# rvp-group/Splat-LOAM

Measured on AMD Instinct MI355X. Metric: fwd+bwd Msplats/s, higher is better.
Workload: dtype f32; 1 GPU; 500000 surfels, 64x2048 spherical, 1 keyframe/GPU per iteration drawn from a window of 8 keyframes as Mapper.optimize does (sample_geometric, p=0.4): render fwd + mapper loss + bwd + fused Adam (one native sls_mapping_step per iteration); step=one bench step = 10 mapping iterations (1013 steps = 10130 timed iterations), N=500000, H=64, W=2048, keyframes=8, parallelism=keyframe-dp1, status_read=lagged-1, gradient_sums=float atomics

## Files before the change

### splat_loam_amd/csrc/sls_launch.hpp

```cpp
#pragma once
#include "sls_common.hpp"

namespace sls {

struct ConsumerArgs;

inline bool launch_order_possible(int T) { return T % 32 == 0 && kTileW == 16 && kTileH == 16; }

struct ScanHandoff {
    const uint32_t *block_sums;
    int resort_windows;
    const uint64_t *resort_edges;
    int counted;
};

constexpr int kDirectChunk = 1024;
constexpr int kDirectMaxBins = 512;

struct DirectBin {
    uint32_t *cnt;
    uint32_t *totals;
    uint2 *serec;
    int bins, nchunks, pos0;
    int stride;
    uint32_t *coarse;
};
constexpr int kDirectGroup = 16;

size_t sort_scratch_bytes(uint64_t cap);
size_t order_scratch_bytes(int N);
int radix_sort_pairs_u32(uint32_t *keys, uint32_t *vals, uint32_t *keys_tmp, uint32_t *vals_tmp,
                         const uint32_t *count_ptr, uint32_t cap, int nbits, void *scratch, size_t scratch_bytes,
                         int *result_in_tmp, hipStream_t st);
void depth_order_key_buffers(int N, void *scratch, uint32_t *order, uint32_t **keys, uint32_t **vals0, uint32_t **n_dev);
uint64_t *resort_comp_buffer(int N, void *scratch);
bool bin_direct_possible(const DevCam &cam, int N, uint32_t cap);
DirectBin make_direct_bin(const DevCam &cam, int N, void *sort_scratch, uint2 *serec, bool repaired, bool coarse);
size_t direct_coarse_words(const DevCam &cam, int N);

struct DepthOrderScan {
    int N; const uint32_t *tiles; uint32_t *order, *offsets, *total_out;
    void *scratch; size_t scratch_bytes;
    int reuse_order;
    uint32_t *fail_flag;
    bool window_sort_done;
    const DirectBin *direct;
    const int4 *erec_box; int GX;
};
int launch_depth_order_scan(const DepthOrderScan &a, hipStream_t st, ScanHandoff *handoff);

struct BinSortLaunch {
    int N;
    const uint32_t *count_ptr; uint32_t cap;
    const uint32_t *order; const int32_t *rect; const uint32_t *tiles; const uint64_t *tile_mask; const int32_t *erec;
    const float *depth; const uint32_t *offsets;
    uint32_t *tkeys, *vals, *tkeys_tmp, *vals_tmp;
    void *scratch; size_t scratch_bytes;
    uint32_t *ranges; uint64_t *keys64_out; uint32_t *overflow;
    const ScanHandoff *handoff; uint32_t *total_out;
    const uint32_t *sbox; int bmask_mode;
};
int launch_bin_sort(const DevCam &cam, const BinSortLaunch &a, hipStream_t st, int *sorted_in_tmp, const uint2 **bmask_out);

struct BinDirectLaunch {
    int N; uint32_t cap;
    DirectBin db; bool counted;
    const uint32_t *order; const int32_t *erec_box; const int32_t *rect; const uint32_t *sbox;
    void *scratch; uint32_t *vals_out, *ranges, *total_out, *overflow;
    int resort_windows; const uint64_t *resort_edges; int bmask_mode;
    uint32_t *status_mirror;
};
int launch_bin_direct(const DevCam &cam, const BinDirectLaunch &a, hipStream_t st, const uint2 **bmask_out);

struct PreFwdLaunch {
    int N;
    int raw; float smax, pen; float *reg_out;
    const float *means, *scales, *rots, *opac;
    float *rec; int32_t *radii, *rect; uint32_t *tiles; float *depth;
    uint32_t *order_keys, *order_vals, *n_dev;
    uint32_t *status_clear;
    const float *col_cs, *row_cs; uint64_t *tile_mask;
    int32_t *erec; int erec_box;
    const uint32_t *resort_prev_order; uint64_t *resort_comp;
    uint32_t *sbox;
    uint32_t *zero_words; int n_zero_words;
};
int launch_preprocess_fwd(const DevCam &cam, const PreFwdLaunch &a, hipStream_t st);

struct PreBwdLaunch {
    int N;
    int raw; float smax, pen;
    const float *means, *scales, *rots, *opac;
    float *dmeans, *dscales, *drots, *dopac; const PoseOut *pose;
    const int32_t *radii; const float *grec; const AdamFuse *fuse;
};
int launch_preprocess_bwd(const DevCam &cam, const PreBwdLaunch &a, hipStream_t st);
int launch_preprocess_bwd_batch(const PreBwdLaunch &a, const BatchFuse &bf, hipStream_t st);
int launch_mark_visible(const DevCam &cam, int N, const float *means, uint8_t *visible, hipStream_t st);

size_t block_mask_bytes(uint64_t cap, int T);
struct RenderFwdLaunch {
    const uint32_t *ranges, *vals; const float *rec, *col_cs, *row_cs;
    float *allmap, *pix_state; uint32_t *pix_contrib, *tile_consumed; bool consumed_zeroed;
    uint64_t *block_masks;
    bool lean; uint32_t *block_cost;
    const uint2 *bmask;
    bool order_in_handover;
};
int launch_render_fwd(const DevCam &cam, const RenderFwdLaunch &a, hipStream_t st);

struct RenderBwdLaunch {
    const uint32_t *ranges, *vals; int vals_stride;
    const float *rec, *col_cs, *row_cs, *pix_state; const uint32_t *pix_contrib; const float *dL_dallmap;
    float *grec; uint8_t *touched; bool lean;
    const uint64_t *block_masks; int block_masks_shape;
    const ConsumerArgs *fused_consumer; bool consumer_b_inline;
    uint32_t *det_max; unsigned long long *det_acc;
    const uint8_t *det_prev; const uint32_t *det_gex; uint32_t *det_flag;
    const uint32_t *block_order; uint32_t order_tag;
    bool order_in_handover;
};
int launch_render_bwd(const DevCam &cam, const RenderBwdLaunch &a, hipStream_t st);

size_t consumer_scratch_bytes(int H, int W);
int launch_consumer(const ConsumerArgs &in, int n_valid, void *scratch, size_t scratch_bytes, bool no_launch, hipStream_t st,
                    ConsumerArgs *args_out_skip_c);
int launch_render_maps(int H, int W, const float *allmap, const float *rot9, const float *col_h, const float *row_h,
                       float depth_ratio, float *rend_normal, float *surf_depth, float *surf_normal, hipStream_t st);
int launch_densify_weights(int H, int W, const float *depth, const uint8_t *valid, const float *alpha, float thr, float *w_out,
                           uint32_t *stats, hipStream_t st);
int launch_densify_rows(int n, int H, int W, const int64_t *pix, const float *depth, const float *normal, const float *col_h,
                        const float *row_h, const float *c2w, const float *mTf, float *xyz, float *quat, hipStream_t st);

size_t densify_draw_scratch_bytes(int H, int W);
int launch_densify_draw(int H, int W, const float *depth, const uint8_t *valid, const float *alpha, float thr, double percentage,
                        uint64_t seed, uint32_t draw_index, float *w_out, int64_t *pixels_out, uint32_t *stats,
                        uint32_t *stats_mirror, void *scratch, hipStream_t st);
size_t surface_scratch_bytes(int H, int W);
int launch_surface_samples(int H, int W, const float *allmap, const float *col_h, const float *row_h, const float *M,
                           float min_opacity, float max_depth_dist, float depth_ratio, int n_samples, uint64_t seed,
                           uint32_t frame_id, float *points, float *normals, int32_t *pixels, uint32_t *status, void *scratch,
                           hipStream_t st);
size_t knn_scratch_bytes(int M);
int launch_knn(int M, const float *xyz, float *out, void *scratch, size_t scratch_bytes, hipStream_t st, int Mq);
int launch_touched_bitmap(int N, const uint8_t *touched, const float *scaling_raw, float smax, float pen,
                          const uint32_t *status_block, uint64_t *bitmap, hipStream_t st);
int launch_adam(const SlsAdamGroup *groups, int ngroups, double beta1, double beta2, double eps, int64_t step,
                const uint32_t *skip_flag, hipStream_t stream, const float *void_flags, uint32_t *status_block,
                uint32_t *status_mirror);

}
```

### splat_loam_amd/csrc/sls_pipeline.hip

```cpp
#include <stdlib.h>
#include <string.h>

#include "sls_consumer_dev.hpp"
#include "sls_launch.hpp"

namespace sls {

struct MapWs {
    float *rec; int32_t *radii; int32_t *rect; uint32_t *tiles; uint64_t *tmask; int32_t *erec; int32_t *serec; uint32_t *sbox; float *depth; uint32_t *order; uint32_t *offsets;
    void *order_scratch; size_t order_scratch_bytes;
    uint32_t *tkeys, *vals, *tkeys_tmp, *vals_tmp; void *sort_scratch; size_t sort_scratch_bytes;
    uint32_t *ranges; float *allmap; float *pix_state; uint32_t *pix_contrib; uint32_t *tile_consumed;
    float *dL_dallmap; void *consumer_scratch; size_t consumer_scratch_bytes; float *grec; size_t zero_bytes; uint64_t *block_masks; float *reg_accum; uint8_t *touched;
    uint32_t *det_max; unsigned long long *det_acc; size_t det_bytes;
    uint32_t *det_gex;
    uint32_t *block_cost, *block_order;
    size_t total;
};

struct Taker {
    char *p; size_t off;
    void *operator()(size_t bytes) { void *r = (void *)(p + off); off += (bytes + 255) & ~(size_t)255; return r; }
};

// ... 201 lines not shown
        po->out[g] = pose_grad[g];
    }
    return SLS_OK;
}
static const PoseOut *pose_arg(const PoseOut &po) { return po.counter ? &po : nullptr; }

int sls_backward(const SlsCamera *cam, int N, uint64_t R, const float *means3D, const float *scales,
                 const float *rotations, const int32_t *radii, const float *rec, const uint32_t *ranges,
                 const uint32_t *vals_sorted, int vals_stride, const float *col_cs, const float *row_cs,
                 const float *pix_state, const uint32_t *pix_contrib, const float *dL_dallmap, float *grec,
                 float *dL_dmeans3D, float *dL_dscales, float *dL_drotations, float *dL_dopacities,
                 const uint64_t *block_masks, int block_masks_shape, void *stream)
{
    return sls_backward_pose(cam, N, R, means3D, scales, rotations, radii, rec, ranges, vals_sorted, vals_stride, col_cs,
                             row_cs, pix_state, pix_contrib, dL_dallmap, grec, dL_dmeans3D, dL_dscales, dL_drotations,
                             dL_dopacities, block_masks, block_masks_shape, nullptr, nullptr, 0, stream);
}

int sls_backward_pose(const SlsCamera *cam, int N, uint64_t R, const float *means3D, const float *scales,
                      const float *rotations, const int32_t *radii, const float *rec, const uint32_t *ranges,
                      const uint32_t *vals_sorted, int vals_stride, const float *col_cs, const float *row_cs,
                      const float *pix_state, const uint32_t *pix_contrib, const float *dL_dallmap, float *grec,
                      float *dL_dmeans3D, float *dL_dscales, float *dL_drotations, float *dL_dopacities,
                      const uint64_t *block_masks, int block_masks_shape, float *pose_grad, void *pose_scratch,
                      size_t pose_scratch_bytes_, void *stream)
{
    SLS_REQUIRE(cam, "null pointer");
    SLS_REQUIRE(N >= 0, "negative N");
    if (N == 0) {
        if (pose_grad) SLS_HIP_CHECK(hipMemsetAsync(pose_grad, 0, 6 * sizeof(float), (hipStream_t)stream));
        return SLS_OK;
    }
    PoseOut po;
    if (int prc = make_pose_out(1, N, &pose_grad, pose_scratch, pose_scratch_bytes_, &po)) return prc;
    SLS_REQUIRE(means3D && scales && rotations && radii && grec && dL_dmeans3D && dL_dscales && dL_drotations &&
                    dL_dopacities,
                "null pointer");
    SLS_REQUIRE(vals_stride == 1 || vals_stride == 2, "vals_stride: 1 (plain list) or 2 ((surfel, block mask) pairs)");
    hipStream_t st = (hipStream_t)stream;
    const DevCam dc = make_devcam(*cam);
    {
        ScopedTimer tm(T_GREC_MEMSET, st);
        SLS_HIP_CHECK(hipMemsetAsync(grec, 0, sizeof(float) * (size_t)N * SLS_GREC_STRIDE, st));
    }
    if (R > 0) {
        SLS_REQUIRE(rec && ranges && vals_sorted && col_cs && row_cs && pix_state && pix_contrib && dL_dallmap,
                    "null pointer");
        RenderBwdLaunch rb{};
        rb.ranges = ranges; rb.vals = vals_sorted; rb.vals_stride = vals_stride; rb.rec = rec; rb.col_cs = col_cs; rb.row_cs = row_cs;
        rb.pix_state = pix_state; rb.pix_contrib = pix_contrib; rb.dL_dallmap = dL_dallmap;
        rb.block_masks = block_masks_shape ? block_masks : nullptr; rb.block_masks_shape = block_masks_shape;
        rb.lean = (cam->flags & SLS_CAM_LEAN_ALLMAP) != 0;
        rb.grec = grec; rb.order_in_handover = true;
        if (int rc = launch_render_bwd(dc, rb, st)) return rc;
    }
    PreBwdLaunch pb{};
    pb.N = N; pb.means = means3D; pb.scales = scales; pb.rots = rotations; pb.radii = radii; pb.grec = grec;
    pb.dmeans = dL_dmeans3D; pb.dscales = dL_dscales; pb.drots = dL_drotations; pb.dopac = dL_dopacities;
    pb.pose = pose_arg(po);
    return launch_preprocess_bwd(dc, pb, st);
}

size_t sls_backward_det_scratch_bytes(int N) { return N > 0 ? (size_t)N * SLS_GREC_STRIDE * 12 + 256 : 256; }

int sls_backward_det(const SlsCamera *cam, int N, uint64_t R, const float *means3D, const float *scales,
                     const float *rotations, const int32_t *radii, const float *rec, const uint32_t *ranges,
                     const uint32_t *vals_sorted, int vals_stride, const float *col_cs, const float *row_cs,
                     const float *pix_state, const uint32_t *pix_contrib, const float *dL_dallmap, float *dL_dmeans3D,
                     float *dL_dscales, float *dL_drotations, float *dL_dopacities, const uint64_t *block_masks,
                     int block_masks_shape, void *det_scratch, size_t det_scratch_bytes, void *stream)
{
    return sls_backward_det_pose(cam, N, R, means3D, scales, rotations, radii, rec, ranges, vals_sorted, vals_stride,
                                 col_cs, row_cs, pix_state, pix_contrib, dL_dallmap, dL_dmeans3D, dL_dscales,
                                 dL_drotations, dL_dopacities, block_masks, block_masks_shape, det_scratch,
                                 det_scratch_bytes, nullptr, nullptr, 0, stream);
}

int sls_backward_det_pose(const SlsCamera *cam, int N, uint64_t R, const float *means3D, const float *scales,
                          const float *rotations, const int32_t *radii, const float *rec, const uint32_t *ranges,
                          const uint32_t *vals_sorted, int vals_stride, const float *col_cs, const float *row_cs,
                          const float *pix_state, const uint32_t *pix_contrib, const float *dL_dallmap,
                          float *dL_dmeans3D, float *dL_dscales, float *dL_drotations, float *dL_dopacities,
                          const uint64_t *block_masks, int block_masks_shape, void *det_scratch, size_t det_scratch_bytes,
                          float *pose_grad, void *pose_scratch, size_t pose_scratch_bytes_, void *stream)
{
    SLS_REQUIRE(cam, "null pointer");
    SLS_REQUIRE(N >= 0, "negative N");
    if (N == 0) {
        if (pose_grad) SLS_HIP_CHECK(hipMemsetAsync(pose_grad, 0, 6 * sizeof(float), (hipStream_t)stream));
        return SLS_OK;
    }
    PoseOut po;
    if (int prc = make_pose_out(1, N, &pose_grad, pose_scratch, pose_scratch_bytes_, &po)) return prc;
    SLS_REQUIRE(means3D && scales && rotations && radii && det_scratch && dL_dmeans3D && dL_dscales && dL_drotations &&
                    dL_dopacities,
                "null pointer");
    SLS_REQUIRE(vals_stride == 1 || vals_stride == 2, "vals_stride: 1 (plain list) or 2 ((surfel, block mask) pairs)");
    if (det_scratch_bytes < sls_backward_det_scratch_bytes(N)) {
        set_error("deterministic-backward scratch too small");
        return SLS_E_SCRATCH;
    }
    hipStream_t st = (hipStream_t)stream;
    const DevCam dc = make_devcam(*cam);
    unsigned long long *acc = (unsigned long long *)(((uintptr_t)det_scratch + 255) & ~(uintptr_t)255);
    uint32_t *mx = (uint32_t *)(acc + (size_t)N * SLS_GREC_STRIDE);
    SLS_HIP_CHECK(hipMemsetAsync(acc, 0, (size_t)N * SLS_GREC_STRIDE * 12, st));
    if (R > 0) {
        SLS_REQUIRE(rec && ranges && vals_sorted && col_cs && row_cs && pix_state && pix_contrib && dL_dallmap,
                    "null pointer");
        RenderBwdLaunch rb{};
        rb.ranges = ranges; rb.vals = vals_sorted; rb.vals_stride = vals_stride; rb.rec = rec; rb.col_cs = col_cs; rb.row_cs = row_cs;
        rb.pix_state = pix_state; rb.pix_contrib = pix_contrib; rb.dL_dallmap = dL_dallmap;
        rb.block_masks = block_masks_shape ? block_masks : nullptr; rb.block_masks_shape = block_masks_shape;
        rb.lean = (cam->flags & SLS_CAM_LEAN_ALLMAP) != 0;
        rb.det_max = mx; rb.det_acc = acc; rb.order_in_handover = true;
        if (int rc = launch_render_bwd(dc, rb, st)) return rc;
    }
    AdamFuse fuse;
    memset(&fuse, 0, sizeof(fuse));
    fuse.det_max = mx;
    fuse.det_acc = (const long long *)acc;
    PreBwdLaunch pb{};
    pb.N = N; pb.means = means3D; pb.scales = scales; pb.rots = rotations; pb.radii = radii;
    pb.dmeans = dL_dmeans3D; pb.dscales = dL_dscales; pb.drots = dL_drotations; pb.dopac = dL_dopacities;
    pb.fuse = &fuse; pb.pose = pose_arg(po);
    return launch_preprocess_bwd(dc, pb, st);
}

struct FrontArgs {
    PreFwdLaunch pf;
    uint32_t *depth_order; int reuse_rounds;
    int workspace_ready;
    uint32_t *status_mirror;
    int list_pairs;
    float *allmap; bool lean;
    bool want_backward;
};

static int binning_front(const DevCam &dc, uint32_t cap, const MapWs &w, const FrontArgs &f, SlsMappingStatus *status_dev,
                         hipStream_t st, const uint32_t **sorted_list, int *sorted_stride)
{
    const int N = f.pf.N;
    if (!f.workspace_ready) {
        ScopedTimer tm(T_GREC_MEMSET, st);
        SLS_HIP_CHECK(hipMemsetAsync(w.reg_accum, 0, w.zero_bytes, st));
    }
    uint32_t *okeys, *ovals, *n_dev;
    uint32_t *order = f.depth_order ? f.depth_order : w.order;
    depth_order_key_buffers(N, w.order_scratch, order, &okeys, &ovals, &n_dev);
    const bool merged_sort = f.reuse_rounds >= 1;
    const bool direct = bin_direct_possible(dc, N, cap);
    BinDirectLaunch bd{};
    if (direct) bd.db = make_direct_bin(dc, N, w.sort_scratch, (uint2 *)w.serec, merged_sort, true);
    PreFwdLaunch pf = f.pf;
    pf.rec = w.rec; pf.order_vals = ovals; pf.n_dev = n_dev;
    pf.status_clear = (uint32_t *)status_dev; pf.tile_mask = w.tmask; pf.erec = w.erec;
    if (merged_sort) { pf.resort_prev_order = order; pf.resort_comp = resort_comp_buffer(N, w.order_scratch); }
    if (direct) {
        pf.order_keys = merged_sort ? nullptr : okeys;
        pf.erec_box = 1;
        if (bd.db.coarse) { pf.zero_words = bd.db.coarse; pf.n_zero_words = (int)direct_coarse_words(dc, N); }
    } else {
        pf.rect = w.rect; pf.tiles = w.tiles; pf.depth = w.depth; pf.order_keys = okeys; pf.sbox = w.sbox;
    }
    if (int rc = launch_preprocess_fwd(dc, pf, st)) return rc;
    ScanHandoff handoff = { nullptr, 0, nullptr, 0 };
    DepthOrderScan ds{};
    ds.N = N; ds.tiles = w.tiles; ds.order = order; ds.offsets = w.offsets; ds.total_out = &status_dev->R;
    ds.scratch = w.order_scratch; ds.scratch_bytes = w.order_scratch_bytes;
    ds.reuse_order = f.reuse_rounds; ds.fail_flag = &status_dev->overflow; ds.window_sort_done = merged_sort;
    ds.direct = direct ? &bd.db : nullptr; ds.erec_box = (const int4 *)w.erec; ds.GX = dc.GX;
    if (int rc = launch_depth_order_scan(ds, st, &handoff)) return rc;
    int in_tmp = 0, rc;
    const uint2 *bmask = nullptr;
    if (direct) {
        bd.N = N; bd.cap = cap; bd.counted = handoff.counted != 0; bd.order = order; bd.erec_box = w.erec;
        bd.scratch = w.sort_scratch; bd.vals_out = w.vals; bd.ranges = w.ranges;
        bd.total_out = &status_dev->R; bd.overflow = &status_dev->overflow;
        bd.resort_windows = handoff.resort_windows; bd.resort_edges = handoff.resort_edges;
        bd.bmask_mode = f.list_pairs; bd.status_mirror = f.status_mirror;
        rc = launch_bin_direct(dc, bd, st, &bmask);
    } else {
        BinSortLaunch bs{};
        bs.N = N; bs.count_ptr = &status_dev->R; bs.cap = cap; bs.order = order; bs.rect = w.rect; bs.tiles = w.tiles;
        bs.tile_mask = dc.tile_cull ? w.tmask : nullptr; bs.erec = (dc.GX < 65536 && dc.GY < 65536) ? w.erec : nullptr;
        bs.depth = w.depth; bs.offsets = w.offsets; bs.sbox = w.sbox; bs.bmask_mode = f.list_pairs;
        bs.tkeys = w.tkeys; bs.vals = w.vals; bs.tkeys_tmp = w.tkeys_tmp; bs.vals_tmp = w.vals_tmp;
        bs.scratch = w.sort_scratch; bs.scratch_bytes = w.sort_scratch_bytes; bs.ranges = w.ranges;
        bs.overflow = &status_dev->overflow; bs.handoff = &handoff; bs.total_out = &status_dev->R;
        rc = launch_bin_sort(dc, bs, st, &in_tmp, &bmask);
    }
    if (rc) return rc;
    *sorted_list = bmask ? (const uint32_t *)bmask : (in_tmp ? w.vals_tmp : w.vals);
    *sorted_stride = bmask ? 2 : 1;
    RenderFwdLaunch rf{};
    rf.ranges = w.ranges; rf.vals = *sorted_list; rf.rec = w.rec; rf.col_cs = pf.col_cs; rf.row_cs = pf.row_cs;
    rf.allmap = f.allmap; rf.pix_state = w.pix_state; rf.pix_contrib = w.pix_contrib; rf.lean = f.lean; rf.bmask = bmask;
    rf.consumed_zeroed = true;
    if (f.want_backward) { rf.block_masks = w.block_masks; rf.block_cost = w.block_cost; }
    return launch_render_fwd(dc, rf, st);
}

size_t sls_forward_ws_bytes(int N, int H, int W, uint64_t R_capacity)
{
    return (N < 0 || H <= 0 || W <= 0) ? 0 : carve(N, H, W, R_capacity, nullptr, false).total;
}

int sls_forward_ws(const SlsCamera *cam, int N, const float *means3D, const float *scales, const float *rotations,
                   const float *opacities, const float *col_cs, const float *row_cs, uint64_t R_capacity,
                   uint32_t *depth_order, int reuse_rounds, int list_pairs, int workspace_ready, int want_backward,
                   int32_t *radii, float *allmap, void *workspace, size_t workspace_bytes, SlsMappingStatus *status_dev,
                   SlsMappingStatus *status_mirror, const uint32_t **sorted_list, int *sorted_stride,
                   int *block_masks_shape, void *stream)
{
    SLS_REQUIRE(cam && status_dev && workspace && sorted_list && sorted_stride && block_masks_shape, "null pointer");
    SLS_REQUIRE(N > 0, "N must be positive");
    SLS_REQUIRE(means3D && scales && rotations && opacities && col_cs && row_cs && radii && allmap, "null pointer");
    SLS_REQUIRE(R_capacity > 0 && R_capacity < (1ull << 32), "bad instance capacity");
    SLS_REQUIRE(((uintptr_t)workspace & 255) == 0, "workspace must be 256-byte aligned");
    SLS_REQUIRE(reuse_rounds >= 0 && reuse_rounds <= 4, "reuse_rounds: 0 from scratch, 1..4 repair rounds");
    SLS_REQUIRE(reuse_rounds == 0 || depth_order, "a repair needs the camera's previous depth order");
    SLS_REQUIRE(list_pairs >= 0 && list_pairs <= 2, "list_pairs: 0 auto, 1 whenever possible, 2 never");
    const int H = cam->H, W = cam->W;
    const DevCam dc = make_devcam(*cam);
    const uint32_t cap = (uint32_t)R_capacity;
    if (!bin_direct_possible(dc, N, cap)) {
        set_error("sls_forward_ws serves what the direct binning serves (<= 512 tiles, D10 off): use the staged forward");
        return SLS_E_UNSUPPORTED;
    }
    const MapWs w = carve(N, H, W, R_capacity, workspace, false);
    if (workspace_bytes < w.total) {
        set_error("forward workspace too small: %zu < %zu", workspace_bytes, w.total);
        return SLS_E_SCRATCH;
    }
    FrontArgs f{};
    f.pf.N = N; f.pf.means = means3D; f.pf.scales = scales; f.pf.rots = rotations; f.pf.opac = opacities;
    f.pf.col_cs = col_cs; f.pf.row_cs = row_cs; f.pf.radii = radii;
    f.depth_order = depth_order; f.reuse_rounds = reuse_rounds; f.workspace_ready = workspace_ready;
    f.status_mirror = (uint32_t *)status_mirror;
    f.list_pairs = list_pairs; f.allmap = allmap; f.lean = (cam->flags & SLS_CAM_LEAN_ALLMAP) != 0;
    f.want_backward = want_backward != 0;
    *block_masks_shape = want_backward ? 3 : 0;
    return binning_front(dc, cap, w, f, status_dev, (hipStream_t)stream, sorted_list, sorted_stride);
}

int sls_backward_ws(const SlsCamera *cam, int N, const float *means3D, const float *scales, const float *rotations,
                    const int32_t *radii, const float *col_cs, const float *row_cs, const float *dL_dallmap,
                    uint64_t R_capacity, void *workspace, size_t workspace_bytes, const uint32_t *sorted_list,
                    int sorted_stride, int block_masks_shape, uint32_t *block_order, float *dL_dmeans3D,
                    float *dL_dscales, float *dL_drotations, float *dL_dopacities, void *stream)
{
    return sls_backward_ws_pose(cam, N, means3D, scales, rotations, radii, col_cs, row_cs, dL_dallmap, R_capacity, workspace,
                                workspace_bytes, sorted_list, sorted_stride, block_masks_shape, block_order, dL_dmeans3D,
                                dL_dscales, dL_drotations, dL_dopacities, nullptr, nullptr, 0, stream);
}

int sls_backward_ws_pose(const SlsCamera *cam, int N, const float *means3D, const float *scales, const float *rotations,
                         const int32_t *radii, const float *col_cs, const float *row_cs, const float *dL_dallmap,
                         uint64_t R_capacity, void *workspace, size_t workspace_bytes, const uint32_t *sorted_list,
                         int sorted_stride, int block_masks_shape, uint32_t *block_order, float *dL_dmeans3D,
                         float *dL_dscales, float *dL_drotations, float *dL_dopacities, float *pose_grad,
                         void *pose_scratch, size_t pose_scratch_bytes_, void *stream)
{
    SLS_REQUIRE(cam && workspace && sorted_list, "null pointer");
    SLS_REQUIRE(N > 0, "N must be positive");
    PoseOut po;
    if (int prc = make_pose_out(1, N, &pose_grad, pose_scratch, pose_scratch_bytes_, &po)) return prc;
    SLS_REQUIRE(means3D && scales && rotations && radii && col_cs && row_cs && dL_dallmap && dL_dmeans3D && dL_dscales &&
                    dL_drotations && dL_dopacities,
                "null pointer");
    SLS_REQUIRE(sorted_stride == 1 || sorted_stride == 2, "sorted_stride: 1 (plain list) or 2 ((surfel, block mask) pairs)");
    const MapWs w = carve(N, cam->H, cam->W, R_capacity, workspace, false);
    if (workspace_bytes < w.total) {
        set_error("forward workspace too small: %zu < %zu", workspace_bytes, w.total);
        return SLS_E_SCRATCH;
    }
    hipStream_t st = (hipStream_t)stream;
    const DevCam dc = make_devcam(*cam);
    const int T = dc.GX * dc.GY;
    const bool order_bwd = block_order != nullptr && block_masks_shape == 3 && launch_order_possible(T);
    RenderBwdLaunch rb{};
    rb.ranges = w.ranges; rb.vals = sorted_list; rb.vals_stride = sorted_stride; rb.rec = w.rec; rb.col_cs = col_cs; rb.row_cs = row_cs;
    rb.pix_state = w.pix_state; rb.pix_contrib = w.pix_contrib; rb.dL_dallmap = dL_dallmap;
    rb.block_masks = block_masks_shape ? w.block_masks : nullptr; rb.block_masks_shape = block_masks_shape;
    rb.lean = (cam->flags & SLS_CAM_LEAN_ALLMAP) != 0;
    rb.grec = w.grec; rb.touched = w.touched;
    if (order_bwd) { rb.block_order = block_order; rb.order_tag = block_order_tag(T); }
    if (int rc = launch_render_bwd(dc, rb, st)) return rc;
    AdamFuse fuse;
    memset(&fuse, 0, sizeof(fuse));
    fuse.clear_grec = 1;
    fuse.touched = w.touched;
    if (order_bwd) { fuse.order_T = T; fuse.order_cost = w.block_cost; fuse.order_out = block_order; }
    PreBwdLaunch pb{};
    pb.N = N; pb.means = means3D; pb.scales = scales; pb.rots = rotations; pb.radii = radii; pb.grec = w.grec;
    pb.dmeans = dL_dmeans3D; pb.dscales = dL_dscales; pb.drots = dL_drotations; pb.dopac = dL_dopacities;
    pb.fuse = &fuse; pb.pose = pose_arg(po);
    return launch_preprocess_bwd(dc, pb, st);
}

struct StepSwitches {
    bool det, det_one;
    bool fuse_c, fuse_b;
    bool order_bwd;
};
static StepSwitches step_switches(const SlsMappingConfig *cfg, int deterministic, bool have_det_prev, bool have_block_order, int T)
{
    StepSwitches s;
    s.det = deterministic != 0;
    s.det_one = deterministic == 2 && have_det_prev;
    s.fuse_c = cfg->depth_ratio == 0.0f;
    s.fuse_b = s.fuse_c && have_block_order;
    s.order_bwd = launch_order_possible(T);
    return s;
}

static void loss_weights(const SlsMappingConfig *cfg, int H, int W, int n_valid, float *lw)
{
    lw[0] = 1.0f / ((float)H * (float)W);
    lw[1] = n_valid > 0 ? cfg->lambda_normal * (1.0f / (float)n_valid) : 0.0f;
    lw[2] = n_valid > 0 ? cfg->lambda_alpha * (1.0f / (float)n_valid) : 0.0f;
}

static void fill_step_fuse(AdamFuse &af, const SlsMappingConfig *cfg, SlsMappingStatus *status_dev, float *reg_accum, int N,
                           float *exp_avg, float *exp_avg_sq, int64_t adam_step)
{
    static_assert(sizeof(SlsMappingStatus) == 32, "the mirror copy moves 8 words");
    af.status_src = (uint32_t *)status_dev; af.status_mirror = (uint32_t *)cfg->status_mirror;
    af.reg_accum = reg_accum; af.void_flags = cfg->void_flags_out;
    const bool aligned = (N % 2 == 0) && ((((uintptr_t)exp_avg | (uintptr_t)exp_avg_sq) & 15) == 0);
    if (!cfg->apply_adam || !aligned) return;
    af.enabled = 1;
    af.write_grads = cfg->keep_grads;
    af.c = make_adam_coef(cfg->beta1, cfg->beta2, cfg->eps, adam_step);
    af.lr_xyz = cfg->lr_xyz; af.lr_opacity = cfg->lr_opacity;
    af.lr_scaling = cfg->lr_scaling; af.lr_rotation = cfg->lr_rotation;
    af.exp_avg = exp_avg; af.exp_avg_sq = exp_avg_sq;
}

static int fallback_adam(const SlsMappingConfig *cfg, int N, float *xyz, float *scaling_raw, float *rotation_raw,
                         float *opacity_raw, float *grads, float *exp_avg, float *exp_avg_sq, int64_t adam_step,
                         const uint32_t *skip_flag, hipStream_t st)
{
    SlsAdamGroup grp[4];
    memset(grp, 0, sizeof(grp));
    float *params[4] = { xyz, opacity_raw, scaling_raw, rotation_raw };
    const size_t offs[4] = { 0, (size_t)3 * N, (size_t)4 * N, (size_t)6 * N };
    const int64_t numel[4] = { (int64_t)3 * N, (int64_t)N, (int64_t)2 * N, (int64_t)4 * N };
    const float lrs[4] = { cfg->lr_xyz, cfg->lr_opacity, cfg->lr_scaling, cfg->lr_rotation };
    for (int k = 0; k < 4; ++k) {
        grp[k].param = params[k];
        grp[k].grad = grads + offs[k];
        grp[k].exp_avg = exp_avg + offs[k];
        grp[k].exp_avg_sq = exp_avg_sq + offs[k];
        grp[k].numel = numel[k];
        grp[k].lr = lrs[k];
    }
    return launch_adam(grp, 4, cfg->beta1, cfg->beta2, cfg->eps, adam_step, skip_flag, st, nullptr, nullptr, nullptr);
}

static int mapping_front(const SlsCamera *cam, int N, const float *xyz, const float *scaling_raw, const float *rotation_raw,
                         const float *opacity_raw, const float *gt_depth, const uint8_t *valid, int n_valid,
                         const float *col_cs, const float *row_cs, const float *col_cs_half, const float *row_cs_half,
                         const SlsMappingConfig *cfg, const StepSwitches &sw, uint32_t cap, const MapWs &w,
                         SlsMappingStatus *status_dev, hipStream_t st)
{
    const DevCam dc = make_devcam(*cam);
    const int T = dc.GX * dc.GY;
    FrontArgs f{};
    f.pf.N = N; f.pf.raw = 1; f.pf.smax = cfg->scaling_max; f.pf.pen = cfg->scaling_max_penalty; f.pf.reg_out = w.reg_accum;
    f.pf.means = xyz; f.pf.scales = scaling_raw; f.pf.rots = rotation_raw; f.pf.opac = opacity_raw;
    f.pf.col_cs = col_cs; f.pf.row_cs = row_cs; f.pf.radii = w.radii;
    f.depth_order = cfg->depth_order; f.reuse_rounds = cfg->reuse_depth_order; f.workspace_ready = cfg->workspace_ready;
    f.list_pairs = cfg->block_masks; f.allmap = w.allmap;
// ... 12 lines not shown
    if (sw.det && !sw.det_one) SLS_HIP_CHECK(hipMemsetAsync(w.det_max, 0, w.det_bytes, st));
    RenderBwdLaunch rb{};
    rb.ranges = w.ranges; rb.vals = sorted_vals; rb.vals_stride = vals_stride; rb.rec = w.rec; rb.col_cs = col_cs; rb.row_cs = row_cs;
    rb.pix_state = w.pix_state; rb.pix_contrib = w.pix_contrib; rb.dL_dallmap = w.dL_dallmap; rb.grec = w.grec;
    rb.block_masks = w.block_masks; rb.block_masks_shape = 3;
    rb.lean = sw.fuse_c;
    rb.touched = w.touched;
    rb.fused_consumer = sw.fuse_c ? &cargs : nullptr; rb.consumer_b_inline = sw.fuse_b;
    rb.det_max = (sw.det && !sw.det_one) ? w.det_max : nullptr; rb.det_acc = sw.det ? w.det_acc : nullptr;
    rb.det_prev = sw.det_one ? cfg->det_prev : nullptr; rb.det_gex = w.det_gex; rb.det_flag = &status_dev->overflow;
    if (sw.order_bwd) rb.block_order = sw.fuse_b ? cfg->block_order : w.block_order;
    if (sw.fuse_b && sw.order_bwd) rb.order_tag = block_order_tag(T);
    if (int rc = launch_render_bwd(dc, rb, st)) return rc;
    if (cfg->phase == 1 && cfg->grad_bitmap)
        return launch_touched_bitmap(N, w.touched, scaling_raw, cfg->scaling_max, cfg->scaling_max_penalty,
                                     (const uint32_t *)status_dev, cfg->grad_bitmap, st);
    return SLS_OK;
}

size_t sls_mapping_workspace_bytes(int N, int H, int W, uint64_t R_capacity)
{
    return (N < 0 || H <= 0 || W <= 0) ? 0 : carve(N, H, W, R_capacity, nullptr, true).total;
}

size_t sls_block_order_bytes(int H, int W)
{
    if (H <= 0 || W <= 0) return 0;
    const size_t T = (size_t)((W + kTileW - 1) / kTileW) * (size_t)((H + kTileH - 1) / kTileH);
    return sizeof(uint32_t) * (1 + T * (size_t)(kTilePix / 16));
}

size_t sls_mapping_workspace_bytes_cfg(int N, int H, int W, uint64_t R_capacity, const SlsMappingConfig *cfg)
{
    return (N < 0 || H <= 0 || W <= 0) ? 0 : carve(N, H, W, R_capacity, nullptr, !cfg || cfg->deterministic != 0).total;
}

int sls_mapping_step(const SlsCamera *cam, int N, float *xyz, float *scaling_raw, float *rotation_raw,
                     float *opacity_raw, float *grads, float *exp_avg, float *exp_avg_sq, int64_t adam_step,
                     const float *gt_depth, const uint8_t *valid, int n_valid, const float *col_cs,
                     const float *row_cs, const float *col_cs_half, const float *row_cs_half,
                     const SlsMappingConfig *cfg, uint64_t R_capacity, void *workspace, size_t workspace_bytes,
                     SlsMappingStatus *status_dev, float **allmap_out, void *stream)
{
    SLS_REQUIRE(cam && cfg && status_dev && workspace, "null pointer");
    SLS_REQUIRE(N > 0, "N must be positive");
    SLS_REQUIRE(xyz && scaling_raw && rotation_raw && opacity_raw && grads && gt_depth && valid && col_cs && row_cs &&
                    col_cs_half && row_cs_half,
                "null pointer");
    SLS_REQUIRE(!cfg->apply_adam || (exp_avg && exp_avg_sq && adam_step >= 1), "Adam state missing");
    SLS_REQUIRE(R_capacity > 0 && R_capacity < (1ull << 32), "bad instance capacity");
    SLS_REQUIRE(((uintptr_t)workspace & 255) == 0, "workspace must be 256-byte aligned");
    SLS_REQUIRE(cfg->phase >= 0 && cfg->phase <= 2, "phase: 0 whole iteration, 1 up to the tile backward, 2 the rest");
    PoseOut po;
    {
        float *pg = cfg->pose_grad;
        if (int prc = make_pose_out(1, N, &pg, cfg->pose_scratch, cfg->pose_scratch_bytes, &po)) return prc;
    }
    SLS_REQUIRE(!cfg->grad_bitmap || ((!cfg->apply_adam || cfg->union_bitmap) && !cfg->grad_chunk),
                "the gradient bitmap belongs to apply_adam = 0 with the flat bucket");
    SLS_REQUIRE(!cfg->union_bitmap || (cfg->phase == 2 && cfg->apply_adam && cfg->union_prefix && cfg->grad_compact && cfg->grad_compact_index &&
                                       !cfg->grad_chunk && !cfg->keep_grads && (N % 2) == 0 &&
                                       ((((uintptr_t)exp_avg | (uintptr_t)exp_avg_sq) & 15) == 0)),
                "union_bitmap: phase 2 with apply_adam = 1, the union's prefix and row buffer, even N, 16-byte aligned moments");
    SLS_REQUIRE(!cfg->grad_chunk ||
                    (!cfg->apply_adam && cfg->grad_ranks >= 1 && (cfg->grad_chunk % 4u) == 0 && (N % 2) == 0 &&
                     (uint64_t)cfg->grad_chunk * cfg->grad_ranks >= (uint64_t)10 * (uint64_t)N &&
                     (uint64_t)10 * (uint64_t)N < (1ull << 32)),
                "reduce-scatter gradient layout: apply_adam = 0, even N, chunk a multiple of 4 covering 10 N");
    const int H = cam->H, W = cam->W;
    const MapWs w = carve(N, H, W, R_capacity, workspace, cfg->deterministic != 0);
    if (workspace_bytes < w.total) {
        set_error("mapping workspace too small: %zu < %zu", workspace_bytes, w.total);
        return SLS_E_SCRATCH;
    }
    hipStream_t st = (hipStream_t)stream;
    const DevCam dc = make_devcam(*cam);
    const uint32_t cap = (uint32_t)R_capacity;
    if (allmap_out) *allmap_out = w.allmap;
    SLS_REQUIRE(cfg->deterministic >= 0 && cfg->deterministic <= 2, "deterministic: 0 off, 1 two launches, 2 one launch with predicted scales");
    SLS_REQUIRE(cfg->deterministic != 2 || cfg->det_prev, "deterministic = 2 needs the keyframe's det_prev buffer");
    const int T = dc.GX * dc.GY;
    const StepSwitches sw = step_switches(cfg, cfg->deterministic, cfg->det_prev != nullptr, cfg->block_order != nullptr, T);
    int rc = SLS_OK;
    if (cfg->phase != 2)
        rc = mapping_front(cam, N, xyz, scaling_raw, rotation_raw, opacity_raw, gt_depth, valid, n_valid, col_cs, row_cs,
                           col_cs_half, row_cs_half, cfg, sw, cap, w, status_dev, st);
    if (rc || cfg->phase == 1) return rc;
    AdamFuse fuse;
    memset(&fuse, 0, sizeof(fuse));
    fill_step_fuse(fuse, cfg, status_dev, w.reg_accum, N, exp_avg, exp_avg_sq, adam_step);
    if (fuse.enabled) fuse.skip_flag = &status_dev->overflow;
    fuse.clear_grec = 1;
    fuse.touched = w.touched;
    fuse.void_count = 1; fuse.void_stride = 0;
    if (sw.det) {
        fuse.det_max = w.det_max; fuse.det_acc = (const long long *)w.det_acc;
        fuse.det_prev = cfg->det_prev; fuse.det_gex = w.det_gex; fuse.det_onepass = sw.det_one ? 1 : 0;
    }
    if (sw.fuse_b) {
        fuse.loss_partials = (const float *)w.consumer_scratch;
        fuse.n_loss_partials = T * (kTilePix / 16);
        loss_weights(cfg, H, W, n_valid, fuse.loss_w);
        if (sw.order_bwd) { fuse.order_T = T; fuse.order_cost = w.block_cost; fuse.order_out = cfg->block_order; }
    }
    if (cfg->grad_bitmap && cfg->phase != 2) { fuse.grad_bitmap = cfg->grad_bitmap; fuse.grad_bitmap_words = (N + 63) / 64; }
    if (cfg->grad_chunk) {
        fuse.gchunk = cfg->grad_chunk; fuse.gbase = grads;
        fuse.void_flags = grads + cfg->grad_chunk; fuse.void_count = (int)cfg->grad_ranks; fuse.void_stride = (int)cfg->grad_chunk + 4;
    }
    if (cfg->union_bitmap) {
        fuse.union_bitmap = cfg->union_bitmap; fuse.union_prefix = cfg->union_prefix;
        fuse.compact = cfg->grad_compact; fuse.compact_idx = cfg->grad_compact_index; fuse.compact_cap = cfg->grad_compact_capacity;
    }
    PreBwdLaunch pb{};
    pb.N = N; pb.raw = 1; pb.smax = cfg->scaling_max; pb.pen = cfg->scaling_max_penalty;
    pb.means = xyz; pb.scales = scaling_raw; pb.rots = rotation_raw; pb.opac = opacity_raw; pb.radii = w.radii; pb.grec = w.grec;
    pb.dmeans = grads; pb.dopac = grads + (size_t)3 * N; pb.dscales = grads + (size_t)4 * N; pb.drots = grads + (size_t)6 * N;
    pb.fuse = &fuse; pb.pose = pose_arg(po);
    rc = launch_preprocess_bwd(dc, pb, st);
    if (rc || !cfg->apply_adam || fuse.enabled) return rc;
    return fallback_adam(cfg, N, xyz, scaling_raw, rotation_raw, opacity_raw, grads, exp_avg, exp_avg_sq, adam_step,
                         &status_dev->overflow, st);
}

size_t sls_mapping_workspace_bytes_batch(int G, int N, int H, int W, uint64_t R_capacity, const SlsMappingConfig *cfg)
{
    if (G < 1 || G > SLS_MAX_BATCH || N < 0 || H <= 0 || W <= 0) return 0;
    return carve_batch(G, N, H, W, R_capacity, nullptr, !cfg || cfg->deterministic != 0, nullptr);
}

int sls_mapping_step_batch(int G, const SlsKeyframeInputs *kfs, int N, float *xyz, float *scaling_raw, float *rotation_raw,
                           float *opacity_raw, float *grads, float *exp_avg, float *exp_avg_sq, int64_t adam_step,
                           const SlsMappingConfig *cfg, uint64_t R_capacity, void *workspace, size_t workspace_bytes,
                           SlsMappingStatus *status_dev, void *stream)
{
    SLS_REQUIRE(G >= 1 && G <= SLS_MAX_BATCH, "G: 1 to SLS_MAX_BATCH keyframes");
    SLS_REQUIRE(kfs && cfg && status_dev && workspace, "null pointer");
    SLS_REQUIRE(N > 0, "N must be positive");
    SLS_REQUIRE(xyz && scaling_raw && rotation_raw && opacity_raw && grads, "null pointer");
    SLS_REQUIRE(!cfg->apply_adam || (exp_avg && exp_avg_sq && adam_step >= 1), "Adam state missing");
    SLS_REQUIRE(R_capacity > 0 && R_capacity < (1ull << 32), "bad instance capacity");
    SLS_REQUIRE(((uintptr_t)workspace & 255) == 0, "workspace must be 256-byte aligned");
    SLS_REQUIRE(cfg->phase == 0 && !cfg->grad_chunk && !cfg->grad_bitmap && !cfg->union_bitmap,
                "a batch is one whole step on the flat bucket: phase 0, no grad_chunk, grad_bitmap or union_bitmap");
    SLS_REQUIRE(cfg->deterministic >= 0 && cfg->deterministic <= 2, "deterministic: 0 off, 1 two launches, 2 one launch with predicted scales");
    const int H = kfs[0].cam.H, W = kfs[0].cam.W;
    SLS_REQUIRE(H > 0 && W > 0, "bad image size");
    for (int g = 0; g < G; ++g) {
        const SlsKeyframeInputs &k = kfs[g];
        SLS_REQUIRE(k.cam.H == H && k.cam.W == W, "the keyframes of a batch share one image size");
        SLS_REQUIRE(k.gt_depth && k.valid && k.col_cs && k.row_cs && k.col_cs_half && k.row_cs_half && k.depth_order,
                    "null per-keyframe pointer");
        SLS_REQUIRE((k.block_order != nullptr) == (kfs[0].block_order != nullptr), "block_order on every keyframe or on none");
        SLS_REQUIRE(k.reuse_depth_order >= 0 && k.reuse_depth_order <= 4, "reuse_depth_order: 0 from scratch, 1..4 repair rounds");
        for (int h = 0; h < g; ++h) {
            SLS_REQUIRE(kfs[h].depth_order != k.depth_order, "two keyframes share one depth_order buffer");
            SLS_REQUIRE(!k.block_order || kfs[h].block_order != k.block_order, "two keyframes share one block_order buffer");
            SLS_REQUIRE(!k.det_prev || kfs[h].det_prev != k.det_prev, "two keyframes share one det_prev buffer");
        }
    }
    SLS_REQUIRE(!cfg->pose_grad, "a batch takes its pose gradients per keyframe: SlsKeyframeInputs.pose_grad");
    PoseOut po;
    {
        float *pg[SLS_MAX_BATCH];
        for (int g = 0; g < G; ++g) pg[g] = kfs[g].pose_grad;
        if (int prc = make_pose_out(G, N, pg, cfg->pose_scratch, cfg->pose_scratch_bytes, &po)) return prc;
    }
    const bool det = cfg->deterministic != 0;
    MapWs ws[SLS_MAX_BATCH];
    const size_t need = carve_batch(G, N, H, W, R_capacity, workspace, det, ws);
    if (workspace_bytes < need) {
        set_error("batch workspace too small: %zu < %zu", workspace_bytes, need);
        return SLS_E_SCRATCH;
    }
    hipStream_t st = (hipStream_t)stream;
    const uint32_t cap = (uint32_t)R_capacity;
    const DevCam dc0 = make_devcam(kfs[0].cam);
    const int T = dc0.GX * dc0.GY;
    const StepSwitches sw = step_switches(cfg, det ? 1 : 0, false, kfs[0].block_order != nullptr, T);
    BatchFuse bf;
    memset(&bf, 0, sizeof(bf));
    bf.G = G;
    for (int g = 0; g < G; ++g) {
        const SlsKeyframeInputs &k = kfs[g];
        const MapWs &w = ws[g];
        SlsMappingConfig kc = *cfg;
        kc.reuse_depth_order = k.reuse_depth_order; kc.depth_order = k.depth_order;
        kc.block_order = k.block_order; kc.det_prev = k.det_prev; kc.deterministic = det ? 1 : 0;
        if (g > 0) kc.scaling_max_penalty = 0.0f;
        int rc = mapping_front(&k.cam, N, xyz, scaling_raw, rotation_raw, opacity_raw, k.gt_depth, k.valid, k.n_valid,
                               k.col_cs, k.row_cs, k.col_cs_half, k.row_cs_half, &kc, sw, cap, w, status_dev + 1 + g, st);
        if (rc) return rc;
        BatchKeyframe &b = bf.kf[g];
        b.cam = make_devcam(k.cam);
        b.radii = w.radii; b.grec = (float4 *)w.grec; b.touched = w.touched;
        b.status = (uint32_t *)(status_dev + 1 + g);
        if (det) {
            b.det_max = w.det_max; b.det_acc = (long long *)w.det_acc;
            b.det_prev = k.det_prev;
        }
        if (sw.fuse_b) {
            b.loss_partials = (const float *)w.consumer_scratch;
            loss_weights(cfg, H, W, k.n_valid, b.loss_w);
            if (sw.order_bwd) { b.order_cost = w.block_cost; b.order_out = k.block_order; }
        }
    }
    if (sw.fuse_b) {
        bf.n_loss_partials = T * (kTilePix / 16);
        if (sw.order_bwd) bf.order_T = T;
    }
    AdamFuse &af = bf.af;
    fill_step_fuse(af, cfg, status_dev, ws[0].reg_accum, N, exp_avg, exp_avg_sq, adam_step);
    PreBwdLaunch pb{};
    pb.N = N; pb.raw = 1; pb.smax = cfg->scaling_max; pb.pen = cfg->scaling_max_penalty;
    pb.means = xyz; pb.scales = scaling_raw; pb.rots = rotation_raw; pb.opac = opacity_raw;
    pb.dmeans = grads; pb.dopac = grads + (size_t)3 * N; pb.dscales = grads + (size_t)4 * N; pb.drots = grads + (size_t)6 * N;
    pb.pose = pose_arg(po);
    int rc = launch_preprocess_bwd_batch(pb, bf, st);
    if (rc || !cfg->apply_adam || af.enabled) return rc;
    return fallback_adam(cfg, N, xyz, scaling_raw, rotation_raw, opacity_raw, grads, exp_avg, exp_avg_sq, adam_step,
                         &status_dev->overflow, st);
}

}
```

### splat_loam_amd/csrc/sls_preprocess.hip

```cpp
#include <cstring>
#include "sls_common.hpp"
#include "sls_consumer_dev.hpp"
#include "sls_resort.hpp"
#include "sls_launch.hpp"

namespace sls {

__device__ __forceinline__ float dot3(const float *a, const float *b)
{
    return fmaf(a[0], b[0], fmaf(a[1], b[1], a[2] * b[2]));
}
__device__ __forceinline__ void cross3(const float *a, const float *b, float *o)
{
    o[0] = fmaf(a[1], b[2], -(a[2] * b[1]));
    o[1] = fmaf(a[2], b[0], -(a[0] * b[2]));
    o[2] = fmaf(a[0], b[1], -(a[1] * b[0]));
}
__device__ __forceinline__ void matvec(const float *M, const float *v, float *o)
{
#pragma unroll
    for (int i = 0; i < 3; ++i) o[i] = dot3(M + 3 * i, v);
}
__device__ __forceinline__ void matTvec(const float *M, const float *v, float *o)
{
#pragma unroll
    for (int i = 0; i < 3; ++i) o[i] = fmaf(M[i], v[0], fmaf(M[3 + i], v[1], M[6 + i] * v[2]));
}
__device__ __forceinline__ int floordiv_i(int a, int b)
{
    int q = a / b;
    if ((a % b != 0) && ((a < 0) != (b < 0))) --q;
    return q;
}
__device__ __forceinline__ int posmod_i(int a, int b)
{
    int m = a % b;
    return m < 0 ? m + b : m;
}
__device__ __forceinline__ int to_int_clamped(float v)
{
    v = fminf(fmaxf(v, -1.0e9f), 1.0e9f);
    return (int)v;
}
__device__ __forceinline__ void quat_axes(const float4 q, float *tu, float *tv, float *tn)
{
    const float r = q.x, x = q.y, y = q.z, z = q.w;
    tu[0] = 1.0f - 2.0f * fmaf(y, y, z * z);
    tu[1] = 2.0f * fmaf(x, y, r * z);
    tu[2] = 2.0f * fmaf(x, z, -(r * y));
    tv[0] = 2.0f * fmaf(x, y, -(r * z));
    tv[1] = 1.0f - 2.0f * fmaf(x, x, z * z);
    tv[2] = 2.0f * fmaf(y, z, r * x);
    tn[0] = 2.0f * fmaf(x, z, r * y);
    tn[1] = 2.0f * fmaf(y, z, -(r * x));
    tn[2] = 1.0f - 2.0f * fmaf(x, x, y * y);
}
__device__ __forceinline__ float asin01_approx(float s)
{
    const float c = __builtin_amdgcn_sqrtf(fmaf(-s, s, 1.0f));
    const float mx = fmaxf(s, c), mn = fminf(s, c);
    const float r = sls_atan_unit(mn * __builtin_amdgcn_rcpf(mx));
    return s > c ? SLS_PIO2 - r : r;
}
template <bool EXACT>
__device__ __forceinline__ void ball_extent(float rad, float rho, float rxy, float &theta, float &daz)
{
    if (!(rad < rho)) { theta = SLS_PI; daz = SLS_PI; return; }
    if (EXACT) {
        theta = sls_asin01(rad / rho);
        const float q = rad / rxy;
        if (!(q < 1.0f)) daz = SLS_PI;
        else daz = sls_asin01(q);
    } else {
        theta = asin01_approx(rad * __builtin_amdgcn_rcpf(rho));
        const float q = rad * __builtin_amdgcn_rcpf(rxy);
        if (!(q < 0.9999f)) daz = SLS_PI;
        else daz = asin01_approx(q);
    }
}

__device__ __forceinline__ uint32_t s_rect_cnt(const int4 rc) { return (uint32_t)(rc.y * rc.w); }

struct SurfelGeom {
    float p[3], rho, rho2, rxy, rxy2;
    float Tu[3], Tv[3], Tn[3], n[3], A[3], B[3], Hu[3], Hv[3];
    float su, sv, sig, c;
};

__device__ __forceinline__ float frcp(float x) { return __builtin_amdgcn_rcpf(x); }
__device__ __forceinline__ float fsqrt(float x) { return __builtin_amdgcn_sqrtf(x); }

template <bool EXACT_ROOTS>
__device__ __forceinline__ void surfel_geom(const DevCam &cam, const float *m, const float2 s, const float4 q,
                                            SurfelGeom &g)
{
#pragma unroll
    for (int k = 0; k < 3; ++k)
        g.p[k] = fmaf(cam.R[3 * k], m[0], fmaf(cam.R[3 * k + 1], m[1], fmaf(cam.R[3 * k + 2], m[2], cam.t[k])));
    g.rxy2 = fmaf(g.p[0], g.p[0], g.p[1] * g.p[1]);
    g.rho2 = fmaf(g.p[2], g.p[2], g.rxy2);
    g.rho = EXACT_ROOTS ? sqrtf(g.rho2) : fsqrt(g.rho2);
    g.rxy = EXACT_ROOTS ? sqrtf(g.rxy2) : fsqrt(g.rxy2);
    float tu[3], tv[3], tn[3];
    quat_axes(q, tu, tv, tn);
    matvec(cam.R, tu, g.Tu);
    matvec(cam.R, tv, g.Tv);
    matvec(cam.R, tn, g.Tn);
    g.su = s.x * cam.mod;
    g.sv = s.y * cam.mod;
    g.c = dot3(g.Tn, g.p);
    g.sig = (g.c > 0.0f) ? -1.0f : 1.0f;
    const float isu = g.sig * frcp(g.su), isv = -g.sig * frcp(g.sv);
#pragma unroll
    for (int k = 0; k < 3; ++k) {
        g.n[k] = g.sig * g.Tn[k];
        g.A[k] = g.Tv[k] * isu;
        g.B[k] = g.Tu[k] * isv;
    }
    cross3(g.A, g.p, g.Hu);
    cross3(g.B, g.p, g.Hv);
}

struct RegArgs {
    int raw;
    float smax, pen;
    float *reg_out;
    uint32_t *status_clear;
    uint32_t *zero_words;
    int n_zero_words;
};

template <bool EXACT>
__device__ __forceinline__ void activate(const RegArgs &ra, float2 &s, float4 &q, float &o)
{
    if (!ra.raw) return;
    const float n2 = q.x * q.x + q.y * q.y + q.z * q.z + q.w * q.w;
    s.x = expf(s.x); s.y = expf(s.y);
    o = frcp(1.0f + __expf(-o));
    const float inv = frcp(fmaxf(fsqrt(n2), 1e-12f));
    q.x *= inv; q.y *= inv; q.z *= inv; q.w *= inv;
}

struct PreFwdArgs {
    const float *means; const float2 *scales; const float4 *rots; const float *opac;
    float4 *rec; int *radii; int4 *rect; uint32_t *tiles; float *depth; uint32_t *order_keys, *order_vals, *n_dev;
    const float2 *col_cs, *row_cs; uint64_t *tile_mask; int4 *erec;
    uint32_t *sbox;
    int erec_box;
};
constexpr int kPreCullBytes = 64 * (int)(sizeof(SlsTileCullSurfel) + sizeof(int4) + 4 * sizeof(uint32_t)) + 16;
constexpr int kPreSliceBytes = kPreCullBytes > 64 * kRec4 * 16 ? kPreCullBytes : 64 * kRec4 * 16;

template <int WAVES>
__device__ __forceinline__ void preprocess_fwd_body(const DevCam &cam, const RegArgs &ra, int N, const PreFwdArgs &pa,
                                                    int first, unsigned char *s_mem, float *s_part)
{
    const float *__restrict__ means = pa.means; const float2 *__restrict__ scales = pa.scales;
    const float4 *__restrict__ rots = pa.rots; const float *__restrict__ opac = pa.opac;
    float4 *__restrict__ rec = pa.rec; int *__restrict__ radii = pa.radii; int4 *__restrict__ rect = pa.rect;
    uint32_t *__restrict__ tiles = pa.tiles; float *__restrict__ depth = pa.depth;
    uint32_t *__restrict__ order_keys = pa.order_keys, *__restrict__ order_vals = pa.order_vals, *__restrict__ n_dev = pa.n_dev;
    const float2 *__restrict__ col_cs = pa.col_cs, *__restrict__ row_cs = pa.row_cs;
    uint64_t *__restrict__ tile_mask = pa.tile_mask; int4 *__restrict__ erec = pa.erec;
    const int i = first + (int)threadIdx.x;
    uint32_t my_tiles = 0;
    uint64_t my_mask = 0;
    bool tested = false;
    SlsTileCullSurfel cull;
    int4 my_rc = make_int4(0, 0, 0, 0);
    float my_reg = 0.0f;
    if (i == 0 && n_dev) *n_dev = (uint32_t)N;
    if (ra.zero_words && i < N) {
        for (int k = i; k < ra.n_zero_words; k += N) ra.zero_words[k] = 0u;
    }
    if (i == 0 && ra.status_clear) {
#pragma unroll
        for (int k = 0; k < 8; ++k) ra.status_clear[k] = 0u;
    }
    float4 q0 = make_float4(0, 0, 0, 0), q1 = q0, q2 = q0, q3 = q0, q4 = q0;
    if (i < N) {
        int r_out = 0;
        int4 rc = make_int4(0, 0, 0, 0);
        float dep = 0.0f;

        const float m[3] = { means[3 * i], means[3 * i + 1], means[3 * i + 2] };
        float2 s = scales[i];
        float4 q = rots[i];
        float o = opac[i];
        activate<true>(ra, s, q, o);
        if (ra.pen != 0.0f) my_reg = ra.pen * fmaxf(fmaxf(s.x, s.y) - ra.smax, 0.0f);
        SurfelGeom g;
        surfel_geom<true>(cam, m, s, q, g);
        bool vis = (g.rho >= cam.near_c) && (g.rho < 1.0e18f);
        if (vis) {
            const float az = sls_atan2(g.p[1], g.p[0]);
            const float el = sls_atan2(g.p[2], g.rxy);
            const float cpx = fmaf(cam.fx, az, cam.cx), cpy = fmaf(cam.fy, el, cam.cy);
            const float smax = fmaxf(g.su, g.sv);
            float theta, daz;
            ball_extent<true>(SLS_CUTOFF * smax, g.rho, g.rxy, theta, daz);
            const float rx = fmaxf(fabsf(cam.fx) * daz, SLS_RMIN_PX);
            const float ry = fmaxf(fabsf(cam.fy) * theta, SLS_RMIN_PX);
            int xlo = to_int_clamped(floorf(cpx - rx + 0.5f));
            int xhi = to_int_clamped(floorf(cpx + rx + 0.5f));
            int ylo = to_int_clamped(floorf(cpy - ry + 0.5f));
            int yhi = to_int_clamped(floorf(cpy + ry + 0.5f));
            ylo = max(ylo, 0);
            yhi = min(yhi, cam.H - 1);
            int txlo = 0, ncols = 0;
            if (ylo > yhi) vis = false;
            if (vis) {
                if (cam.wrap) {
                    if ((long long)xhi - (long long)xlo + 1 >= (long long)cam.W) { txlo = 0; ncols = cam.GX; }
                    else {
                        const int a = floordiv_i(xlo, kTileW), b = floordiv_i(xhi, kTileW);
                        ncols = min(b - a + 1, cam.GX);
                        txlo = posmod_i(a, cam.GX);
                    }
                } else {
                    xlo = max(xlo, 0);
                    xhi = min(xhi, cam.W - 1);
                    if (xlo > xhi) vis = false;
                    else { txlo = xlo / kTileW; ncols = xhi / kTileW - txlo + 1; }
                }
            }
            if (vis) {
                const int tylo = ylo / kTileH, nrows = yhi / kTileH - tylo + 1;
                rc = make_int4(txlo, ncols, tylo, nrows);
                my_tiles = (uint32_t)(ncols * nrows);
                my_rc = rc;
                const float dcv[3] = { g.p[0] / g.rho, g.p[1] / g.rho, g.p[2] / g.rho };
                my_mask = my_tiles >= 64u ? ~0ull : ((1ull << my_tiles) - 1ull);
                tested = cam.tile_cull > 0 && tile_mask && my_tiles >= (uint32_t)cam.tile_cull && my_tiles <= 64u;
                if (tested) sls_tile_cull_surfel(g.Tu, g.Tv, g.n, g.p, dcv, g.su, g.sv, o, cpx, cpy, &cull);
                r_out = to_int_clamped(ceilf(fmaxf(rx, ry)));
                dep = g.rho;
                float ex = -1.0e30f, ey = -1.0e30f, kc = 0.0f;
                const float lo = 255.0f * o;
                if (lo > 1.0f) {
                    const float rho_max = 2.0f * __logf(lo) * 1.001f + 1.0e-3f;
                    float th2, daz2;
                    const float kk = __builtin_amdgcn_sqrtf(rho_max), rad = kk * smax;
                    kc = kk * 1.0001f;
                    ball_extent<false>(rad, g.rho, g.rxy, th2, daz2);
                    const float r2 = __builtin_amdgcn_sqrtf(0.5f * rho_max);
                    if (g.rxy > 2.0f * rad && g.rxy > 0.5f * g.rho) {
                        const float irxy2 = __builtin_amdgcn_rcpf(g.rxy2), irho2 = __builtin_amdgcn_rcpf(g.rho2);
                        const float au = (g.p[0] * g.Tu[1] - g.p[1] * g.Tu[0]) * irxy2;
                        const float av = (g.p[0] * g.Tv[1] - g.p[1] * g.Tv[0]) * irxy2;
                        const float rat_xy = rad * __builtin_amdgcn_rcpf(g.rxy - rad);
                        const float az_ell = kk * __builtin_amdgcn_sqrtf(g.su * g.su * au * au + g.sv * g.sv * av * av) + 0.75f * rat_xy * rat_xy;
                        const float zr = g.p[2] * __builtin_amdgcn_rcpf(g.rxy) * irho2;
                        const float eu = -zr * (g.p[0] * g.Tu[0] + g.p[1] * g.Tu[1]) + g.rxy * irho2 * g.Tu[2];
                        const float ev = -zr * (g.p[0] * g.Tv[0] + g.p[1] * g.Tv[1]) + g.rxy * irho2 * g.Tv[2];
                        const float rat = rad * __builtin_amdgcn_rcpf(g.rho - rad);
                        const float el_ell = kk * __builtin_amdgcn_sqrtf(g.su * g.su * eu * eu + g.sv * g.sv * ev * ev) + 1.5f * rat * rat;
                        daz2 = fminf(daz2, az_ell * 1.02f);
                        th2 = fminf(th2, el_ell * 1.02f);
                    }
                    ex = fmaxf(fabsf(cam.fx) * daz2, r2) * 1.001f + 0.05f;
                    ey = fmaxf(fabsf(cam.fy) * th2, r2) * 1.001f + 0.05f;
                }
                q0 = make_float4(g.Hu[0], g.Hu[1], g.Hu[2], g.sig * g.c);
                q1 = make_float4(g.Hv[0], g.Hv[1], g.Hv[2], g.rho);
                q2 = make_float4(g.n[0], g.n[1], g.n[2], o);
                q3 = make_float4(dcv[0], dcv[1], dcv[2], kc);
                q4 = make_float4(cpx, cpy, ex, ey);
            }
        }
        radii[i] = r_out;
        if (rect) rect[i] = rc;
        if (depth) depth[i] = dep;
        if (order_keys) {
            order_keys[i] = depth_order_key(g.rho);
            if (order_vals) order_vals[i] = (uint32_t)i;
        }
    }
    if (__ballot(tested)) {
        const int lane = threadIdx.x & 63, wave = threadIdx.x >> 6;
        int4 *s_rect_w = reinterpret_cast<int4 *>(s_mem + (size_t)wave * kPreSliceBytes);
        SlsTileCullSurfel *s_cull_w = reinterpret_cast<SlsTileCullSurfel *>(s_rect_w + 64);
        uint32_t *s_scan_w = reinterpret_cast<uint32_t *>(s_cull_w + 64);
        uint32_t *s_drop_w = s_scan_w + 64;
        uint32_t *s_seg_w = s_drop_w + 128;
        uint32_t *s_ends_w = s_seg_w + 64;
        if (tested) s_cull_w[lane] = cull;
        s_rect_w[lane] = tested ? my_rc : make_int4(0, 1, 0, 1);
        uint32_t incl = tested ? my_tiles : 0u;
#pragma unroll
        for (int off = 1; off < 64; off <<= 1) {
            const uint32_t t = __shfl_up(incl, off, 64);
            if (lane >= off) incl += t;
        }
        s_scan_w[lane] = incl;
        s_drop_w[2 * lane] = 0u; s_drop_w[2 * lane + 1] = 0u;
        {
            const uint64_t tb = __ballot(tested);
            if (tested) s_seg_w[__popcll(tb & ((1ull << lane) - 1ull))] = (uint32_t)lane;
            if (lane == 0) { s_ends_w[0] = 0u; s_ends_w[1] = 0u; }
        }
        int seg_base = 0;
        const uint32_t total = (uint32_t)__shfl((int)incl, 63, 64);
        __builtin_amdgcn_wave_barrier();
        for (uint32_t base = 0; base < total; base += 64u) {
            const uint32_t j = base + (uint32_t)lane;
            const bool valid = j < total;
            if (tested && incl > base && incl <= base + 64u) atomicOr(&s_ends_w[(incl - 1u - base) >> 5], 1u << ((incl - 1u - base) & 31u));
            __builtin_amdgcn_wave_barrier();
            const uint64_t ends = ((uint64_t)s_ends_w[1] << 32) | (uint64_t)s_ends_w[0];
            __builtin_amdgcn_wave_barrier();
            if (lane == 0) { s_ends_w[0] = 0u; s_ends_w[1] = 0u; }
            const int seg = seg_base + (int)__popcll(ends & ((1ull << lane) - 1ull));
            seg_base += (int)__popcll(ends);
            const int owner = valid ? (int)s_seg_w[min(seg, 63)] : 0;
            const uint32_t idx = valid ? j - (s_scan_w[owner] - s_rect_cnt(s_rect_w[owner])) : 0u;
            const int4 orc = s_rect_w[owner];
            const int ncols = max(orc.y, 1);
            const int ky = (int)idx / ncols, kx = (int)idx - ky * ncols;
            int tx = orc.x + kx;
            if (tx >= cam.GX) tx -= cam.GX;
            const int ty = orc.z + ky;
            const int x0 = tx * kTileW, y0 = ty * kTileH;
            const float2 cc = col_cs[min(max(x0 + kTileW / 2 - 1, 0), cam.W - 1)], rr = row_cs[min(max(y0 + kTileH / 2 - 1, 0), cam.H - 1)];
            const int out = sls_tile_outside(&cam.tc, &s_cull_w[owner], (float)x0, (float)y0, cc.x, cc.y, rr.x, rr.y);
            if (valid && out) atomicOr(&s_drop_w[2 * owner + (int)(idx >> 5)], 1u << (idx & 31u));
        }
// ... 559 lines not shown
        }
    }
    if (i >= N) { if constexpr (POSE) goto pose_reduce; else return; }
    {
    uint32_t skip = 0u;
#pragma unroll
    for (int g = 0; g < SLS_MAX_BATCH; ++g) {
        if (g >= bf.G) break;
        skip |= bf.kf[g].status[1];
    }
    float dm[3] = { 0, 0, 0 };
    float2 ds = make_float2(0, 0);
    float4 dq = make_float4(0, 0, 0, 0);
    float dop = 0.0f;
    const float2 s_in = scales[i];
    float2 s = s_in;
    const float4 q_in = rots[i];
    float4 q = q_in;
    const float o_in = opac[i];
    float o = o_in;
    activate<false>(ra, s, q, o);
    const float m[3] = { means[3 * i], means[3 * i + 1], means[3 * i + 2] };
#pragma unroll
    for (int kg = 0; kg < SLS_MAX_BATCH; ++kg) {
        if (kg >= bf.G) break;
        const BatchKeyframe &kf = bf.kf[kg];
        if (kf.touched[i] == 0) continue;
        kf.touched[i] = 0;
        if (kf.radii[i] <= 0) continue;
        SurfelGeom g;
        surfel_geom<false>(kf.cam, m, s, q, g);
        float4 g0, g1, g2, g3;
        if (kf.det_acc) {
            float gv[16];
#pragma unroll
            for (int k = 0; k < 16; ++k) {
                const int ex = (int)((kf.det_max[(size_t)i * 16 + k] >> 23) & 0xFFu);
                gv[k] = (float)ldexp((double)kf.det_acc[(size_t)i * 16 + k], ex - 166);
                kf.det_acc[(size_t)i * 16 + k] = 0;
            }
            if (kf.det_prev && skip == 0u) {
                uint32_t pw[4];
#pragma unroll
                for (int w4 = 0; w4 < 4; ++w4) {
                    pw[w4] = 0u;
#pragma unroll
                    for (int b = 0; b < 4; ++b) pw[w4] |= det_predict(gv[4 * w4 + b]) << (8 * b);
                }
                reinterpret_cast<uint4 *>(kf.det_prev)[i] = make_uint4(pw[0], pw[1], pw[2], pw[3]);
                if (kf.det_gex) {
#pragma unroll
                    for (int k = 0; k < 16; ++k) {
                        const uint32_t pe = (pw[k >> 2] >> (8 * (k & 3))) & 0xFFu;
                        if (pe > kf.det_gex[k]) atomicMax(&kf.det_gex[k], pe);
                    }
                }
            }
            g0 = make_float4(gv[0], gv[1], gv[2], gv[3]); g1 = make_float4(gv[4], gv[5], gv[6], gv[7]);
            g2 = make_float4(gv[8], gv[9], gv[10], gv[11]); g3 = make_float4(gv[12], gv[13], gv[14], gv[15]);
        } else {
            float4 *rec = kf.grec + (size_t)i * 4;
            g0 = rec[0]; g1 = rec[1]; g2 = rec[2]; g3 = rec[3];
            const float4 z = make_float4(0.0f, 0.0f, 0.0f, 0.0f);
            rec[0] = z; rec[1] = z; rec[2] = z; rec[3] = z;
        }
        float dmk[3], dopk;
        float2 dsk;
        float4 dqk;
        chain_grad_record<POSE>(kf.cam, g, q, g0, g1, g2, g3, dmk, dsk, dopk, dqk, pg[POSE ? kg : 0]);
        dm[0] += dmk[0]; dm[1] += dmk[1]; dm[2] += dmk[2];
        ds.x += dsk.x; ds.y += dsk.y;
        dop += dopk;
        dq.x += dqk.x; dq.y += dqk.y; dq.z += dqk.z; dq.w += dqk.w;
    }
    if (ra.pen != 0.0f) {
        const bool first = s.x >= s.y;
        if ((first ? s.x : s.y) >= ra.smax) { if (first) ds.x += ra.pen; else ds.y += ra.pen; }
    }
    ds.x *= s.x; ds.y *= s.y;
    dop *= o * (1.0f - o);
    {
        const float nrm = fsqrt(q_in.x * q_in.x + q_in.y * q_in.y + q_in.z * q_in.z + q_in.w * q_in.w);
        const float inv = frcp(fmaxf(nrm, 1e-12f));
        const float dd = dq.x * q.x + dq.y * q.y + dq.z * q.z + dq.w * q.w;
        dq.x = (dq.x - dd * q.x) * inv; dq.y = (dq.y - dd * q.y) * inv;
        dq.z = (dq.z - dd * q.z) * inv; dq.w = (dq.w - dd * q.w) * inv;
    }
    if (!af.enabled || af.write_grads) {
        dmeans[3 * i] = dm[0]; dmeans[3 * i + 1] = dm[1]; dmeans[3 * i + 2] = dm[2];
        dscales[i] = ds;
        drots[i] = dq;
        dopac[i] = dop;
    }
    if (af.enabled && skip == 0u) {
        const size_t n = (size_t)N, ix = 3 * (size_t)i, io = 3 * n + i, is = 4 * n + 2 * (size_t)i, ir = 6 * n + 4 * (size_t)i;
        float *M = af.exp_avg, *V = af.exp_avg_sq;
        float p, mm, vv;
        const float ibc1 = frcp(af.c.bc1);
        const float st_x = af.lr_xyz * ibc1, st_o = af.lr_opacity * ibc1;
        const float st_s = af.lr_scaling * ibc1, st_r = af.lr_rotation * ibc1;
#pragma unroll
        for (int k = 0; k < 3; ++k) {
            p = m[k]; mm = M[ix + k]; vv = V[ix + k];
            adam_one(p, dm[k], mm, vv, st_x, af.c);
            means[3 * i + k] = p; M[ix + k] = mm; V[ix + k] = vv;
        }
        p = o_in; mm = M[io]; vv = V[io];
        adam_one(p, dop, mm, vv, st_o, af.c);
        opac[i] = p; M[io] = mm; V[io] = vv;
        float2 ps = s_in, ms = *reinterpret_cast<float2 *>(M + is), vs = *reinterpret_cast<float2 *>(V + is);
        adam_one(ps.x, ds.x, ms.x, vs.x, st_s, af.c);
        adam_one(ps.y, ds.y, ms.y, vs.y, st_s, af.c);
        scales[i] = ps; *reinterpret_cast<float2 *>(M + is) = ms; *reinterpret_cast<float2 *>(V + is) = vs;
        float4 pq = q_in, mq = *reinterpret_cast<float4 *>(M + ir), vq = *reinterpret_cast<float4 *>(V + ir);
        adam_one(pq.x, dq.x, mq.x, vq.x, st_r, af.c);
        adam_one(pq.y, dq.y, mq.y, vq.y, st_r, af.c);
        adam_one(pq.z, dq.z, mq.z, vq.z, st_r, af.c);
        adam_one(pq.w, dq.w, mq.w, vq.w, st_r, af.c);
        rots[i] = pq; *reinterpret_cast<float4 *>(M + ir) = mq; *reinterpret_cast<float4 *>(V + ir) = vq;
    }
    }
pose_reduce:
    if constexpr (POSE) {
        const PoseOut &po = pose_arg(pose_args...);
        const int row = (int)blockIdx.x - 1 - n_ord, nb = (int)gridDim.x - 1 - n_ord;
#pragma unroll
        for (int g = 0; g < SLS_MAX_BATCH; ++g) {
            if (g >= bf.G) break;
            pose_block_row(pg[g], po.rows + ((size_t)g * nb + row) * kPoseRow);
        }
        pose_finish(po, bf.G, nb);
    }
}

__global__ __launch_bounds__(256) void mark_visible_kernel(DevCam cam, int N, const float *__restrict__ means,
                                                           uint8_t *__restrict__ visible)
{
    const int i = blockIdx.x * 256 + threadIdx.x;
    if (i >= N) return;
    float p[3];
#pragma unroll
    for (int k = 0; k < 3; ++k)
        p[k] = fmaf(cam.R[3 * k], means[3 * i], fmaf(cam.R[3 * k + 1], means[3 * i + 1], fmaf(cam.R[3 * k + 2], means[3 * i + 2], cam.t[k])));
    const float rho = sqrtf(fmaf(p[2], p[2], fmaf(p[0], p[0], p[1] * p[1])));
    visible[i] = (rho >= cam.near_c && rho < 1.0e18f) ? 1 : 0;
}

int launch_preprocess_fwd(const DevCam &cam, const PreFwdLaunch &a, hipStream_t st)
{
    const int N = a.N;
    RegArgs ra;
    ra.raw = a.raw; ra.smax = a.smax; ra.pen = a.pen; ra.reg_out = a.reg_out; ra.status_clear = a.status_clear;
    ra.zero_words = a.zero_words; ra.n_zero_words = a.n_zero_words;
    PreFwdArgs pa;
    pa.means = a.means; pa.scales = (const float2 *)a.scales; pa.rots = (const float4 *)a.rots; pa.opac = a.opac;
    pa.rec = (float4 *)a.rec; pa.radii = a.radii; pa.rect = (int4 *)a.rect; pa.tiles = a.tiles; pa.depth = a.depth;
    pa.order_keys = a.order_keys; pa.order_vals = a.order_vals; pa.n_dev = a.n_dev;
    pa.col_cs = (const float2 *)a.col_cs; pa.row_cs = (const float2 *)a.row_cs;
    pa.tile_mask = (a.col_cs && a.row_cs) ? a.tile_mask : nullptr;
    pa.erec = (cam.GX < 65536 && cam.GY < 65536) ? (int4 *)a.erec : nullptr;
    pa.sbox = block_box_fits(cam.GX * kTileW, cam.H) ? a.sbox : nullptr;
    pa.erec_box = (a.erec_box && pa.erec && block_box_fits(cam.GX * kTileW, cam.H)) ? 1 : 0;
    ScopedTimer tm(T_PREPROCESS_FWD, st);
    if (a.resort_prev_order && a.resort_comp) {
        pa.order_vals = nullptr;
        const int nw = (N + kResortWindow - 1) / kResortWindow, nb = (N + 511) / 512;
        hipLaunchKernelGGL(preprocess_fwd_resort_kernel, dim3(nw + nb), dim3(512), 0, st, cam, ra, N, pa, nw, a.resort_prev_order,
                           a.resort_comp);
        SLS_LAUNCH_CHECK("preprocess_fwd_resort_kernel");
        return SLS_OK;
    }
    hipLaunchKernelGGL(preprocess_fwd_kernel, dim3((N + 255) / 256), dim3(256), 0, st, cam, ra, N, pa);
    SLS_LAUNCH_CHECK("preprocess_fwd_kernel");
    return SLS_OK;
}

int launch_preprocess_bwd(const DevCam &cam, const PreBwdLaunch &a, hipStream_t st)
{
    const int N = a.N, nb = (N + 255) / 256;
    RegArgs ra{};
    ra.raw = a.raw; ra.smax = a.smax; ra.pen = a.pen;
    AdamFuse af;
    memset(&af, 0, sizeof(af));
    if (a.fuse) af = *a.fuse;
    af.publisher = (af.loss_partials || af.reg_accum || af.void_flags || af.status_mirror || af.grad_bitmap) ? 1 : 0;
    ScopedTimer tm(T_PREPROCESS_BWD, st);
    if (a.pose)
        hipLaunchKernelGGL((preprocess_bwd_kernel<true, PoseOut>), dim3(nb + af.publisher + (af.order_out ? 8 : 0)), dim3(256), 0, st, cam, ra, af, N,
                           const_cast<float *>(a.means), (float2 *)const_cast<float *>(a.scales), (float4 *)const_cast<float *>(a.rots),
                           const_cast<float *>(a.opac), a.radii, (float4 *)const_cast<float *>(a.grec), a.dmeans, (float2 *)a.dscales,
                           (float4 *)a.drots, a.dopac, *a.pose);
    else
        hipLaunchKernelGGL(preprocess_bwd_kernel<false>, dim3(nb + af.publisher + (af.order_out ? 8 : 0)), dim3(256), 0, st, cam, ra, af, N,
                           const_cast<float *>(a.means), (float2 *)const_cast<float *>(a.scales), (float4 *)const_cast<float *>(a.rots),
                           const_cast<float *>(a.opac), a.radii, (float4 *)const_cast<float *>(a.grec), a.dmeans, (float2 *)a.dscales,
                           (float4 *)a.drots, a.dopac);
    SLS_LAUNCH_CHECK("preprocess_bwd_kernel");
    return SLS_OK;
}

int launch_preprocess_bwd_batch(const PreBwdLaunch &a, const BatchFuse &bf, hipStream_t st)
{
    const int N = a.N, nb = (N + 255) / 256;
    float *means = const_cast<float *>(a.means), *scales = const_cast<float *>(a.scales), *rots = const_cast<float *>(a.rots),
          *opac = const_cast<float *>(a.opac);
    RegArgs ra{};
    ra.raw = 1; ra.smax = a.smax; ra.pen = a.pen;
    ScopedTimer tm(T_PREPROCESS_BWD, st);
    if (a.pose)
        hipLaunchKernelGGL((preprocess_bwd_batch_kernel<true, PoseOut>), dim3(nb + 1 + (bf.order_T > 0 ? 8 * bf.G : 0)), dim3(256), 0, st, ra, bf, N,
                           means, (float2 *)scales, (float4 *)rots, opac, a.dmeans, (float2 *)a.dscales, (float4 *)a.drots, a.dopac, *a.pose);
    else
        hipLaunchKernelGGL(preprocess_bwd_batch_kernel<false>, dim3(nb + 1 + (bf.order_T > 0 ? 8 * bf.G : 0)), dim3(256), 0, st, ra, bf, N,
                           means, (float2 *)scales, (float4 *)rots, opac, a.dmeans, (float2 *)a.dscales, (float4 *)a.drots, a.dopac);
    SLS_LAUNCH_CHECK("preprocess_bwd_batch_kernel");
    return SLS_OK;
}

int launch_mark_visible(const DevCam &cam, int N, const float *means, uint8_t *visible, hipStream_t st)
{
    const int nb = (N + 255) / 256;
    hipLaunchKernelGGL(mark_visible_kernel, dim3(nb), dim3(256), 0, st, cam, N, means, visible);
    SLS_LAUNCH_CHECK("mark_visible_kernel");
    return SLS_OK;
}

}
```

### splat_loam_amd/csrc/sls_resort.hpp

```cpp
#pragma once
#include "sls_common.hpp"

namespace sls {

constexpr int kResortWindow = 1024;
constexpr uint32_t kResortFailed = 2u;

constexpr int kResortThreads = 512;
static_assert(kResortWindow == 2 * kResortThreads, "one pair of elements per thread");

template <int M>
__device__ __forceinline__ uint32_t lane_xor_u32(uint32_t v)
{
    static_assert(M == 1 || M == 2 || M == 4 || M == 8 || M == 16 || M == 32, "lane distance inside a wave");
    if (M == 1) return (uint32_t)__builtin_amdgcn_update_dpp(0, (int)v, 0xB1, 0xF, 0xF, true);
    if (M == 2) return (uint32_t)__builtin_amdgcn_update_dpp(0, (int)v, 0x4E, 0xF, 0xF, true);
    if (M == 4) {
        int a = __builtin_amdgcn_update_dpp(0, (int)v, 0x104, 0xF, 0x5, false);
        a = __builtin_amdgcn_update_dpp(a, (int)v, 0x114, 0xF, 0xA, false);
        return (uint32_t)a;
    }
    if (M == 8) return (uint32_t)__builtin_amdgcn_update_dpp(0, (int)v, 0x128, 0xF, 0xF, false);
    return (uint32_t)__shfl_xor((int)v, M, 64);
}
template <int M>
__device__ __forceinline__ uint64_t lane_xor_u64(uint64_t v)
{
    return ((uint64_t)lane_xor_u32<M>((uint32_t)(v >> 32)) << 32) | lane_xor_u32<M>((uint32_t)v);
}
__device__ __forceinline__ void keep64(uint64_t &e, uint64_t p, bool keep_min)
{
    e = ((p < e) == keep_min) ? p : e;
}
template <int M>
__device__ __forceinline__ void bitonic_stage(uint64_t &e0, uint64_t &e1, bool asc, ulonglong2 *s_pairs)
{
    const int t = threadIdx.x;
    const bool keep_min = ((t & M) == 0) == asc;
    uint64_t p0, p1;
    if constexpr (M >= 64) {
        s_pairs[t] = make_ulonglong2(e0, e1);
        __syncthreads();
        const ulonglong2 pp = s_pairs[t ^ M];
        p0 = pp.x; p1 = pp.y;
        __syncthreads();
    } else {
        p0 = lane_xor_u64<M>(e0); p1 = lane_xor_u64<M>(e1);
    }
    keep64(e0, p0, keep_min);
    keep64(e1, p1, keep_min);
}
template <int K>
__device__ __forceinline__ void bitonic_width(uint64_t &e0, uint64_t &e1, ulonglong2 *s_pairs)
{
    const bool asc = (K == kResortWindow) || ((2 * (int)threadIdx.x) & K) == 0;
    if constexpr (K >= 1024) bitonic_stage<256>(e0, e1, asc, s_pairs);
    if constexpr (K >= 512) bitonic_stage<128>(e0, e1, asc, s_pairs);
    if constexpr (K >= 256) bitonic_stage<64>(e0, e1, asc, s_pairs);
    if constexpr (K >= 128) bitonic_stage<32>(e0, e1, asc, s_pairs);
    if constexpr (K >= 64) bitonic_stage<16>(e0, e1, asc, s_pairs);
    if constexpr (K >= 32) bitonic_stage<8>(e0, e1, asc, s_pairs);
    if constexpr (K >= 16) bitonic_stage<4>(e0, e1, asc, s_pairs);
    if constexpr (K >= 8) bitonic_stage<2>(e0, e1, asc, s_pairs);
    if constexpr (K >= 4) bitonic_stage<1>(e0, e1, asc, s_pairs);
    const bool sw = (e0 > e1) == asc;
    const uint64_t lo = sw ? e1 : e0, hi = sw ? e0 : e1;
    e0 = lo; e1 = hi;
}
template <int K0>
__device__ __forceinline__ void bitonic_pairs(uint64_t &e0, uint64_t &e1, ulonglong2 *s_pairs)
{
    if constexpr (K0 <= 2) bitonic_width<2>(e0, e1, s_pairs);
    if constexpr (K0 <= 4) bitonic_width<4>(e0, e1, s_pairs);
    if constexpr (K0 <= 8) bitonic_width<8>(e0, e1, s_pairs);
    if constexpr (K0 <= 16) bitonic_width<16>(e0, e1, s_pairs);
    if constexpr (K0 <= 32) bitonic_width<32>(e0, e1, s_pairs);
    if constexpr (K0 <= 64) bitonic_width<64>(e0, e1, s_pairs);
    if constexpr (K0 <= 128) bitonic_width<128>(e0, e1, s_pairs);
    if constexpr (K0 <= 256) bitonic_width<256>(e0, e1, s_pairs);
    if constexpr (K0 <= 512) bitonic_width<512>(e0, e1, s_pairs);
    bitonic_width<1024>(e0, e1, s_pairs);
}
__device__ __forceinline__ int bitonic_src(int o)
{
    return o < kResortWindow / 2 ? o : (kResortWindow + kResortWindow / 2 - 1 - o);
}


template <typename KeyOf>
__device__ __forceinline__ void resort_sort_window(int window, int N, const uint32_t *__restrict__ prev_order, KeyOf key_of,
                                                   uint64_t *__restrict__ comp, ulonglong2 *s_pairs)
{
    const int pos0 = window * kResortWindow + 2 * (int)threadIdx.x;
    const uint32_t g0 = min(prev_order[min(pos0, N - 1)], (uint32_t)(N - 1));
    const uint32_t g1 = min(prev_order[min(pos0 + 1, N - 1)], (uint32_t)(N - 1));
    const uint32_t k0 = key_of(g0), k1 = key_of(g1);
    uint64_t e0 = pos0 < N ? (((uint64_t)k0 << 32) | g0) : ~0ull;
    uint64_t e1 = pos0 + 1 < N ? (((uint64_t)k1 << 32) | g1) : ~0ull;
    bitonic_pairs<2>(e0, e1, s_pairs);
    if (pos0 < N) comp[pos0] = e0;
    if (pos0 + 1 < N) comp[pos0 + 1] = e1;
}

}
```

### splat_loam_amd/csrc/sls_sort.hip

```cpp
#include <cstdlib>
#include "sls_common.hpp"
#include "sls_resort.hpp"
#include "sls_launch.hpp"

namespace sls {

#ifndef SLS_SORT_ROUNDS
#define SLS_SORT_ROUNDS 16
#endif
#ifndef SLS_SORT_WAVES
#define SLS_SORT_WAVES 8
#endif
constexpr int kSortRounds = SLS_SORT_ROUNDS;
constexpr int kSortWaveItems = kWave * kSortRounds;
constexpr int kSortMaxBins = 2048;
constexpr int kDepthKeyBits = 29;

__device__ __forceinline__ uint32_t load_count(const uint32_t *count_ptr, uint32_t cap)
{
    const uint32_t c = *count_ptr;
    return c < cap ? c : cap;
}

__device__ __forceinline__ void resort_verify(int nwin, const uint64_t *__restrict__ edges, uint32_t *__restrict__ flag);
// ... 1043 lines not shown
}

__global__ __launch_bounds__(256) void gather_scan_final_kernel(int N, const uint32_t *__restrict__ order,
                                                                const uint32_t *__restrict__ tiles,
                                                                const uint32_t *__restrict__ block_sums,
                                                                uint32_t *__restrict__ offsets,
                                                                uint32_t *__restrict__ total_out, int resort_windows,
                                                                const uint64_t *__restrict__ resort_edges,
                                                                uint32_t *__restrict__ fail_flag)
{
    __shared__ uint32_t s_wave[4];
    __shared__ uint32_t s_pre[4];
    if (resort_windows > 0 && blockIdx.x == 0) resort_verify(resort_windows, resort_edges, fail_flag);
    const int i = blockIdx.x * 256 + threadIdx.x;
    const int lane = threadIdx.x & 63, wave = threadIdx.x >> 6;
    uint32_t pre = 0;
    for (int b = threadIdx.x; b < (int)blockIdx.x; b += 256) pre += block_sums[b];
#pragma unroll
    for (int off = 32; off > 0; off >>= 1) pre += __shfl_xor(pre, off, 64);
    const uint32_t v = (i < N) ? tiles[order[i]] : 0u;
    uint32_t incl = v;
#pragma unroll
    for (int off = 1; off < 64; off <<= 1) {
        const uint32_t t = __shfl_up(incl, off, 64);
        if (lane >= off) incl += t;
    }
    if (lane == 63) s_wave[wave] = incl;
    if (lane == 0) s_pre[wave] = pre;
    __syncthreads();
    uint32_t wave_prefix = 0;
    for (int w = 0; w < wave; ++w) wave_prefix += s_wave[w];
    const uint32_t block_prefix = s_pre[0] + s_pre[1] + s_pre[2] + s_pre[3];
    if (i < N) offsets[i] = block_prefix + wave_prefix + incl;
    if (blockIdx.x == gridDim.x - 1 && threadIdx.x == 255) *total_out = block_prefix + wave_prefix + incl;
}

template <int EB>
__global__ __launch_bounds__(EB) void emit_tiles_kernel(int N, int GX, const uint32_t *__restrict__ order,
                                                         const int4 *__restrict__ rect,
                                                         const uint32_t *__restrict__ tiles,
                                                         const uint64_t *__restrict__ tile_mask,
                                                         const int4 *__restrict__ erec,
                                                         const uint32_t *__restrict__ offsets, uint32_t cap,
                                                         uint32_t *__restrict__ tkeys, uint32_t *__restrict__ vals,
                                                         uint32_t *__restrict__ overflow, int pack_shift,
                                                         ScanHandoff fused, uint32_t *__restrict__ total_out,
                                                         uint32_t *__restrict__ fail_flag,
                                                         uint32_t *__restrict__ hist_cnt, int hist_bins,
                                                         uint32_t *__restrict__ chunk_start,
                                                         const uint32_t *__restrict__ sbox, uint64_t *__restrict__ wide)
{
    __shared__ uint32_t s_hist[kSortMaxBins];
    if (hist_cnt) {
        for (int d = threadIdx.x; d < hist_bins; d += EB) s_hist[d] = 0u;
        __syncthreads();
    }
    constexpr int EW = EB / 64;
    const int i = blockIdx.x * EB + threadIdx.x;
    const uint32_t g = order[min(i, N - 1)];
    int4 rc;
    uint64_t mask;
    if (erec) {
        const int4 e = erec[g];
        rc = make_int4(e.x & 0xFFFF, e.y & 0xFFFF, (int)((uint32_t)e.x >> 16), (int)((uint32_t)e.y >> 16));
        mask = ((uint64_t)(uint32_t)e.w << 32) | (uint64_t)(uint32_t)e.z;
    } else {
        rc = rect[g];
        mask = (tile_mask && (uint32_t)(rc.y * rc.w) <= 64u) ? tile_mask[g] : ~0ull;
    }
    const uint64_t box_hi = wide ? ((uint64_t)sbox[g] << 32) : 0ull;
    const uint32_t nrect = (uint32_t)(rc.y * rc.w);
    if (nrect > 64u) mask = ~0ull;
    const uint32_t t = (i < N) ? (nrect <= 64u ? (uint32_t)__popcll(mask & (nrect >= 64u ? ~0ull : ((1ull << nrect) - 1ull))) : nrect) : 0u;
    uint32_t end;
    if (fused.block_sums) {
        __shared__ uint32_t s_wave[EW];
        __shared__ uint32_t s_pre[EW];
        if (fused.resort_windows > 0 && blockIdx.x == 0) resort_verify(fused.resort_windows, fused.resort_edges, fail_flag);
        const int lane = threadIdx.x & 63, wave = threadIdx.x >> 6;
        uint32_t pre = 0;
        for (int b = threadIdx.x; b < (int)blockIdx.x * (EB / 256); b += EB) pre += fused.block_sums[b];
#pragma unroll
        for (int off = 32; off > 0; off >>= 1) pre += __shfl_xor(pre, off, 64);
        uint32_t incl = t;
#pragma unroll
        for (int off = 1; off < 64; off <<= 1) {
            const uint32_t u = __shfl_up(incl, off, 64);
            if (lane >= off) incl += u;
        }
        if (lane == 63) s_wave[wave] = incl;
        if (lane == 0) s_pre[wave] = pre;
        __syncthreads();
        uint32_t wave_prefix = 0;
        for (int w = 0; w < wave; ++w) wave_prefix += s_wave[w];
        uint32_t block_prefix = 0;
#pragma unroll
        for (int w = 0; w < EW; ++w) block_prefix += s_pre[w];
        end = block_prefix + wave_prefix + incl;
        if (blockIdx.x == gridDim.x - 1 && threadIdx.x == EB - 1) *total_out = end;
    } else {
        end = (i < N) ? offsets[i] : 0u;
    }
    if (chunk_start && threadIdx.x == 0) {
        chunk_start[blockIdx.x] = end - t;
        if (blockIdx.x == gridDim.x - 1 && !fused.block_sums) chunk_start[gridDim.x] = offsets[N - 1];
    }
    if (chunk_start && fused.block_sums && blockIdx.x == gridDim.x - 1 && threadIdx.x == EB - 1) chunk_start[gridDim.x] = end;
    bool emit = i < N && t != 0u;
    uint32_t off = end - t;
    if (emit && end > cap) {
        if (overflow) atomicOr(overflow, 1u);
        if (off >= cap) emit = false;
    }
    if (emit) {
        uint32_t bit = 0;
        for (int y = 0; y < rc.w; ++y) {
            const uint32_t row = (uint32_t)(rc.z + y) * (uint32_t)GX;
            for (int k = 0; k < rc.y; ++k, ++bit) {
                if (bit < 64u && !((mask >> bit) & 1ull)) continue;
                int tx = rc.x + k;
                if (tx >= GX) tx -= GX;
                if (off < cap) {
                    const uint32_t tile = row + (uint32_t)tx;
                    if (wide) wide[off] = box_hi | (uint64_t)((tile << pack_shift) | g);
                    else if (vals) { tkeys[off] = tile; vals[off] = g; }
                    else tkeys[off] = (tile << pack_shift) | g;
                    if (hist_cnt) atomicAdd(&s_hist[tile], 1u);
                }
                ++off;
            }
        }
    }
    if (hist_cnt) {
        __syncthreads();
        for (int d = threadIdx.x; d < hist_bins; d += EB) hist_cnt[(size_t)d * gridDim.x + blockIdx.x] = s_hist[d];
    }
}

__global__ __launch_bounds__(256) void tile_ranges_kernel(const uint32_t *__restrict__ tkeys,
                                                          const uint32_t *__restrict__ vals,
                                                          const uint32_t *__restrict__ count_ptr, uint32_t cap,
                                                          const float *__restrict__ depth, uint2 *__restrict__ ranges,
                                                          uint64_t *__restrict__ keys64)
{
    const uint32_t R = load_count(count_ptr, cap);
    const uint32_t j = blockIdx.x * 256 + threadIdx.x;
    if (j >= R) return;
    const uint32_t t = tkeys[j];
    if (j == 0 || tkeys[j - 1] != t) ranges[t].x = j;
    if (j + 1 == R || tkeys[j + 1] != t) ranges[t].y = j + 1;
    if (keys64) keys64[j] = ((uint64_t)t << 32) | (uint64_t)__float_as_uint(depth[vals[j]]);
}

static int bits_for(uint32_t max_value)
{
    int b = 0;
    while (b < 32 && (max_value >> b) != 0) ++b;
    return b;
}

size_t order_scratch_bytes(int N)
{
    const size_t n = (size_t)(N > 0 ? N : 1);
    return sizeof(uint32_t) * (3 * n + (n + 255) / 256 + 64) + sort_scratch_bytes(n) + 16 + n / 32 + 128;
}

struct OrderScratch {
    uint32_t *keys, *keys_tmp, *vals_tmp, *block_sums, *n_dev;
    void *sort_scratch;
    uint64_t *comp;
    bool odd;
    OrderScratch(int N, void *scratch)
    {
        keys = (uint32_t *)scratch; keys_tmp = keys + N; vals_tmp = keys_tmp + N;
        block_sums = vals_tmp + N + 2;
        n_dev = block_sums + (N + 255) / 256;
        sort_scratch = (void *)(n_dev + 32);
        comp = (uint64_t *)(((uintptr_t)keys_tmp + 7) & ~(uintptr_t)7);
        odd = (sort_passes(kDepthKeyBits) & 1) != 0;
    }
};

void depth_order_key_buffers(int N, void *scratch, uint32_t *order, uint32_t **keys, uint32_t **vals0, uint32_t **n_dev)
{
    const OrderScratch s(N, scratch);
    *keys = s.keys;
    *vals0 = s.odd ? s.vals_tmp : order;
    *n_dev = s.n_dev;
}

uint64_t *resort_comp_buffer(int N, void *scratch) { return OrderScratch(N, scratch).comp; }

int launch_depth_order_scan(const DepthOrderScan &a, hipStream_t st, ScanHandoff *handoff)
{
    const int N = a.N, reuse_order = a.reuse_order;
    uint32_t *order = a.order;
    const DirectBin *direct = a.direct;
    if (a.scratch_bytes < order_scratch_bytes(N)) {
        set_error("depth-order scratch too small: %zu < %zu", a.scratch_bytes, order_scratch_bytes(N));
        return SLS_E_SCRATCH;
    }
    const int nb = (N + 255) / 256;
    const OrderScratch s(N, a.scratch);
    uint32_t *keys = s.keys, *block_sums = s.block_sums;
    uint32_t *v0 = s.odd ? s.vals_tmp : order, *v1 = s.odd ? order : s.vals_tmp;
    int resort_windows = 0;
    const uint64_t *resort_edges = nullptr;
    if (reuse_order && a.fail_flag) {
        uint64_t *comp = s.comp;
        uint64_t *edges = (uint64_t *)(((uintptr_t)s.sort_scratch + 7) & ~(uintptr_t)7);
        const int nA = (N + kResortWindow - 1) / kResortWindow;
        const int nB = (N + kResortWindow / 2 + kResortWindow - 1) / kResortWindow;
        ScopedTimer tm(T_RESORT, st);
        if (!a.window_sort_done) {
            hipLaunchKernelGGL(resort_sort_kernel, dim3(nA), dim3(kResortThreads), 0, st, N, (const uint32_t *)order,
                               (const uint32_t *)keys, comp);
            SLS_LAUNCH_CHECK("resort_sort_kernel");
        }
        const DirectBin no_db = { nullptr, nullptr, nullptr, 0, 0, 0 };
        const bool count_here = direct != nullptr && handoff != nullptr;
        uint64_t *comp2 = edges + 2 * (size_t)nB + 2;
#define SLS_MERGE(PRE_, last_, in_, out_)                                                                                    \
        do {                                                                                                                 \
            if (count_here && (last_))                                                                                       \
                hipLaunchKernelGGL((resort_merge_kernel<true, PRE_>), dim3(nB), dim3(kResortThreads), 0, st, N,               \
                                   (const uint64_t *)(in_), order, edges, a.tiles, block_sums, a.GX, (const uint2 *)a.erec_box,      \
                                   *direct, (uint64_t *)(out_));                                                              \
            else                                                                                                             \
                hipLaunchKernelGGL((resort_merge_kernel<false, PRE_>), dim3(nB), dim3(kResortThreads), 0, st, N,              \
                                   (const uint64_t *)(in_), order, edges, a.tiles, block_sums, a.GX, (const uint2 *)a.erec_box,      \
                                   no_db, (uint64_t *)(out_));                                                                \
        } while (0)
        SLS_MERGE(false, reuse_order <= 1, comp, reuse_order > 1 ? comp : nullptr);
        SLS_LAUNCH_CHECK("resort_merge_kernel");
        uint64_t *cin = comp, *cout = comp2;
        for (int round = 1; round < reuse_order; ++round) {
            const bool last = round + 1 == reuse_order;
            SLS_MERGE(true, last, cin, last ? nullptr : cout);
            SLS_LAUNCH_CHECK("resort_merge_kernel (further round)");
            uint64_t *t = cin; cin = cout; cout = t;
        }
#undef SLS_MERGE
        if (count_here) {
            if (direct->nchunks != nB || direct->pos0 != -kResortWindow / 2) {
                set_error("internal: the direct binning's chunks are not the repair's windows");
                return SLS_E_ARG;
            }
            handoff->counted = 1;
        }
        resort_windows = nB;
        resort_edges = edges;
    } else {
        int which = 0;
        int rc = radix_sort_pairs_t<uint32_t>(keys, v0, s.keys_tmp, v1, s.n_dev, (uint32_t)N, kDepthKeyBits, s.sort_scratch,
                                              sort_scratch_bytes((uint64_t)N), &which, st, nullptr, 0, true);
        if (rc) return rc;
        if ((which != 0) != s.odd) {
            set_error("internal: depth order ended in the wrong buffer");
            return SLS_E_ARG;
        }
    }
    if (handoff && direct && resort_windows == 0) {
        *handoff = ScanHandoff{ nullptr, 0, nullptr, 0 };
        return SLS_OK;
    }
    if (handoff && resort_windows > 0) {
        *handoff = ScanHandoff{ block_sums, resort_windows, resort_edges, handoff->counted };
        return SLS_OK;
    }
    ScopedTimer tm(T_SCAN, st);
    if (resort_windows == 0) {
        hipLaunchKernelGGL(gather_block_sums_kernel, dim3(nb), dim3(256), 0, st, N, (const uint32_t *)order, a.tiles,
                           block_sums);
        SLS_LAUNCH_CHECK("gather_block_sums_kernel");
    }
    if (handoff) {
        *handoff = ScanHandoff{ block_sums, 0, nullptr, handoff->counted };
        return SLS_OK;
    }
    hipLaunchKernelGGL(gather_scan_final_kernel, dim3(nb), dim3(256), 0, st, N, (const uint32_t *)order, a.tiles,
                       (const uint32_t *)block_sums, a.offsets, a.total_out, resort_windows, resort_edges, a.fail_flag);
    SLS_LAUNCH_CHECK("gather_scan_final_kernel");
    return SLS_OK;
}

int launch_bin_sort(const DevCam &cam, const BinSortLaunch &a, hipStream_t st, int *sorted_in_tmp, const uint2 **bmask_out)
{
    const int T = cam.GX * cam.GY, N = a.N;
    const uint32_t cap = a.cap;
    void *scratch = a.scratch;
    uint32_t *ranges = a.ranges, *tkeys = a.tkeys, *vals = a.vals, *tkeys_tmp = a.tkeys_tmp, *vals_tmp = a.vals_tmp;
    *sorted_in_tmp = 0;
    if (bmask_out) *bmask_out = nullptr;
    if (cap == 0 || N == 0) {
        SLS_HIP_CHECK(hipMemsetAsync(ranges, 0, sizeof(uint32_t) * 2 * (size_t)T, st));
        return SLS_OK;
    }
    if (a.scratch_bytes < sort_scratch_bytes(cap)) {
        set_error("sort scratch too small: %zu < %zu", a.scratch_bytes, sort_scratch_bytes(cap));
        return SLS_E_SCRATCH;
    }
    const int tile_bits = bits_for((uint32_t)(T - 1));
    const bool fused_ranges = sort_passes(tile_bits) == 1 && a.keys64_out == nullptr;
    if (!fused_ranges) SLS_HIP_CHECK(hipMemsetAsync(ranges, 0, sizeof(uint32_t) * 2 * (size_t)T, st));
    const int idx_bits = bits_for((uint32_t)(N - 1)) > 0 ? bits_for((uint32_t)(N - 1)) : 1;
    const bool packed = fused_ranges && tile_bits + idx_bits <= 32;
    const int bins = 1 << (tile_bits < 8 ? 8 : tile_bits);
    constexpr int eb = 256;
    const int nemit = (N + eb - 1) / eb;
    uint32_t *cnt = (uint32_t *)scratch, *totals = cnt + (size_t)bins * nemit, *chunk_start = totals + bins;
    const bool emit_hist = fused_ranges && (size_t)bins * nemit <= (size_t)400000 &&
                           ((size_t)bins * nemit + bins + nemit + 1) * sizeof(uint32_t) <= sort_core_bytes(cap);
    const bool long_lists = a.bmask_mode == 1 || (a.bmask_mode == 0 && (uint64_t)cap >= 1500ull * (uint64_t)T);
    BlockMaskArgs bm = { nullptr, cam.GX, 1.0f / (float)cam.GX, (cam.GX * kTileW) / 8 };
    uint64_t *wide = nullptr;
    if (a.sbox && bmask_out && packed && kTileW == 16 && kTileH == 16 && long_lists &&
        block_box_fits(cam.GX * kTileW, cam.H)) {
        bm.out = sort_bmask_buffer(scratch, cap);
        wide = sort_wide_buffer(scratch, cap);
        *bmask_out = bm.out;
    }
    {
        ScopedTimer tm(T_EMIT_KEYS, st);
        hipLaunchKernelGGL(emit_tiles_kernel<eb>, dim3(nemit), dim3(eb), 0, st, N, cam.GX, a.order, (const int4 *)a.rect, a.tiles,
                           a.tile_mask, (const int4 *)a.erec, a.offsets, cap, tkeys, packed ? (uint32_t *)nullptr : vals, a.overflow,
                           packed ? idx_bits : 0, a.handoff ? *a.handoff : ScanHandoff{ nullptr, 0, nullptr, 0 }, a.total_out,
                           a.overflow, emit_hist ? cnt : (uint32_t *)nullptr, bins, emit_hist ? chunk_start : (uint32_t *)nullptr,
                           a.sbox, wide);
    }
    SLS_LAUNCH_CHECK("emit_tiles_kernel");
    int which = 0;
    int rc;
    if (emit_hist) {
        const uint32_t *vin = packed ? nullptr : vals;
        const int shift = packed ? idx_bits : 0;
        const uint32_t pmask = packed ? ((1u << idx_bits) - 1u) : 0u;
#define SLS_CASE(K_, B) case B: rc = tile_sort_emit_chunks<K_, B>(wide ? (const K_ *)wide : (const K_ *)tkeys, vin, (K_ *)nullptr, vals_tmp, chunk_start, \
                                                              cap, shift, cnt, totals, nemit, (uint2 *)ranges, T, pmask, st, bm); break;
        if (wide) {
            switch (tile_bits < 8 ? 8 : tile_bits) { SLS_CASE(uint64_t, 8) SLS_CASE(uint64_t, 9) SLS_CASE(uint64_t, 10) default: SLS_CASE(uint64_t, 11) }
        } else {
            switch (tile_bits < 8 ? 8 : tile_bits) { SLS_CASE(uint32_t, 8) SLS_CASE(uint32_t, 9) SLS_CASE(uint32_t, 10) default: SLS_CASE(uint32_t, 11) }
        }
#undef SLS_CASE
        which = 1;
    } else if (wide) {
        rc = radix_sort_pairs_t<uint64_t>(wide, nullptr, nullptr, vals_tmp, a.count_ptr, cap, tile_bits, scratch,
                                          a.scratch_bytes, &which, st, (uint2 *)ranges, T, true, idx_bits, bm);
    } else if (packed) {
        rc = radix_sort_pairs_t<uint32_t>(tkeys, nullptr, tkeys_tmp, vals_tmp, a.count_ptr, cap, tile_bits, scratch,
                                          a.scratch_bytes, &which, st, (uint2 *)ranges, T, true, idx_bits);
    } else {
        rc = radix_sort_pairs_t<uint32_t>(tkeys, vals, tkeys_tmp, vals_tmp, a.count_ptr, cap, tile_bits, scratch,
                                          a.scratch_bytes, &which, st, fused_ranges ? (uint2 *)ranges : nullptr, T,
                                          fused_ranges);
    }
    if (rc) return rc;
    *sorted_in_tmp = which;
    if (!fused_ranges) {
        ScopedTimer tm(T_TILE_RANGES, st);
        hipLaunchKernelGGL(tile_ranges_kernel, dim3((cap + 255) / 256), dim3(256), 0, st,
                           (const uint32_t *)(which ? tkeys_tmp : tkeys), (const uint32_t *)(which ? vals_tmp : vals),
                           a.count_ptr, cap, a.depth, (uint2 *)ranges, a.keys64_out);
        SLS_LAUNCH_CHECK("tile_ranges_kernel");
    }
    return SLS_OK;
}


static int direct_bins(const DevCam &cam)
{
    const int tb = bits_for((uint32_t)(cam.GX * cam.GY - 1));
    return 1 << (tb < 8 ? 8 : tb);
}
static size_t direct_max_stride(int N)
{
    const size_t nchunks = (size_t)(N + kDirectChunk / 2 + kDirectChunk - 1) / kDirectChunk;
    return (nchunks + kDirectGroup - 1) / kDirectGroup * kDirectGroup;
}
bool bin_direct_possible(const DevCam &cam, int N, uint32_t cap)
{
    if (N <= 0 || cap == 0 || cam.tile_cull != 0 || cam.GX > 512 || cam.GY > 64) return false;
    if (cam.GX * cam.GY > kDirectMaxBins) return false;
    if (!block_box_fits(cam.GX * kTileW, cam.H)) return false;
    const size_t bins = (size_t)direct_bins(cam);
    return (bins * direct_max_stride(N) + bins + direct_coarse_words(cam, N)) * sizeof(uint32_t) <= sort_core_bytes(cap);
}
size_t direct_coarse_words(const DevCam &cam, int N)
{
    const size_t nchunks = (size_t)(N + kDirectChunk / 2 + kDirectChunk - 1) / kDirectChunk;
    return ((nchunks + kDirectGroup - 1) / kDirectGroup) * (size_t)direct_bins(cam);
}
DirectBin make_direct_bin(const DevCam &cam, int N, void *sort_scratch, uint2 *serec, bool repaired, bool coarse)
{
    DirectBin db;
    db.bins = direct_bins(cam);
    db.nchunks = repaired ? (N + kResortWindow / 2 + kResortWindow - 1) / kResortWindow : (N + kDirectChunk - 1) / kDirectChunk;
    db.pos0 = repaired ? -kResortWindow / 2 : 0;
    db.stride = coarse ? (db.nchunks + kDirectGroup - 1) / kDirectGroup * kDirectGroup : db.nchunks;
    db.cnt = (uint32_t *)sort_scratch;
    db.totals = db.cnt + (size_t)db.bins * db.stride;
    db.serec = serec;
    db.coarse = coarse ? (uint32_t *)sort_scratch + (size_t)db.bins * direct_max_stride(N) + db.bins : nullptr;
    return db;
// ... 43 lines not shown
```

### splat_loam_amd/engine.py

```python
from __future__ import annotations

import ctypes as C
import os
import weakref

import torch
import torch.distributed as dist

from . import _abi
from .fused import camera_aux
from .rasterizer import GaussianRasterizationSettings, get_camera


def carry_bucket(buf: torch.Tensor, keep: torch.Tensor, n_new: int) -> torch.Tensor:
    n_old = int(keep.numel())
    n_keep = int(keep.sum().item())
    if buf.numel() != 10 * n_old or n_new < n_keep:
        raise ValueError("bucket / mask / new size do not fit together")
    out = torch.zeros((10 * n_new,), dtype=buf.dtype, device=buf.device)
    src_off = dst_off = 0
    for width in (3, 1, 2, 4):
        src = buf[src_off:src_off + width * n_old].view(n_old, width)
        out[dst_off:dst_off + width * n_keep].view(n_keep, width).copy_(src[keep])
        src_off += width * n_old
        dst_off += width * n_new
    return out


def dp_chunk(N: int, G: int) -> int:
    return -(-(10 * N) // (4 * G)) * 4


def dp_pieces(N: int, lo: int, hi: int, lrs):
    out = []
    for g0, g1, lr in ((0, 3 * N, lrs[0]), (3 * N, 4 * N, lrs[1]), (4 * N, 6 * N, lrs[2]), (6 * N, 10 * N, lrs[3])):
        a, b = max(lo, g0), min(hi, g1)
        if b > a:
            out.append((a, b, lr))
    return out


def dp_chunked(flat: torch.Tensor, C: int, G: int) -> torch.Tensor:
    out = torch.zeros((G, C + 4), dtype=flat.dtype, device=flat.device)
    pad = torch.zeros((G * C,), dtype=flat.dtype, device=flat.device)
    pad[:flat.numel()] = flat
    out[:, :C] = pad.view(G, C)
    return out.reshape(-1)


class MappingEngine:
    def __init__(self, model, cfg, lrs=(5e-4, 5e-2, 5e-3, 1e-3), betas=(0.9, 0.999), eps=1e-15,
                 capacity_factor: float = 1.3):
        self.model, self.cfg = model, cfg
        self.lrs, self.betas, self.eps = tuple(lrs), tuple(betas), float(eps)
        self.capacity_factor = float(capacity_factor)
        p = model._xyz
        if not p.is_cuda:
            raise RuntimeError("MappingEngine needs ROCm device parameters; there is no CPU fallback")
        self.dev = p.device
        self.N = int(p.shape[0])
        n10 = 10 * self.N
        self.grads = torch.zeros((n10 + 2,), dtype=torch.float32, device=self.dev)
        self.exp_avg = torch.zeros((n10,), dtype=torch.float32, device=self.dev)
        self.exp_avg_sq = torch.zeros((n10,), dtype=torch.float32, device=self.dev)
        self.status = torch.zeros((8,), dtype=torch.int32, device=self.dev)
        self.t = 0
        self.capacity = 0
        self.workspace = None
        self.allmap_ptr = C.c_void_p(0)
        self.last = None
        self._lag_dev = torch.zeros((2, 8), dtype=torch.int32, device=self.dev)
        self._lag_host = torch.zeros((2, 8), dtype=torch.int32).pin_memory()
        self._lag_ev = [torch.cuda.Event(), torch.cuda.Event()]
        self._lag_np = self._lag_host.numpy()
        self.status_poll = True
        self._lag_polled = [False, False]
        self._group = None
        self._lag_ready = []
        self.flushed = []
        self._lag_pending = None
        self.reuse_depth_order = True
        self.inline_loss_stage = True
        self.repair_span = 256
        self._repair_rounds, self._repair_until = 1, 0
        self.keep_grads = False
        self._ws_ready = False
        self._ws_hw = None
        self._ws_det = None
        self.status_mirror = True
        self._orders = {}
        self._set_order_ages()
        self.max_cached_orders = 64
        self.stats = {"repeated_too_small": 0, "repeated_resort": 0, "repeated_exchange": 0, "repeated_det": 0}
        self._enq = 0
        self.dp_mode = os.environ.get("SLS_DP_MODE", "rs_ag")
        self._dp = None
        self._dp_agreed, self._dp_use_rs, self._dp_scheme = None, False, 0
        from .rasterizer import deterministic_mode
        self.deterministic = 2 if os.environ.get("SLS_DETERMINISTIC", "0") == "2" else deterministic_mode()
        self._det_prev = {}
        self._det_two_pass_next = True
        self.block_masks = int(os.environ.get("SLS_BLOCK_MASKS", "0"))
        self._sx = None
        self.exchanged_bytes = 0
        self.exchange_at_world_1 = False
        self.comm_events = None
        self._last_call = None
        self.pose_grad = None
        self._pose_buf = torch.zeros((_abi.SLS_MAX_BATCH, 6), dtype=torch.float32, device=self.dev)
        self._pose_scratch = None

    def grad_views(self):
        N = self.N
        g = self.grads
        if self._dp is not None:
            C, G = self._dp["C"], self._dp["G"]
            g = g.view(G, C + 4)[:, :C].reshape(-1)[:10 * N].clone()
        return {"xyz": g[0:3 * N].view(N, 3), "opacity": g[3 * N:4 * N].view(N, 1),
                "scaling": g[4 * N:6 * N].view(N, 2), "rotation": g[6 * N:10 * N].view(N, 4)}

    def _ensure_workspace(self, H, W, capacity):
        lib = _abi.lib()
        if (self.workspace is None or capacity > self.capacity or (H, W) != self._ws_hw
                or self._ws_det != bool(self.deterministic) or self.N > getattr(self, "_ws_n", 0)):
            self._ws_det = bool(self.deterministic)
            self.capacity, self._ws_hw = int(max(capacity, self.capacity)), (H, W)
            wcfg = _abi.SlsMappingConfig()
            wcfg.deterministic = 1 if self.deterministic else 0
            self._ws_n = self.N + (self.N // 4 if getattr(self, "_bucket_store", None) is not None else 0)
            nbytes = int(lib.sls_mapping_workspace_bytes_cfg(self._ws_n, H, W, self.capacity, C.byref(wcfg)))
            self.workspace = None
            self.workspace = torch.empty((nbytes + 256,), dtype=torch.uint8, device=self.dev)
            self._ws_ready = False
        base = self.workspace.data_ptr()
        return (base + 255) & ~255, self.workspace.numel() - 256

    def _config(self, apply_adam, with_regulariser, reuse_order=False):
        c, cfg = _abi.SlsMappingConfig(), self.cfg
        c.reuse_depth_order = int(reuse_order)
        c.keep_grads = 1 if self.keep_grads else 0
        c.workspace_ready = 1 if self._ws_ready else 0
        self._ws_ready = True
        c.lambda_alpha, c.lambda_normal = cfg.opt_lambda_alpha, cfg.opt_lambda_normal
        c.scaling_max = cfg.opt_scaling_max
        c.scaling_max_penalty = cfg.opt_scaling_max_penalty if with_regulariser else 0.0
        c.depth_ratio = cfg.depth_ratio
        c.lr_xyz, c.lr_opacity, c.lr_scaling, c.lr_rotation = self.lrs
        c.apply_adam = 1 if apply_adam else 0
        c.beta1, c.beta2, c.eps = self.betas[0], self.betas[1], self.eps
        if self._dp is not None and not apply_adam:
            c.grad_chunk, c.grad_ranks = self._dp["C"], self._dp["G"]
        c.deterministic = 1 if self.deterministic else 0
        c.block_masks = int(self.block_masks)
        if self._sx is not None and not apply_adam:
            c.grad_bitmap = self._sx["mine"].data_ptr()
        return c

    def _order_entry(self, camera):
        ent = self._orders.get(id(camera))
        return ent if ent is not None and ent[2]() is camera else None

    def _forget_order(self, camera, failed_repair=False):
        ent = self._order_entry(camera)
        if ent is not None:
            ent[1] = None
        if failed_repair:
            self._repair_rounds = min(self._repair_rounds + 1, 3)
            self._repair_until = self._enq + self.repair_span

    def _set_order_ages(self):
        scale = min(max(500000.0 / max(self.N, 1), 1.0), 3.0)
        self.max_order_age = int(4 * scale)
        self.order_age_round3 = int(12 * scale)
        self.max_order_age_extra = int(48 * scale)
        self.order_age_round4 = 1000000

    def _order_for(self, camera, allow_reuse, H, W, advance=True):
        lib = _abi.lib()
        ent = self._order_entry(camera)
        if ent is None:
            stale = [k for k, e in self._orders.items() if e[2]() is None]
            for k in stale:
                del self._orders[k]
            if len(self._orders) >= self.max_cached_orders:
                self._orders.pop(next(iter(self._orders)))
            ent = [torch.empty((self.N,), dtype=torch.int32, device=self.dev), None, weakref.ref(camera),
                   torch.zeros((int(lib.sls_block_order_bytes(H, W)) // 4,), dtype=torch.int32, device=self.dev)]
            self._orders[id(camera)] = ent
        age = self._enq - ent[1] if ent[1] is not None else None
        reuse = allow_reuse and self.reuse_depth_order and age is not None and age <= self.max_order_age_extra
        if self._repair_rounds > 1 and self._enq >= self._repair_until:
            self._repair_rounds -= 1
            self._repair_until = self._enq + self.repair_span
        reuse = min(self._repair_rounds + (1 if age is not None and age > self.max_order_age else 0)
                    + (1 if age is not None and age > self.order_age_round3 else 0)
                    + (1 if age is not None and age > self.order_age_round4 else 0), 4) if reuse else 0
        if advance:
            self._enq += 1
            ent[1] = self._enq
        return ent, reuse

    def _det_prev_for(self, camera):
        dent = self._det_prev.get(id(camera))
        first_visit = dent is None or dent[1]() is not camera
        if first_visit:
            for k in [k for k, e in self._det_prev.items() if e[1]() is None]:
                del self._det_prev[k]
            while len(self._det_prev) >= self.max_cached_orders:
                self._det_prev.pop(next(iter(self._det_prev)))
            dent = [torch.zeros((self.N, 16), dtype=torch.uint8, device=self.dev), weakref.ref(camera)]
            self._det_prev[id(camera)] = dent
        return dent, first_visit

    def _pose_args(self, cfg, slots):
        need = int(_abi.lib().sls_pose_grad_scratch_bytes(self.N)) * int(slots)
        if self._pose_scratch is None or self._pose_scratch.numel() < need:
            self._pose_scratch = torch.zeros((need,), dtype=torch.uint8, device=self.dev)
        cfg.pose_scratch, cfg.pose_scratch_bytes = self._pose_scratch.data_ptr(), int(self._pose_scratch.numel())

    def _params(self):
        m = self.model
        ps = (m._xyz, m._scaling, m._rotation, m._opacity)
        for p in ps:
            if p.dtype != torch.float32 or not p.is_contiguous() or p.shape[0] != self.N:
                raise RuntimeError("model parameters must stay contiguous float32 of the engine's size")
        return ps

    def _enqueue(self, camera, apply_adam, with_regulariser, status=None, mirror=None, allow_reuse=True, phase=0,
                 pose_grad=False):
        lib = _abi.lib()
        H, W = int(camera.image_height), int(camera.image_width)
        settings = GaussianRasterizationSettings(H, W, 1.0, camera.world_view_transform, camera.projection_matrix)
        ce = get_camera(settings, self.dev)
        aux = camera_aux(camera)
        if self.capacity == 0:
            self.capacity = max(4 * self.N, 1 << 16)
        ws_ptr, ws_bytes = self._ensure_workspace(H, W, self.capacity)
        xyz, scaling, rotation, opacity = self._params()
        ent, reuse = self._order_for(camera, allow_reuse, H, W)
        cfg = self._config(apply_adam, with_regulariser, reuse)
        if self.deterministic == 2:
            dent, first_visit = self._det_prev_for(camera)
            cfg.det_prev = dent[0].data_ptr()
            cfg.deterministic = 1 if (self._det_two_pass_next or first_visit or not cfg.workspace_ready) else 2
            self._det_two_pass_next = False
        cfg.depth_order = ent[0].data_ptr()
        cfg.block_order = ent[3].data_ptr() if self.inline_loss_stage else None
        cfg.status_mirror = mirror
        cfg.void_flags_out = None if (apply_adam or self._dp is not None) else self.grads.data_ptr() + 4 * 10 * self.N
        cfg.phase = int(phase)
        if pose_grad:
            cfg.pose_grad = self._pose_buf.data_ptr()
            self._pose_args(cfg, 1)
        args = (C.byref(ce.cam), self.N, xyz.data_ptr(), scaling.data_ptr(), rotation.data_ptr(), opacity.data_ptr(),
                self.grads.data_ptr(), self.exp_avg.data_ptr(), self.exp_avg_sq.data_ptr(), self.t + 1,
                aux.gt.data_ptr(), aux.valid.data_ptr(), aux.n_valid, ce.col_cs.data_ptr(), ce.row_cs.data_ptr(),
                aux.col_h.data_ptr(), aux.row_h.data_ptr(), C.byref(cfg), self.capacity, ws_ptr, ws_bytes,
                (self.status if status is None else status).data_ptr(), C.byref(self.allmap_ptr),
                torch.cuda.current_stream(self.dev).cuda_stream)
        self._last_call = (args, cfg) if phase == 1 else None
        _abi.check(lib.sls_mapping_step(*args), "sls_mapping_step")

    @staticmethod
    def _void_reason(st):
        if st["too_small"]:
            return "repeated_too_small"
        if st["resort_failed"]:
            return "repeated_resort"
        return "repeated_det" if st.get("det_mispredicted") else "repeated_exchange"

    def _sharded(self, group):
        if not dist.is_initialized():
            return False
        return dist.get_world_size(group) > 1 or self.exchange_at_world_1

    def _read_status(self):
        return self._note(self._parse_status(self.status.cpu()))

    def _note(self, st):
        if st["overflow"] and self.deterministic == 2:
            self._det_two_pass_next = True
        if st.get("outside_union"):
            raise RuntimeError("a surfel outside the agreed union of the touched sets had a non-zero gradient: the early "
                               "gradient bitmap was no superset (sparse exchange) — the iteration's update is void")
        if st.get("handover_mismatch"):
            raise RuntimeError("the tile backward found a forward -> backward hand-over buffer that is not this forward's "
                               "(its tag word does not match): the iteration's gradients are void")
        if self._sx is not None and (not st["overflow"] or st["exchange_too_small"]):
            want = int(st["exchange_count"] * 1.5) + 4096
            self._sx["send"] = int(min(self.N, max(want, int(self._sx["send"] * 0.97))))
        return st

    @staticmethod
    def _parse_status(h):
        R, flags = int(h[0].item()) & 0xFFFFFFFF, int(h[1].item())
        f = h.view(torch.float32)
        return {"R": R, "overflow": bool(flags), "too_small": bool(flags & 1), "resort_failed": bool(flags & 2),
                "exchange_too_small": bool(flags & 4), "det_mispredicted": bool(flags & 8),
                "handover_mismatch": bool(flags & 16), "outside_union": bool(flags & 32),
                "exchange_count": int(h[7].item()) & 0xFFFFFFFF,
                "loss_pixel": float(f[5]), "loss_reg": float(f[6]),
                "loss": float(f[5]) + float(f[6]), "sums": [float(f[2]), float(f[3]), float(f[4])]}

    @staticmethod
    def _parse_status_np(h):
        import numpy as np
        f = h.view(np.float32)
        R, flags = int(h[0]) & 0xFFFFFFFF, int(h[1])
        return {"R": R, "overflow": bool(flags), "too_small": bool(flags & 1), "resort_failed": bool(flags & 2),
                "exchange_too_small": bool(flags & 4), "det_mispredicted": bool(flags & 8),
                "handover_mismatch": bool(flags & 16), "outside_union": bool(flags & 32),
                "exchange_count": int(h[7]) & 0xFFFFFFFF,
                "loss_pixel": float(f[5]), "loss_reg": float(f[6]),
                "loss": float(f[5]) + float(f[6]), "sums": [float(f[2]), float(f[3]), float(f[4])]}

    @torch.no_grad()
    def step(self, camera, group=None, sync: bool = True, pose_grad: bool = False):
        sharded = self._sharded(group)
        if pose_grad:
            if sync is not True:
                raise ValueError("pose_grad needs sync=True: the gradient belongs to the iteration whose status is returned")
            if sharded:
                raise NotImplementedError("pose_grad is served on the single-process path only")
        if self._dp is not None and not sharded:
            raise RuntimeError("this engine's optimiser state is sharded over a process group (dp_mode rs_ag): "
                               "it cannot take a single-process step")
        self._group = group
        if sync == "lagged":
            return self._step_lagged(camera)
        if self._lag_pending is not None:
            self.flush()
        reuse_ok = sync is not False
        while True:
            if not sharded:
                self._enqueue(camera, apply_adam=True, with_regulariser=True, allow_reuse=reuse_ok, pose_grad=pose_grad)
            else:
                rank = dist.get_rank(group)
                self._ensure_dp(group)
                self._enqueue(camera, apply_adam=False, with_regulariser=(rank == 0), allow_reuse=reuse_ok,
                              phase=self._phase_for_exchange())
                self._exchange_and_adam(group, self.status, None)
            if not sync:
                self.t += 1
                return None
            st = self._read_status()
            if not st["overflow"]:
                self.t += 1
                self.last = st
                self.pose_grad = self._pose_buf[0] if pose_grad else None
                return st
            if st["too_small"] or st["resort_failed"]:
                self._forget_order(camera, failed_repair=st["resort_failed"])
            self.stats[self._void_reason(st)] += 1
            if st["too_small"]:
                need = st["R"]
                if sharded:
                    t = torch.tensor([need], dtype=torch.int64, device=self.dev)
                    dist.all_reduce(t, op=dist.ReduceOp.MAX, group=group)
                    need = int(t.item())
                self.capacity = int(max(need, self.capacity) * self.capacity_factor) + 1024
                self.workspace = None

    @torch.no_grad()
    def pose_step(self, camera):
        if self._dp is not None or self._sx is not None:
            raise RuntimeError("this engine's gradient bucket is laid out for a keyframe-parallel exchange: pose_step "
                               "needs the single-process engine")
        if self._lag_pending is not None:
            self.flush()
        while True:
            self._enqueue(camera, apply_adam=False, with_regulariser=False, pose_grad=True)
            st = self._read_status()
            if not st["overflow"]:
                self.pose_grad = self._pose_buf[0]
                return st
            if st["too_small"] or st["resort_failed"]:
                self._forget_order(camera, failed_repair=st["resort_failed"])
            self.stats[self._void_reason(st)] += 1
            if st["too_small"]:
                self.capacity = int(max(st["R"], self.capacity) * self.capacity_factor) + 1024
                self.workspace = None

    def _ensure_batch_workspace(self, G, H, W, capacity):
        lib = _abi.lib()
        b = getattr(self, "_bws", None)
        det = bool(self.deterministic)
        if b is None or G > b["G"] or capacity != b["cap"] or (H, W) != b["hw"] or det != b["det"] or self.N != b["n"]:
            wcfg = _abi.SlsMappingConfig()
            wcfg.deterministic = 1 if det else 0
            Gw = max(G, b["G"] if b is not None and (H, W) == b["hw"] else 1)
            nbytes = int(lib.sls_mapping_workspace_bytes_batch(Gw, self.N, H, W, capacity, C.byref(wcfg)))
            self._bws = None
            b = self._bws = {"G": Gw, "cap": int(capacity), "hw": (H, W), "det": det, "n": self.N, "ready": 0,
                             "buf": torch.empty((nbytes + 256,), dtype=torch.uint8, device=self.dev),
                             "status": torch.zeros((_abi.SLS_MAX_BATCH + 1, 8), dtype=torch.int32, device=self.dev)}
        base = b["buf"].data_ptr()
        return b, (base + 255) & ~255, b["buf"].numel() - 256

    def _enqueue_batch(self, cameras, apply_adam, with_regulariser, allow_reuse=True, pose_grad=False):
        lib = _abi.lib()
        G = len(cameras)
        H, W = int(cameras[0].image_height), int(cameras[0].image_width)
        if self.capacity == 0:
            self.capacity = max(4 * self.N, 1 << 16)
        b, ws_ptr, ws_bytes = self._ensure_batch_workspace(G, H, W, self.capacity)
        xyz, scaling, rotation, opacity = self._params()
        kfs = (_abi.SlsKeyframeInputs * G)()
        keep = []
        reuse_used, ents = [], []
        for g, camera in enumerate(cameras):
            settings = GaussianRasterizationSettings(H, W, 1.0, camera.world_view_transform, camera.projection_matrix)
            ce = get_camera(settings, self.dev)
            aux = camera_aux(camera)
            ent, reuse = self._order_for(camera, allow_reuse, H, W, advance=False)
            ents.append(ent)
            k = kfs[g]
            k.cam = ce.cam
            k.gt_depth, k.valid, k.n_valid = aux.gt.data_ptr(), aux.valid.data_ptr(), aux.n_valid
            k.reuse_depth_order = int(reuse)
            k.col_cs, k.row_cs = ce.col_cs.data_ptr(), ce.row_cs.data_ptr()
            k.col_cs_half, k.row_cs_half = aux.col_h.data_ptr(), aux.row_h.data_ptr()
            k.depth_order = ent[0].data_ptr()
            k.block_order = ent[3].data_ptr() if self.inline_loss_stage else None
            k.det_prev = self._det_prev_for(camera)[0][0].data_ptr() if self.deterministic == 2 else None
            k.pose_grad = self._pose_buf[g].data_ptr() if pose_grad else None
            keep.append((ce, aux))
            reuse_used.append(int(reuse))
        self._enq += 1
        for ent in ents:
            ent[1] = self._enq
        ready = self._ws_ready
        cfg = self._config(apply_adam, with_regulariser)
        self._ws_ready = ready
        cfg.workspace_ready = 1 if G <= b["ready"] else 0
        b["ready"] = max(b["ready"], G)
        cfg.void_flags_out = None if apply_adam else self.grads.data_ptr() + 4 * 10 * self.N
        if pose_grad:
            self._pose_args(cfg, G)
        self.last_batch_reuse = reuse_used
        _abi.check(lib.sls_mapping_step_batch(G, kfs, self.N, xyz.data_ptr(), scaling.data_ptr(), rotation.data_ptr(),
                                              opacity.data_ptr(), self.grads.data_ptr(), self.exp_avg.data_ptr(),
                                              self.exp_avg_sq.data_ptr(), self.t + 1, C.byref(cfg), b["cap"],
                                              ws_ptr, ws_bytes, b["status"].data_ptr(),
                                              torch.cuda.current_stream(self.dev).cuda_stream),
                   "sls_mapping_step_batch")
        return b["status"]

    @torch.no_grad()
    def step_batch(self, cameras, group=None, sync: bool = True, pose_grad: bool = False):
        cams = list(cameras)
        if pose_grad and sync is not True:
            raise ValueError("pose_grad needs sync=True: the gradients belong to the iteration whose status is returned")
        if pose_grad and self._sharded(group):
            raise NotImplementedError("pose_grad is served on the single-process path only")
        if sync == "lagged":
            raise ValueError("step_batch has no lagged mode")
        if not 1 <= len(cams) <= _abi.SLS_MAX_BATCH:
            raise ValueError(f"a batch holds 1 to {_abi.SLS_MAX_BATCH} keyframes, not {len(cams)}")
        if len({id(c) for c in cams}) != len(cams):
            raise ValueError("a keyframe appears twice in the batch")
        if len({(int(c.image_height), int(c.image_width)) for c in cams}) != 1:
            raise ValueError("the keyframes of a batch must share one image size")
        sharded = self._sharded(group)
        if sharded and self.dp_mode != "allreduce":
            raise NotImplementedError(f"step_batch over a process group needs dp_mode 'allreduce', not {self.dp_mode!r}")
        if self._dp is not None or self._sx is not None:
            raise RuntimeError("this engine's optimiser state is laid out for another exchange: step_batch cannot use it")
        self._group = group
        if self._lag_pending is not None:
            self.flush()
        reuse_ok = sync is not False
        while True:
            if not sharded:
                status = self._enqueue_batch(cams, apply_adam=True, with_regulariser=True, allow_reuse=reuse_ok,
                                             pose_grad=pose_grad)
            else:
                self._ensure_dp(group)
                status = self._enqueue_batch(cams, apply_adam=False, with_regulariser=(dist.get_rank(group) == 0),
                                             allow_reuse=reuse_ok)
                self._exchange_and_adam(group, status[0], None)
            if not sync:
                self.t += 1
                return None
            h = status[:len(cams) + 1].cpu()
            st = self._note(self._parse_status(h[0]))
            st["keyframes"] = [self._parse_status(h[1 + g]) for g in range(len(cams))]
            if not st["overflow"]:
                self.t += 1
                self.last = st
                self.pose_grad = self._pose_buf[:len(cams)] if pose_grad else None
                return st
            for cam, kst in zip(cams, st["keyframes"]):
                if kst["too_small"] or kst["resort_failed"]:
                    self._forget_order(cam, failed_repair=kst["resort_failed"])
            self.stats[self._void_reason(st)] += 1
            if st["too_small"]:
                need = st["R"]
                if sharded:
                    t = torch.tensor([need], dtype=torch.int64, device=self.dev)
                    dist.all_reduce(t, op=dist.ReduceOp.MAX, group=group)
                    need = int(t.item())
                self.capacity = int(max(need, self.capacity) * self.capacity_factor) + 1024
                self.workspace = None
                self._bws = None

    def _step_lagged(self, camera):
        slot = 0 if self._lag_pending is None else self._lag_pending[0] ^ 1
        group = self._group
        polled = False
        if self._sharded(group):
            self._ensure_dp(group)
            self._enqueue(camera, apply_adam=False, with_regulariser=(dist.get_rank(group) == 0),
                          status=self._lag_dev[slot], phase=self._phase_for_exchange())
            self._exchange_and_adam(group, self._lag_dev[slot],
                                    self._lag_host[slot].data_ptr() if self.status_mirror else None)
            if not self.status_mirror:
                self._lag_host[slot].copy_(self._lag_dev[slot], non_blocking=True)
        elif self.status_mirror:
            polled = self.status_poll
            if polled:
                self._lag_np[slot, 0] = -1
                self._lag_np[slot, 7] = -1
            self._enqueue(camera, apply_adam=True, with_regulariser=True, status=self._lag_dev[slot],
                          mirror=self._lag_host[slot].data_ptr())
        else:
            self._enqueue(camera, apply_adam=True, with_regulariser=True, status=self._lag_dev[slot])
            self._lag_host[slot].copy_(self._lag_dev[slot], non_blocking=True)
        self.t += 1
        self._lag_polled[slot] = polled
        if not polled:
            self._lag_ev[slot].record(torch.cuda.current_stream(self.dev))
        prev, self._lag_pending = self._lag_pending, (slot, camera)
        if prev is not None:
            self._lag_collect(prev, redo_current=True)
        return self._lag_ready.pop(0) if self._lag_ready else None

    def _lag_collect(self, prev, redo_current):
        pslot, pcam = prev
        if self._lag_polled[pslot]:
            row, spins = self._lag_np[pslot], 0
            while row[7] == -1 or row[0] == -1:
                spins += 1
                if spins > 2_000_000:
                    torch.cuda.current_stream(self.dev).synchronize()
                    if row[7] == -1 or row[0] == -1:
                        raise RuntimeError("the mapping iteration's status never reached its host mirror")
            st = self._note(self._parse_status_np(row.copy()))
        else:
            self._lag_ev[pslot].synchronize()
            st = self._note(self._parse_status(self._lag_host[pslot].clone()))
        if not st["overflow"]:
            self.last = st
            self._lag_ready.append(st)
            return st
        cur, self._lag_pending = self._lag_pending, None
        torch.cuda.current_stream(self.dev).synchronize()
        cur_st = self._note(self._parse_status(self._lag_dev[cur[0]].cpu())) if cur is not None else None
        cur_void = cur_st is not None and cur_st["overflow"]
        self.t -= 2 if cur is not None else 1
        if st["too_small"] or st["resort_failed"]:
            self._forget_order(pcam, failed_repair=st["resort_failed"])
        if cur_void and (cur_st["too_small"] or cur_st["resort_failed"]):
            self._forget_order(cur[1], failed_repair=cur_st["resort_failed"])
        self.stats[self._void_reason(st)] += 1
        if st["too_small"] or (cur_void and cur_st["too_small"]):
            need = max(st["R"], cur_st["R"] if cur_void else 0, self.capacity)
            self.capacity = int(need * self.capacity_factor) + 1024
            self.workspace = None
        if cur_st is not None and not cur_void:
            self._lag_ready.append(cur_st)
        st = self.step(pcam, group=self._group, sync=True)
        self._lag_ready.append(st)
        if cur is not None and not cur_void:
            self.t += 1
        if cur_void:
            if redo_current:
                self._redo_pending(cur[1])
            else:
                self._lag_ready.append(self.step(cur[1], group=self._group, sync=True))
        return st

    def _redo_pending(self, camera):
        ready, self._lag_ready = self._lag_ready, []
        self._step_lagged(camera)
        self._lag_ready = ready + self._lag_ready

    def flush(self):
        if self._lag_pending is not None:
            prev, self._lag_pending = self._lag_pending, None
            self._lag_collect(prev, redo_current=False)
        self.flushed, self._lag_ready = self._lag_ready, []
        return self.flushed[-1] if self.flushed else None

    def _ensure_dp(self, group):
        if self.dp_mode not in ("rs_ag", "allreduce", "sparse"):
            raise ValueError(f"dp_mode must be 'rs_ag', 'allreduce' or 'sparse', not {self.dp_mode!r}")
        G, rank, N = dist.get_world_size(group), dist.get_rank(group), self.N
        if self._dp is not None:
            if self._dp["G"] != G or self._dp["rank"] != rank:
                raise RuntimeError("the process group changed under an engine whose optimiser state is sharded "
                                   f"({self._dp['G']} ranks -> {G}): build a new engine (or remap(reset_state=True))")
            return
        if self._dp_agreed != (G, rank):
            want = (2 if N % 2 == 0 else 0) if self.dp_mode == "sparse" else (1 if (self.dp_mode == "rs_ag" and N % 2 == 0 and 10 * N < 2 ** 32) else 0)
            t = torch.tensor([want, -want], dtype=torch.int32, device=self.dev)
            dist.all_reduce(t, op=dist.ReduceOp.MIN, group=group)
            lo, hi = int(t[0].item()), -int(t[1].item())
            if hi == 2 and lo != 2:
                raise RuntimeError("keyframe-parallel ranks disagree on the gradient exchange: some ask for dp_mode "
                                   "'sparse', others for a dense scheme (check SLS_DP_MODE on every rank)")
            self._dp_use_rs = lo == 1
            self._dp_agreed = (G, rank)
            self._dp_scheme = lo
        if self._dp_scheme == 2:
            if self._sx is not None and (self._sx["G"], self._sx["rank"]) != (G, rank):
                raise RuntimeError("the process group changed under an engine set up for the sparse exchange "
                                   f"({self._sx['G']} ranks -> {G}): build a new engine (or remap())")
            if self._sx is None:
                lib = _abi.lib()
                nw = int(lib.sls_grad_bitmap_words(N))
                self._sx = {"bitmap": torch.zeros((nw,), dtype=torch.int64, device=self.dev),
                            "mine": torch.zeros((nw,), dtype=torch.int64, device=self.dev),
                            "all": torch.zeros((G * nw,), dtype=torch.int64, device=self.dev),
                            "prefix": torch.zeros((nw,), dtype=torch.int32, device=self.dev),
                            "compact": torch.zeros((10 * N,), dtype=torch.float32, device=self.dev),
                            "index": torch.zeros((N,), dtype=torch.int32, device=self.dev),
                            "send": N,
                            "G": G, "rank": rank}
            return
        if not self._dp_use_rs:
            return
        C = dp_chunk(N, G)
        flat = torch.zeros((G * C,), dtype=torch.float32, device=self.dev)
        m = self.model
        for p, off, w in ((m._xyz, 0, 3), (m._opacity, 3 * N, 1), (m._scaling, 4 * N, 2), (m._rotation, 6 * N, 4)):
            view = flat[off:off + w * N].view(N, w)
            view.copy_(p.data)
            p.data = view
        lo, hi = min(rank * C, 10 * N), min((rank + 1) * C, 10 * N)
        ea, es = torch.zeros((C,), dtype=torch.float32, device=self.dev), torch.zeros((C,), dtype=torch.float32, device=self.dev)
        ea[:hi - lo].copy_(self.exp_avg[lo:hi])
        es[:hi - lo].copy_(self.exp_avg_sq[lo:hi])
        self.exp_avg, self.exp_avg_sq = ea, es
        self.grads = torch.zeros((G * (C + 4),), dtype=torch.float32, device=self.dev)
        self._dp = {"G": G, "rank": rank, "C": C, "flat": flat, "lo": lo, "hi": hi,
                    "gshard": torch.zeros((C + 4,), dtype=torch.float32, device=self.dev)}

    def _phase_for_exchange(self):
        return 1 if self._sx is not None else 0

    def _exchange_and_adam(self, group, status, mirror):
        ev = None
        if self.comm_events is not None:
            ev = [torch.cuda.Event(enable_timing=True) for _ in range(4)]
            ev[0].record()
        if self._sx is not None:
            lib, sx, N = _abi.lib(), self._sx, self.N
            st = torch.cuda.current_stream(self.dev).cuda_stream
            dist.all_gather_into_tensor(sx["all"], sx["mine"], group=group)
            G = int(sx["all"].numel() // sx["mine"].numel())
            send = int(sx["send"])
            _abi.check(lib.sls_grad_union(N, sx["all"].data_ptr(), G, sx["bitmap"].data_ptr(), send, sx["prefix"].data_ptr(),
                                          status.data_ptr(), st), "sls_grad_union")
            args, cfg = self._last_call
            cfg.phase, cfg.workspace_ready, cfg.apply_adam, cfg.keep_grads = 2, 1, 1, 0
            cfg.union_bitmap, cfg.union_prefix = sx["bitmap"].data_ptr(), sx["prefix"].data_ptr()
            cfg.grad_compact, cfg.grad_compact_index, cfg.grad_compact_capacity = sx["compact"].data_ptr(), sx["index"].data_ptr(), send
            _abi.check(lib.sls_mapping_step(*args), "sls_mapping_step (phase 2)")
            dist.all_reduce(sx["compact"][:10 * send], op=dist.ReduceOp.SUM, group=group)
            if ev:
                ev[1].record()
            xyz, scaling, rotation, opacity = self._params()
            _abi.check(lib.sls_adam_step_union(N, xyz.data_ptr(), opacity.data_ptr(), scaling.data_ptr(), rotation.data_ptr(),
                                               sx["index"].data_ptr(), sx["compact"].data_ptr(), send, self.exp_avg.data_ptr(),
                                               self.exp_avg_sq.data_ptr(), self.lrs[0], self.lrs[1], self.lrs[2], self.lrs[3],
                                               self.betas[0], self.betas[1], self.eps, self.t + 1, status.data_ptr(), mirror,
                                               st), "sls_adam_step_union")
            if ev:
                ev[2].record(); ev[3].record()
            self.exchanged_bytes = 8 * int(sx["mine"].numel()) + 40 * send
        elif self._dp is None:
            dist.all_reduce(self.grads, op=dist.ReduceOp.SUM, group=group)
            if ev:
                ev[1].record()
            self._adam_reduced(status, mirror)
            if ev:
                ev[2].record(); ev[3].record()
            self.exchanged_bytes = 4 * int(self.grads.numel())
        else:
            d = self._dp
            dist.reduce_scatter_tensor(d["gshard"], self.grads, op=dist.ReduceOp.SUM, group=group)
            if ev:
                ev[1].record()
            self._adam_shard(status, mirror)
            if ev:
                ev[2].record()
            C, r = d["C"], d["rank"]
            mine = d["flat"][r * C:(r + 1) * C]
            if d.get("ag_in_place", True):
                try:
                    dist.all_gather_into_tensor(d["flat"], mine, group=group)
                except (RuntimeError, ValueError):
                    d["ag_in_place"] = False
            if not d.get("ag_in_place", True):
                dist.all_gather_into_tensor(d["flat"], mine.clone(), group=group)
            if ev:
                ev[3].record()
            self.exchanged_bytes = 4 * int(self.grads.numel()) + 4 * C
        if ev:
            self.comm_events.append(ev)

    def _adam_shard(self, status, mirror):
        lib, d, N = _abi.lib(), self._dp, self.N
        lo, hi, C = d["lo"], d["hi"], d["C"]
        arr = (_abi.SlsAdamGroup * 4)()
        k = 0
# ... 105 lines not shown
```

### splat_loam_amd/rasterizer.py

```python
from __future__ import annotations

import ctypes as C
import os
from collections import OrderedDict
from typing import NamedTuple, Optional

import torch
from torch import nn

from . import _abi


class GaussianRasterizationSettings(NamedTuple):
    image_height: int
    image_width: int
    scale_modifier: float
    viewmatrix: torch.Tensor
    projmatrix: torch.Tensor
    prefiltered: bool = False
    debug: bool = False
    pix_offset: Optional[tuple] = None
    tile_cull_min: Optional[int] = None
    lean_allmap: Optional[bool] = None

# ... 167 lines not shown
        raise ValueError("expected means3D (N,3), scales (N,2), rotations (N,4), opacities (N,1)")
    ce = get_camera(settings, dev)
    cam = ce.cam
    H, W = cam.H, cam.W
    tw, th = _abi.tile_size()
    T = ((W + tw - 1) // tw) * ((H + th - 1) // th)
    st = _stream(dev)
    debug = bool(settings.debug)

    def dbg():
        if debug:
            torch.cuda.synchronize(dev)

    s = ForwardState()
    s.cam, s.N, s.a2, s.keys, s._views = ce, N, None, None, {}
    sb = int(lib.sls_stage1_scratch_bytes(N))
    radii = s._views["radii"] = torch.empty((N,), dtype=torch.int32, device=dev)
    a1 = s.a1 = _Arena(dev, (("rec", "f32", (N, lib.sls_rec_stride())), ("rect", "i32", (N, 4)),
                             ("tiles", "i32", (N,)), ("tmask", "i64", (N,)),
                             ("sbox", "i32", (N,)),
                             ("depth", "f32", (N,)), ("order", "i32", (N,)), ("offsets", "i32", (N,)),
                             ("total", "i32", (4,)), ("scratch1", "u8", (max(sb, 4),))))
    _abi.check(lib.sls_forward_stage1(C.byref(cam), N, means3D.data_ptr(), scales.data_ptr(), rotations.data_ptr(),
                                      opacities.data_ptr(), ce.col_cs.data_ptr(), ce.row_cs.data_ptr(),
                                      a1.ptr("rec"), radii.data_ptr(), a1.ptr("rect"), a1.ptr("tiles"), a1.ptr("tmask"),
                                      a1.ptr("sbox"), a1.ptr("depth"), a1.ptr("order"), a1.ptr("offsets"),
                                      a1.ptr("total"), a1.ptr("scratch1"), sb, st), "sls_forward_stage1")
    dbg()
    R = int(a1.view("total")[0].item()) & 0xFFFFFFFF
    s.R = R
    Ra = max(R, 1)
    ssb = int(lib.sls_sort_scratch_bytes(R))
    hand_over = True
    allmap = s._views["allmap"] = torch.empty((7, H, W), dtype=torch.float32, device=dev)
    spec2 = [("ranges", "i32", (T, 2)), ("pix_state", "f32", (H * W, 4)),
             ("pix_contrib", "i32", (H * W, 2)), ("tile_consumed", "i32", (T,)),
             ("keys_a", "i32", (Ra,)), ("keys_b", "i32", (Ra,)), ("vals_a", "i32", (Ra,)), ("vals_b", "i32", (Ra,)),
             ("sort_scratch", "u8", (max(ssb, 4),))]
    if hand_over:
        spec2.append(("block_masks", "i64", (int(lib.sls_block_mask_bytes(R, H, W)) // 8,)))
    a2 = s.a2 = _Arena(dev, spec2)
    in_tmp, stride, shape = C.c_int(0), C.c_int(1), C.c_int(0)
    lst = C.c_void_p(0)
    _abi.check(lib.sls_forward_stage2(C.byref(cam), N, R, a1.ptr("rec"), a1.ptr("rect"), a1.ptr("tiles"),
                                      a1.ptr("tmask"), a1.ptr("sbox"), a1.ptr("depth"), a1.ptr("order"),
                                      a1.ptr("offsets"), a1.ptr("total"),
                                      a2.ptr("keys_a"), a2.ptr("vals_a"), a2.ptr("keys_b"), a2.ptr("vals_b"),
                                      a2.ptr("sort_scratch"), ssb, C.byref(in_tmp), None,
                                      list_pairs_mode() if list_pairs is None else int(list_pairs),
                                      C.byref(lst), C.byref(stride), a2.ptr("ranges"),
                                      ce.col_cs.data_ptr(), ce.row_cs.data_ptr(), allmap.data_ptr(), a2.ptr("pix_state"),
                                      a2.ptr("pix_contrib"), a2.ptr("tile_consumed"),
                                      a2.ptr("block_masks") if hand_over else None, C.byref(shape), st),
               "sls_forward_stage2")
    dbg()
    s.vals_stride, s.block_masks_shape = int(stride.value), int(shape.value)
    s.vals_ptr = int(lst.value) if R > 0 else a2.ptr("vals_a")
    s._vals = None
    if want_keys:
        _list_and_keys(s, T)
    return s


def sorted_list(s: ForwardState) -> torch.Tensor:
    if s._vals is None:
        Ra = max(s.R, 1)
        off = s.vals_ptr - s.a2.base.data_ptr()
        v = s.a2.base[off:off + 4 * s.vals_stride * Ra].view(torch.int32).view(Ra, s.vals_stride)[:, 0]
        s._vals = v[:0] if s.R == 0 else v
    return s._vals


def _list_and_keys(s: ForwardState, T: int) -> None:
    vals = sorted_list(s)
    dev = vals.device
    cnt = (s.ranges[:, 1].long() - s.ranges[:, 0].long()) & 0xFFFFFFFF
    tile = torch.repeat_interleave(torch.arange(T, device=dev, dtype=torch.int64), cnt)
    bits = s.depth.view(torch.int32)[vals.long()].long() & 0xFFFFFFFF
    s.keys = (tile << 32) | bits


def deterministic_mode() -> bool:
    return os.environ.get("SLS_DETERMINISTIC", "0") in ("1", "2")


_POSE_SCRATCH: "OrderedDict[tuple, torch.Tensor]" = OrderedDict()


def pose_scratch(dev, N: int, slots: int = 1) -> torch.Tensor:
    key = (str(dev), _stream(dev), int(N), int(slots))
    buf = _POSE_SCRATCH.get(key)
    if buf is None:
        nbytes = int(_abi.lib().sls_pose_grad_scratch_bytes(int(N))) * int(slots)
        buf = _POSE_SCRATCH[key] = torch.zeros((max(nbytes, 8),), dtype=torch.uint8, device=dev)
        while len(_POSE_SCRATCH) > 8:
            _POSE_SCRATCH.popitem(last=False)
    else:
        _POSE_SCRATCH.move_to_end(key)
    return buf


def check_pose_delta(pose_delta, dev) -> None:
    if not isinstance(pose_delta, torch.Tensor):
        raise TypeError("pose_delta must be a torch.Tensor")
    if tuple(pose_delta.shape) != (6,):
        raise ValueError(f"pose_delta must have shape (6,) [v | w], got {tuple(pose_delta.shape)}")
    if pose_delta.dtype != torch.float32:
        raise ValueError(f"pose_delta must be float32, got {pose_delta.dtype}")
    if pose_delta.device != dev:
        raise ValueError(f"pose_delta is on {pose_delta.device}, the surfels on {dev}")


def rasterize_backward(state: ForwardState, means3D, scales, rotations, dL_dallmap, deterministic=None, pose_grad=None):
    lib = _abi.lib()
    dev = means3D.device
    N = state.N
    dL = _f32c(dL_dallmap)
    ps = pose_scratch(dev, N) if pose_grad is not None else None
    pose_args = (pose_grad.data_ptr(), ps.data_ptr(), ps.numel()) if pose_grad is not None else (None, None, 0)
    det = deterministic_mode() if deterministic is None else deterministic
    nbytes = int(lib.sls_backward_det_scratch_bytes(N)) if det else 0
    out = _Arena(dev, (("dmeans", "f32", (N, 3)), ("dscales", "f32", (N, 2)), ("drots", "f32", (N, 4)), ("dopac", "f32", (N, 1)))
                 + ((("scratch", "u8", (nbytes,)),) if det else (("grec", "f32", (N, lib.sls_grec_stride())),)))
    ce, a1, a2 = state.cam, state.a1, state.a2
    bm = a2.ptr("block_masks") if "block_masks" in a2.spec else None
    if det:
        _abi.check(lib.sls_backward_det_pose(C.byref(ce.cam), N, state.R, means3D.data_ptr(), scales.data_ptr(),
                                             rotations.data_ptr(), state.radii.data_ptr(), a1.ptr("rec"),
                                             a2.ptr("ranges"), state.vals_ptr, state.vals_stride, ce.col_cs.data_ptr(),
                                             ce.row_cs.data_ptr(), a2.ptr("pix_state"), a2.ptr("pix_contrib"),
                                             dL.data_ptr(), out.ptr("dmeans"), out.ptr("dscales"), out.ptr("drots"),
                                             out.ptr("dopac"), bm, state.block_masks_shape,
                                             out.ptr("scratch"), nbytes, *pose_args, _stream(dev)), "sls_backward_det")
        return out.view("dmeans"), out.view("dscales"), out.view("drots"), out.view("dopac"), None
    _abi.check(lib.sls_backward_pose(C.byref(ce.cam), N, state.R, means3D.data_ptr(), scales.data_ptr(),
                                     rotations.data_ptr(), state.radii.data_ptr(), a1.ptr("rec"),
                                     a2.ptr("ranges"), state.vals_ptr, state.vals_stride, ce.col_cs.data_ptr(),
                                     ce.row_cs.data_ptr(), a2.ptr("pix_state"), a2.ptr("pix_contrib"),
                                     dL.data_ptr(), out.ptr("grec"), out.ptr("dmeans"), out.ptr("dscales"),
                                     out.ptr("drots"), out.ptr("dopac"), bm,
                                     state.block_masks_shape, *pose_args, _stream(dev)),
               "sls_backward")
    return out.view("dmeans"), out.view("dscales"), out.view("drots"), out.view("dopac"), out.view("grec")


class _WsEntry:
    __slots__ = ("ws", "ws_ptr", "ws_bytes", "cap", "ready", "busy", "status", "mirror", "mirror_np", "orders", "calls",
                 "rounds", "rounds_until", "stats", "stream", "cap_hint")


_WS_CACHE: "OrderedDict[tuple, _WsEntry]" = OrderedDict()
_WS_CACHE_MAX = 4
_WS_ORDERS_MAX = 64
_SENTINEL = -1


def workspace_path_enabled() -> bool:
    return os.environ.get("SLS_STAGED_FORWARD", "0") != "1"


def _ws_entry(dev, N, H, W, lean) -> _WsEntry:
    key = (str(dev), N, H, W, bool(lean))
    e = _WS_CACHE.get(key)
    if e is not None:
        _WS_CACHE.move_to_end(key)
        return e
    e = _WsEntry()
    e.ws, e.cap, e.ready, e.busy = None, 0, False, False
    e.status = torch.zeros((8,), dtype=torch.int32, device=dev)
    e.mirror = torch.zeros((8,), dtype=torch.int32).pin_memory()
    e.mirror_np = e.mirror.numpy()
    e.orders, e.calls, e.rounds, e.rounds_until = OrderedDict(), 0, 1, 0
    e.stats = {"too_small": 0, "repair_failed": 0, "from_scratch": 0, "repaired": 0}
    e.stream, e.cap_hint = None, 0
    for old in [k for k, v in _WS_CACHE.items() if k[0] == key[0] and k[2:] == key[2:] and k[1] != N]:
        seen = _WS_CACHE[old].stats.get("R")
        if seen:
            e.cap_hint = max(e.cap_hint, int(1.3 * seen * N / max(old[1], 1)) + 1024)
        if not _WS_CACHE[old].busy:
            del _WS_CACHE[old]
    _WS_CACHE[key] = e
    while len(_WS_CACHE) > _WS_CACHE_MAX:
        _WS_CACHE.popitem(last=False)
    return e


_WARNED = set()


def _warn_once(key, text) -> None:
    if key not in _WARNED:
        _WARNED.add(key)
        import warnings
        warnings.warn(text, RuntimeWarning, stacklevel=3)


def _ws_alloc(e: _WsEntry, dev, N, H, W, cap) -> None:
    nbytes = int(_abi.lib().sls_forward_ws_bytes(N, H, W, cap))
    e.ws = None
    e.ws = torch.empty((nbytes + 256,), dtype=torch.uint8, device=dev)
    e.ws_ptr = (e.ws.data_ptr() + 255) & ~255
    e.ws_bytes, e.cap, e.ready = nbytes, int(cap), False


class WsState:
    __slots__ = ("cam", "entry", "N", "R", "cap", "radii", "allmap", "list_ptr", "stride", "shape", "ws", "ws_ptr", "ws_bytes",
                 "block_order")


def rasterize_forward_ws(settings: GaussianRasterizationSettings, means3D, opacities, scales, rotations,
                         keep_for_backward: bool = True) -> Optional[WsState]:
    lib = _abi.lib()
    dev = means3D.device
    N = int(means3D.shape[0])
    if N == 0:
        return None
    ce = get_camera(settings, dev)
    cam = ce.cam
    H, W = cam.H, cam.W
    tw, th = _abi.tile_size()
    T = ((W + tw - 1) // tw) * ((H + th - 1) // th)
    if T > 512 or cam.tile_cull_min >= 2:
        return None
    e = _ws_entry(dev, N, H, W, bool(cam.flags & 1))
    st = _stream(dev)
    if e.busy:
        _warn_once("busy", "GaussianRasterizer: the workspace of this (N, H, W) is held by an earlier forward whose "
                           "backward has not run; this call takes the staged path (slower).  Drop or backward() the "
                           "earlier result to get the one-call path back.")
        return None
    if e.stream is not None and e.stream != st:
        _warn_once("stream", "GaussianRasterizer: called on another stream than the one its workspace belongs to; this "
                             "call takes the staged path.")
        return None
    e.stream = st
    if e.ws is None:
        _ws_alloc(e, dev, N, H, W, max(4 * N, 1 << 16, e.cap_hint))
    okey = id(ce)
    ent = e.orders.get(okey)
    if ent is None or ent[2] is not ce:
        ent = [torch.empty((N,), dtype=torch.int32, device=dev), None, ce,
               torch.zeros((int(lib.sls_block_order_bytes(H, W)) // 4,), dtype=torch.int32, device=dev)]
        e.orders[okey] = ent
        while len(e.orders) > _WS_ORDERS_MAX:
            e.orders.popitem(last=False)
    else:
        e.orders.move_to_end(okey)
    scale = min(max(500000.0 / N, 1.0), 3.0)
    age = None if ent[1] is None else e.calls - ent[1]
    if e.rounds > 1 and e.calls >= e.rounds_until:
        e.rounds, e.rounds_until = e.rounds - 1, e.calls + 256
    reuse = 0
    if age is not None and age <= int(48 * scale):
        reuse = min(e.rounds + (1 if age > int(4 * scale) else 0) + (1 if age > int(12 * scale) else 0), 4)
    radii = torch.empty((N,), dtype=torch.int32, device=dev)
    allmap = torch.empty((7, H, W), dtype=torch.float32, device=dev)
    lst, stride, shape = C.c_void_p(0), C.c_int(1), C.c_int(0)
    row = e.mirror_np
    while True:
        row[0] = _SENTINEL
        row[7] = _SENTINEL
        rc = lib.sls_forward_ws(C.byref(cam), N, means3D.data_ptr(), scales.data_ptr(), rotations.data_ptr(),
                                opacities.data_ptr(), ce.col_cs.data_ptr(), ce.row_cs.data_ptr(), e.cap,
                                ent[0].data_ptr(), reuse, list_pairs_mode(), 1 if e.ready else 0,
                                1 if keep_for_backward else 0, radii.data_ptr(),
                                allmap.data_ptr(), e.ws_ptr, e.ws_bytes, e.status.data_ptr(), e.mirror.data_ptr(),
                                C.byref(lst), C.byref(stride), C.byref(shape), st)
        if rc == -4:
            return None
        _abi.check(rc, "sls_forward_ws")
        e.ready = True
        _abi.check(lib.sls_wait_status_mirror(e.mirror.data_ptr(), 0xFFFFFFFF, st), "sls_wait_status_mirror")
        R, flags = int(row[0]) & 0xFFFFFFFF, int(row[1])
        if flags == 0:
            break
        if flags & 1:
            e.stats["too_small"] += 1
            _ws_alloc(e, dev, N, H, W, int(R * 1.3) + 1024)
        if flags & 2:
            e.stats["repair_failed"] += 1
            e.rounds, e.rounds_until = min(e.rounds + 1, 3), e.calls + 256
        reuse = 0
    e.stats["repaired" if reuse else "from_scratch"] += 1
    e.stats["R"] = R
    e.calls += 1
    ent[1] = e.calls
    if settings.debug:
        torch.cuda.synchronize(dev)
        final = e.status.cpu().numpy()
        if (int(final[0]) & 0xFFFFFFFF) != R or int(final[1]) != 0:
            raise RuntimeError(f"sls_forward_ws: the status block changed after its early mirror (R {R} -> "
                               f"{int(final[0]) & 0xFFFFFFFF}, flags 0 -> {int(final[1])})")
    s = WsState()
    s.cam, s.entry, s.N, s.R, s.cap, s.radii, s.allmap = ce, e, N, R, e.cap, radii, allmap
    s.list_ptr, s.stride, s.shape = int(lst.value), int(stride.value), int(shape.value)
    s.ws, s.ws_ptr, s.ws_bytes, s.block_order = e.ws, e.ws_ptr, e.ws_bytes, ent[3]
    if keep_for_backward:
        e.busy = True
    return s


def rasterize_backward_ws(state: WsState, means3D, scales, rotations, dL_dallmap, pose_grad=None):
    lib = _abi.lib()
    dev = means3D.device
    N, ce = state.N, state.cam
    dL = _f32c(dL_dallmap)
    ps = pose_scratch(dev, N) if pose_grad is not None else None
    pose_args = (pose_grad.data_ptr(), ps.data_ptr(), ps.numel()) if pose_grad is not None else (None, None, 0)
    out = _Arena(dev, (("dmeans", "f32", (N, 3)), ("dscales", "f32", (N, 2)), ("drots", "f32", (N, 4)), ("dopac", "f32", (N, 1))))
    try:
        _abi.check(lib.sls_backward_ws_pose(C.byref(ce.cam), N, means3D.data_ptr(), scales.data_ptr(), rotations.data_ptr(),
                                            state.radii.data_ptr(), ce.col_cs.data_ptr(), ce.row_cs.data_ptr(), dL.data_ptr(),
                                            state.cap, state.ws_ptr, state.ws_bytes, state.list_ptr, state.stride, state.shape,
                                            state.block_order.data_ptr(), out.ptr("dmeans"), out.ptr("dscales"), out.ptr("drots"), out.ptr("dopac"),
                                            *pose_args, _stream(dev)), "sls_backward_ws")
    except Exception:
        state.entry.ready = False
        raise
    return out.view("dmeans"), out.view("dscales"), out.view("drots"), out.view("dopac")


class _WsLease:
    __slots__ = ("state",)

    def __init__(self, state):
        self.state = state

    def release(self):
        st, self.state = self.state, None
        if st is not None and st.entry.ws is st.ws:
            st.entry.busy = False

    def __del__(self):
        self.release()


def frame_from_precomp(cov3D_precomp: torch.Tensor):
    t = cov3D_precomp
    if t.dim() != 3 or tuple(t.shape[1:]) not in ((4, 4), (3, 3)):
        raise ValueError(f"cov3D_precomp must be (N,4,4) or (N,3,3), got {tuple(t.shape)}")
    rs_t = t[:, :3, :3].to(torch.float32)
    su, sv = rs_t[:, 0].norm(dim=1), rs_t[:, 1].norm(dim=1)
    tu = rs_t[:, 0] / su.clamp_min(1e-30)[:, None]
    tv = rs_t[:, 1] / sv.clamp_min(1e-30)[:, None]
    tn = torch.cross(tu, tv, dim=1)
    R = torch.stack([tu, tv, tn], dim=2)
    m00, m11, m22 = R[:, 0, 0], R[:, 1, 1], R[:, 2, 2]
    q_abs = torch.sqrt(torch.clamp(torch.stack([1 + m00 + m11 + m22, 1 + m00 - m11 - m22,
                                                1 - m00 + m11 - m22, 1 - m00 - m11 + m22], dim=1), min=0.0))
    cand = torch.stack([
        torch.stack([q_abs[:, 0] ** 2, R[:, 2, 1] - R[:, 1, 2], R[:, 0, 2] - R[:, 2, 0], R[:, 1, 0] - R[:, 0, 1]], dim=1),
        torch.stack([R[:, 2, 1] - R[:, 1, 2], q_abs[:, 1] ** 2, R[:, 1, 0] + R[:, 0, 1], R[:, 0, 2] + R[:, 2, 0]], dim=1),
        torch.stack([R[:, 0, 2] - R[:, 2, 0], R[:, 1, 0] + R[:, 0, 1], q_abs[:, 2] ** 2, R[:, 2, 1] + R[:, 1, 2]], dim=1),
        torch.stack([R[:, 1, 0] - R[:, 0, 1], R[:, 2, 0] + R[:, 0, 2], R[:, 2, 1] + R[:, 1, 2], q_abs[:, 3] ** 2], dim=1),
    ], dim=1)
    best = q_abs.argmax(dim=1)
    q = cand[torch.arange(R.shape[0], device=R.device), best]
    q = q / (2.0 * q_abs.gather(1, best[:, None]).clamp_min(1e-12))
    q = torch.nn.functional.normalize(q, dim=1)
    return torch.stack([su, sv], dim=1).contiguous(), q.contiguous()


_AUTOGRAD_POLICY_DONE = False


def _autograd_policy() -> None:
    global _AUTOGRAD_POLICY_DONE
    if _AUTOGRAD_POLICY_DONE:
        return
    _AUTOGRAD_POLICY_DONE = True
    want = os.environ.get("SLS_AUTOGRAD_SINGLE_THREAD", "")
    if want == "1" or (want == "" and torch.cuda.device_count() == 1):
        torch.autograd.set_multithreading_enabled(False)


class _RasterizeGaussians(torch.autograd.Function):
    @staticmethod
    def forward(ctx, means3D, means2D, opacities, scales, rotations, cov3D_precomp, raster_settings, pose_delta=None):
        if scales is None or rotations is None:
            raise ValueError("scales and rotations are required")
        if pose_delta is not None:
            check_pose_delta(pose_delta, means3D.device)
        m, o, s_, r = map(_f32c, (means3D.detach(), opacities.detach(), scales.detach(), rotations.detach()))
        for name, t in (("means3D", m), ("opacities", o), ("scales", s_), ("rotations", r)):
            _need_cuda(t, name)
        if m.shape != (m.shape[0], 3) or s_.shape != (m.shape[0], 2) or r.shape != (m.shape[0], 4) or o.numel() != m.shape[0]:
            raise ValueError("expected means3D (N,3), scales (N,2), rotations (N,4), opacities (N,1)")
        ctx.want_pose = pose_delta is not None and ctx.needs_input_grad[7]
        needs_grad = any(ctx.needs_input_grad[:5]) or ctx.want_pose
        if needs_grad:
            _autograd_policy()
        ctx.debug = bool(raster_settings.debug)
        ctx.lease = None
        st = None
        if workspace_path_enabled() and not (needs_grad and deterministic_mode()):
            st = rasterize_forward_ws(raster_settings, m, o, s_, r, keep_for_backward=needs_grad)
            if st is not None and needs_grad:
                ctx.lease = _WsLease(st)
        if st is None:
            st = rasterize_forward(raster_settings, m, o, s_, r)
        ctx.state = st
        ctx.settings = raster_settings
        ctx.save_for_backward(m, s_, r, o)
        ctx.mark_non_differentiable(st.radii)
        return st.radii, st.allmap

    @staticmethod
    def backward(ctx, _grad_radii, grad_allmap):
        m, s_, r, o = ctx.saved_tensors
        st = ctx.state
        if grad_allmap is None:
            grad_allmap = torch.zeros_like(st.allmap)
        if isinstance(st, WsState) and (ctx.lease is None or ctx.lease.state is None):
            st = ctx.state = rasterize_forward(ctx.settings, m, o, s_, r)
        pose = torch.empty((6,), dtype=torch.float32, device=m.device) if ctx.want_pose else None
        if isinstance(st, WsState):
            try:
                dmeans, dscales, drots, dopac = rasterize_backward_ws(st, m, s_, r, grad_allmap, pose_grad=pose)
            finally:
                ctx.lease.release()
        else:
            dmeans, dscales, drots, dopac, _ = rasterize_backward(st, m, s_, r, grad_allmap, pose_grad=pose)
        if ctx.debug:
            torch.cuda.synchronize(m.device)
        return dmeans, None, dopac, dscales, drots, None, None, pose


_PENDING_HOOKS: dict = {}


class GaussianRasterizer(nn.Module):
    def __init__(self, raster_settings: GaussianRasterizationSettings):
        super().__init__()
        self.raster_settings = raster_settings
        for hook in list(_PENDING_HOOKS.values()):
            hook()
# ... 21 lines not shown
```

Measured before the change: 1850 Msplats/s.

## Rebuild from-scratch depth order with bucket scatter and per-run bitonic sort

When no previous depth order can be repaired, the depth order is built by a three-kernel bucket sort instead of the full radix sort. The kernels build a histogram over the top key bits, scatter (key,index) pairs into buckets, then bitonic-sort each run of up to 2048 elements in shared memory. It aims to replace the multi-pass radix sort on 500k keys with fewer global passes. If a run exceeds 2048 elements a new failure flag is set, the iteration is voided and the caller falls back to the radix path (reuse=-1).

Result: no change. 1868 Msplats/s (median of 4 runs) (+0.9%).

```diff
diff --git a/splat_loam_amd/csrc/sls_launch.hpp b/splat_loam_amd/csrc/sls_launch.hpp
--- a/splat_loam_amd/csrc/sls_launch.hpp
+++ b/splat_loam_amd/csrc/sls_launch.hpp
@@ -34,6 +34,8 @@
                          int *result_in_tmp, hipStream_t st);
 void depth_order_key_buffers(int N, void *scratch, uint32_t *order, uint32_t **keys, uint32_t **vals0, uint32_t **n_dev);
 uint64_t *resort_comp_buffer(int N, void *scratch);
+constexpr int kOrderRebuildWords = 2 * 16384;
+uint32_t *order_rebuild_tables(int N, void *scratch);
 bool bin_direct_possible(const DevCam &cam, int N, uint32_t cap);
 DirectBin make_direct_bin(const DevCam &cam, int N, void *sort_scratch, uint2 *serec, bool repaired, bool coarse);
 size_t direct_coarse_words(const DevCam &cam, int N);
@@ -43,6 +45,7 @@
     void *scratch; size_t scratch_bytes;
     int reuse_order;
     uint32_t *fail_flag;
+    bool bucket_rebuild;
     bool window_sort_done;
     const DirectBin *direct;
     const int4 *erec_box; int GX;
@@ -84,6 +87,7 @@
     const uint32_t *resort_prev_order; uint64_t *resort_comp;
     uint32_t *sbox;
     uint32_t *zero_words; int n_zero_words;
+    uint32_t *zero_words2; int n_zero_words2;
 };
 int launch_preprocess_fwd(const DevCam &cam, const PreFwdLaunch &a, hipStream_t st);
 
diff --git a/splat_loam_amd/csrc/sls_pipeline.hip b/splat_loam_amd/csrc/sls_pipeline.hip
--- a/splat_loam_amd/csrc/sls_pipeline.hip
+++ b/splat_loam_amd/csrc/sls_pipeline.hip
@@ -377,6 +377,7 @@
     const bool direct = bin_direct_possible(dc, N, cap);
     BinDirectLaunch bd{};
     if (direct) bd.db = make_direct_bin(dc, N, w.sort_scratch, (uint2 *)w.serec, merged_sort, true);
+    const bool bucket_rebuild = direct && f.reuse_rounds == 0;
     PreFwdLaunch pf = f.pf;
     pf.rec = w.rec; pf.order_vals = ovals; pf.n_dev = n_dev;
     pf.status_clear = (uint32_t *)status_dev; pf.tile_mask = w.tmask; pf.erec = w.erec;
@@ -385,6 +386,7 @@
         pf.order_keys = merged_sort ? nullptr : okeys;
         pf.erec_box = 1;
         if (bd.db.coarse) { pf.zero_words = bd.db.coarse; pf.n_zero_words = (int)direct_coarse_words(dc, N); }
+        if (bucket_rebuild) { pf.zero_words2 = order_rebuild_tables(N, w.order_scratch); pf.n_zero_words2 = kOrderRebuildWords; }
     } else {
         pf.rect = w.rect; pf.tiles = w.tiles; pf.depth = w.depth; pf.order_keys = okeys; pf.sbox = w.sbox;
     }
@@ -393,7 +395,8 @@
     DepthOrderScan ds{};
     ds.N = N; ds.tiles = w.tiles; ds.order = order; ds.offsets = w.offsets; ds.total_out = &status_dev->R;
     ds.scratch = w.order_scratch; ds.scratch_bytes = w.order_scratch_bytes;
-    ds.reuse_order = f.reuse_rounds; ds.fail_flag = &status_dev->overflow; ds.window_sort_done = merged_sort;
+    ds.reuse_order = f.reuse_rounds > 0 ? f.reuse_rounds : 0; ds.fail_flag = &status_dev->overflow; ds.window_sort_done = merged_sort;
+    ds.bucket_rebuild = bucket_rebuild;
     ds.direct = direct ? &bd.db : nullptr; ds.erec_box = (const int4 *)w.erec; ds.GX = dc.GX;
     if (int rc = launch_depth_order_scan(ds, st, &handoff)) return rc;
     int in_tmp = 0, rc;
@@ -443,8 +446,8 @@
     SLS_REQUIRE(means3D && scales && rotations && opacities && col_cs && row_cs && radii && allmap, "null pointer");
     SLS_REQUIRE(R_capacity > 0 && R_capacity < (1ull << 32), "bad instance capacity");
     SLS_REQUIRE(((uintptr_t)workspace & 255) == 0, "workspace must be 256-byte aligned");
-    SLS_REQUIRE(reuse_rounds >= 0 && reuse_rounds <= 4, "reuse_rounds: 0 from scratch, 1..4 repair rounds");
-    SLS_REQUIRE(reuse_rounds == 0 || depth_order, "a repair needs the camera's previous depth order");
+    SLS_REQUIRE(reuse_rounds >= -1 && reuse_rounds <= 4, "reuse_rounds: 0 from scratch (-1: through the radix sort), 1..4 repair rounds");
+    SLS_REQUIRE(reuse_rounds <= 0 || depth_order, "a repair needs the camera's previous depth order");
     SLS_REQUIRE(list_pairs >= 0 && list_pairs <= 2, "list_pairs: 0 auto, 1 whenever possible, 2 never");
     const int H = cam->H, W = cam->W;
     const DevCam dc = make_devcam(*cam);
@@ -763,7 +766,7 @@
         SLS_REQUIRE(k.gt_depth && k.valid && k.col_cs && k.row_cs && k.col_cs_half && k.row_cs_half && k.depth_order,
                     "null per-keyframe pointer");
         SLS_REQUIRE((k.block_order != nullptr) == (kfs[0].block_order != nullptr), "block_order on every keyframe or on none");
-        SLS_REQUIRE(k.reuse_depth_order >= 0 && k.reuse_depth_order <= 4, "reuse_depth_order: 0 from scratch, 1..4 repair rounds");
+        SLS_REQUIRE(k.reuse_depth_order >= -1 && k.reuse_depth_order <= 4, "reuse_depth_order: 0 from scratch (-1: through the radix sort), 1..4 repair rounds");
         for (int h = 0; h < g; ++h) {
             SLS_REQUIRE(kfs[h].depth_order != k.depth_order, "two keyframes share one depth_order buffer");
             SLS_REQUIRE(!k.block_order || kfs[h].block_order != k.block_order, "two keyframes share one block_order buffer");
diff --git a/splat_loam_amd/csrc/sls_preprocess.hip b/splat_loam_amd/csrc/sls_preprocess.hip
--- a/splat_loam_amd/csrc/sls_preprocess.hip
+++ b/splat_loam_amd/csrc/sls_preprocess.hip
@@ -128,6 +128,8 @@
     uint32_t *status_clear;
     uint32_t *zero_words;
     int n_zero_words;
+    uint32_t *zero_words2;
+    int n_zero_words2;
 };
 
 template <bool EXACT>
@@ -172,6 +174,9 @@
     if (i == 0 && n_dev) *n_dev = (uint32_t)N;
     if (ra.zero_words && i < N) {
         for (int k = i; k < ra.n_zero_words; k += N) ra.zero_words[k] = 0u;
+    }
+    if (ra.zero_words2 && i < N) {
+        for (int k = i; k < ra.n_zero_words2; k += N) ra.zero_words2[k] = 0u;
     }
     if (i == 0 && ra.status_clear) {
 #pragma unroll
@@ -1037,6 +1042,7 @@
     RegArgs ra;
     ra.raw = a.raw; ra.smax = a.smax; ra.pen = a.pen; ra.reg_out = a.reg_out; ra.status_clear = a.status_clear;
     ra.zero_words = a.zero_words; ra.n_zero_words = a.n_zero_words;
+    ra.zero_words2 = a.zero_words2; ra.n_zero_words2 = a.n_zero_words2;
     PreFwdArgs pa;
     pa.means = a.means; pa.scales = (const float2 *)a.scales; pa.rots = (const float4 *)a.rots; pa.opac = a.opac;
     pa.rec = (float4 *)a.rec; pa.radii = a.radii; pa.rect = (int4 *)a.rect; pa.tiles = a.tiles; pa.depth = a.depth;
diff --git a/splat_loam_amd/csrc/sls_resort.hpp b/splat_loam_amd/csrc/sls_resort.hpp
--- a/splat_loam_amd/csrc/sls_resort.hpp
+++ b/splat_loam_amd/csrc/sls_resort.hpp
@@ -5,6 +5,7 @@
 
 constexpr int kResortWindow = 1024;
 constexpr uint32_t kResortFailed = 2u;
+constexpr uint32_t kOrderRebuildFailed = 64u;
 
 constexpr int kResortThreads = 512;
 static_assert(kResortWindow == 2 * kResortThreads, "one pair of elements per thread");
@@ -50,10 +51,11 @@
     keep64(e0, p0, keep_min);
     keep64(e1, p1, keep_min);
 }
-template <int K>
+template <int K, int W = kResortWindow>
 __device__ __forceinline__ void bitonic_width(uint64_t &e0, uint64_t &e1, ulonglong2 *s_pairs)
 {
-    const bool asc = (K == kResortWindow) || ((2 * (int)threadIdx.x) & K) == 0;
+    const bool asc = (K == W) || ((2 * (int)threadIdx.x) & K) == 0;
+    if constexpr (K >= 2048) bitonic_stage<512>(e0, e1, asc, s_pairs);
     if constexpr (K >= 1024) bitonic_stage<256>(e0, e1, asc, s_pairs);
     if constexpr (K >= 512) bitonic_stage<128>(e0, e1, asc, s_pairs);
     if constexpr (K >= 256) bitonic_stage<64>(e0, e1, asc, s_pairs);
@@ -67,19 +69,21 @@
     const uint64_t lo = sw ? e1 : e0, hi = sw ? e0 : e1;
     e0 = lo; e1 = hi;
 }
-template <int K0>
+template <int K0, int W = kResortWindow>
 __device__ __forceinline__ void bitonic_pairs(uint64_t &e0, uint64_t &e1, ulonglong2 *s_pairs)
 {
-    if constexpr (K0 <= 2) bitonic_width<2>(e0, e1, s_pairs);
-    if constexpr (K0 <= 4) bitonic_width<4>(e0, e1, s_pairs);
-    if constexpr (K0 <= 8) bitonic_width<8>(e0, e1, s_pairs);
-    if constexpr (K0 <= 16) bitonic_width<16>(e0, e1, s_pairs);
-    if constexpr (K0 <= 32) bitonic_width<32>(e0, e1, s_pairs);
-    if constexpr (K0 <= 64) bitonic_width<64>(e0, e1, s_pairs);
-    if constexpr (K0 <= 128) bitonic_width<128>(e0, e1, s_pairs);
-    if constexpr (K0 <= 256) bitonic_width<256>(e0, e1, s_pairs);
-    if constexpr (K0 <= 512) bitonic_width<512>(e0, e1, s_pairs);
-    bitonic_width<1024>(e0, e1, s_pairs);
+    static_assert(W == 1024 || W == 2048, "windows of 1024 (512 threads) or 2048 (1024 threads)");
+    if constexpr (K0 <= 2) bitonic_width<2, W>(e0, e1, s_pairs);
+    if constexpr (K0 <= 4) bitonic_width<4, W>(e0, e1, s_pairs);
+    if constexpr (K0 <= 8) bitonic_width<8, W>(e0, e1, s_pairs);
+    if constexpr (K0 <= 16) bitonic_width<16, W>(e0, e1, s_pairs);
+    if constexpr (K0 <= 32) bitonic_width<32, W>(e0, e1, s_pairs);
+    if constexpr (K0 <= 64) bitonic_width<64, W>(e0, e1, s_pairs);
+    if constexpr (K0 <= 128) bitonic_width<128, W>(e0, e1, s_pairs);
+    if constexpr (K0 <= 256) bitonic_width<256, W>(e0, e1, s_pairs);
+    if constexpr (K0 <= 512) bitonic_width<512, W>(e0, e1, s_pairs);
+    if constexpr (K0 <= 1024 || W == 1024) bitonic_width<1024, W>(e0, e1, s_pairs);
+    if constexpr (W == 2048) bitonic_width<2048, W>(e0, e1, s_pairs);
 }
 __device__ __forceinline__ int bitonic_src(int o)
 {
diff --git a/splat_loam_amd/csrc/sls_sort.hip b/splat_loam_amd/csrc/sls_sort.hip
--- a/splat_loam_amd/csrc/sls_sort.hip
+++ b/splat_loam_amd/csrc/sls_sort.hip
@@ -1219,6 +1219,166 @@
     if (keys64) keys64[j] = ((uint64_t)t << 32) | (uint64_t)__float_as_uint(depth[vals[j]]);
 }
 
+constexpr int kOrderBucketShift = 15, kOrderBuckets = 1 << (kDepthKeyBits - kOrderBucketShift);
+constexpr int kOrderThreads = 1024;
+constexpr int kOrderRunMax = 2048, kOrderRunStride = 1024;
+constexpr int kOrderHistPer = 4, kOrderScatterPer = 4;
+constexpr int kOrderOwn = kOrderBuckets / kOrderThreads;
+static_assert(kOrderRunMax == 2 * kOrderThreads && kOrderOwn % 4 == 0, "one pair per thread; whole uint4 of counts");
+
+__device__ __forceinline__ uint32_t order_bucket_of(uint32_t key) { return min(key >> kOrderBucketShift, (uint32_t)kOrderBuckets - 1u); }
+
+__device__ __forceinline__ uint32_t order_block_scan(uint32_t v, uint32_t *s_wave)
+{
+    const int lane = threadIdx.x & 63, wave = threadIdx.x >> 6;
+    uint32_t incl = v;
+#pragma unroll
+    for (int off = 1; off < 64; off <<= 1) {
+        const uint32_t t = __shfl_up(incl, off, 64);
+        if (lane >= off) incl += t;
+    }
+    if (lane == 63) s_wave[wave] = incl;
+    __syncthreads();
+    uint32_t run = incl - v;
+    for (int w = 0; w < wave; ++w) run += s_wave[w];
+    return run;
+}
+
+__global__ __launch_bounds__(kOrderThreads) void order_bucket_hist_kernel(int N, const uint32_t *__restrict__ keys,
+                                                                          uint32_t *__restrict__ hist)
+{
+    __shared__ __attribute__((aligned(16))) uint32_t s_cnt[kOrderBuckets];
+    const uint32_t first = blockIdx.x * (uint32_t)(kOrderThreads * kOrderHistPer) + threadIdx.x;
+    uint32_t k[kOrderHistPer];
+#pragma unroll
+    for (int q = 0; q < kOrderHistPer; ++q) k[q] = keys[min(first + (uint32_t)(q * kOrderThreads), (uint32_t)N - 1u)];
+#pragma unroll
+    for (int j = 0; j < kOrderOwn / 4; ++j) ((uint4 *)s_cnt)[threadIdx.x + j * kOrderThreads] = make_uint4(0u, 0u, 0u, 0u);
+    __syncthreads();
+#pragma unroll
+    for (int q = 0; q < kOrderHistPer; ++q)
+        if (first + (uint32_t)(q * kOrderThreads) < (uint32_t)N) atomicAdd(&s_cnt[order_bucket_of(k[q])], 1u);
+    __syncthreads();
+#pragma unroll
+    for (int j = 0; j < kOrderOwn; ++j) {
+        const int b = (int)threadIdx.x + j * kOrderThreads;
+        const uint32_t c = s_cnt[b];
+        if (c) atomicAdd(&hist[b], c);
+    }
+}
+
+__global__ __launch_bounds__(kOrderThreads) void order_bucket_scatter_kernel(int N, const uint32_t *__restrict__ keys,
+                                                                             const uint32_t *__restrict__ hist,
+                                                                             uint32_t *__restrict__ cursor,
+                                                                             uint64_t *__restrict__ pairs)
+{
+    __shared__ __attribute__((aligned(16))) uint32_t s_cnt[kOrderBuckets];
+    __shared__ __attribute__((aligned(16))) uint32_t s_base[kOrderBuckets];
+    __shared__ uint32_t s_wave[kOrderThreads / 64];
+    const uint32_t first = blockIdx.x * (uint32_t)(kOrderThreads * kOrderScatterPer) + threadIdx.x;
+    uint32_t k[kOrderScatterPer], rank[kOrderScatterPer];
+#pragma unroll
+    for (int q = 0; q < kOrderScatterPer; ++q) k[q] = keys[min(first + (uint32_t)(q * kOrderThreads), (uint32_t)N - 1u)];
+    uint4 h[kOrderOwn / 4];
+#pragma unroll
+    for (int j = 0; j < kOrderOwn / 4; ++j) h[j] = ((const uint4 *)hist)[threadIdx.x * (kOrderOwn / 4) + j];
+#pragma unroll
+    for (int j = 0; j < kOrderOwn / 4; ++j) ((uint4 *)s_cnt)[threadIdx.x + j * kOrderThreads] = make_uint4(0u, 0u, 0u, 0u);
+    __syncthreads();
+#pragma unroll
+    for (int q = 0; q < kOrderScatterPer; ++q) {
+        rank[q] = 0u;
+        if (first + (uint32_t)(q * kOrderThreads) < (uint32_t)N) rank[q] = atomicAdd(&s_cnt[order_bucket_of(k[q])], 1u);
+    }
+    uint32_t sum = 0;
+#pragma unroll
+    for (int j = 0; j < kOrderOwn / 4; ++j) sum += h[j].x + h[j].y + h[j].z + h[j].w;
+    uint32_t run = order_block_scan(sum, s_wave);
+#pragma unroll
+    for (int j = 0; j < kOrderOwn / 4; ++j) {
+        uint4 b;
+        b.x = run; run += h[j].x;
+        b.y = run; run += h[j].y;
+        b.z = run; run += h[j].z;
+        b.w = run; run += h[j].w;
+        ((uint4 *)s_base)[threadIdx.x * (kOrderOwn / 4) + j] = b;
+    }
+    __syncthreads();
+    uint32_t c[kOrderOwn], g[kOrderOwn];
+#pragma unroll
+    for (int j = 0; j < kOrderOwn; ++j) {
+        const int b = (int)threadIdx.x + j * kOrderThreads;
+        c[j] = s_cnt[b];
+        g[j] = 0u;
+        if (c[j]) g[j] = atomicAdd(&cursor[b], c[j]);
+    }
+#pragma unroll
+    for (int j = 0; j < kOrderOwn; ++j) {
+        const int b = (int)threadIdx.x + j * kOrderThreads;
+        if (c[j]) s_cnt[b] = s_base[b] + g[j];
+    }
+    __syncthreads();
+#pragma unroll
+    for (int q = 0; q < kOrderScatterPer; ++q) {
+        const uint32_t i = first + (uint32_t)(q * kOrderThreads);
+        const uint32_t pos = s_cnt[order_bucket_of(k[q])] + rank[q];
+        if (i < (uint32_t)N && pos < (uint32_t)N) pairs[pos] = ((uint64_t)k[q] << 32) | i;
+    }
+}
+
+__global__ __launch_bounds__(kOrderThreads) void order_run_sort_kernel(int N, const uint32_t *__restrict__ hist,
+                                                                       const uint64_t *__restrict__ pairs,
+                                                                       uint32_t *__restrict__ order,
+                                                                       uint32_t *__restrict__ fail_flag)
+{
+    __shared__ __attribute__((aligned(16))) ulonglong2 s_pairs[kOrderThreads];
+    __shared__ uint32_t s_wave[kOrderThreads / 64];
+    __shared__ uint32_t s_cut[2];
+    const uint32_t lo = blockIdx.x * (uint32_t)kOrderRunStride, hi = lo + (uint32_t)kOrderRunStride;
+    uint4 h[kOrderOwn / 4];
+#pragma unroll
+    for (int j = 0; j < kOrderOwn / 4; ++j) h[j] = ((const uint4 *)hist)[threadIdx.x * (kOrderOwn / 4) + j];
+    if (threadIdx.x < 2) s_cut[threadIdx.x] = (uint32_t)N;
+    uint32_t sum = 0;
+#pragma unroll
+    for (int j = 0; j < kOrderOwn / 4; ++j) sum += h[j].x + h[j].y + h[j].z + h[j].w;
+    uint32_t run = order_block_scan(sum, s_wave);
+    uint32_t m0 = (uint32_t)N, m1 = (uint32_t)N;
+    if (run + sum > lo) {
+#pragma unroll
+        for (int j = 0; j < kOrderOwn; ++j) {
+            const uint32_t cj = j % 4 == 0 ? h[j / 4].x : (j % 4 == 1 ? h[j / 4].y : (j % 4 == 2 ? h[j / 4].z : h[j / 4].w));
+            if (cj && run >= lo) m0 = min(m0, run);
+            if (cj && run >= hi) m1 = min(m1, run);
+            run += cj;
+        }
+    }
+#pragma unroll
+    for (int off = 32; off > 0; off >>= 1) {
+        m0 = min(m0, (uint32_t)__shfl_xor((int)m0, off, 64));
+        m1 = min(m1, (uint32_t)__shfl_xor((int)m1, off, 64));
+    }
+    if ((threadIdx.x & 63) == 0) {
+        if (m0 < (uint32_t)N) atomicMin(&s_cut[0], m0);
+        if (m1 < (uint32_t)N) atomicMin(&s_cut[1], m1);
+    }
+    __syncthreads();
+    const uint32_t e0 = s_cut[0], e1 = s_cut[1];
+    if (e0 >= e1) return;
+    const uint32_t n = e1 - e0;
+    if (n > (uint32_t)kOrderRunMax) {
+        if (threadIdx.x == 0) atomicOr(fail_flag, kOrderRebuildFailed);
+        for (uint32_t p = e0 + threadIdx.x; p < e1; p += (uint32_t)kOrderThreads) order[p] = min((uint32_t)pairs[p], (uint32_t)N - 1u);
+        return;
+    }
+    const uint32_t o = 2u * threadIdx.x;
+    const uint64_t a0 = pairs[min(e0 + o, (uint32_t)N - 1u)], a1 = pairs[min(e0 + o + 1u, (uint32_t)N - 1u)];
+    uint64_t v0 = o < n ? a0 : ~0ull, v1 = o + 1u < n ? a1 : ~0ull;
+    bitonic_pairs<2, kOrderRunMax>(v0, v1, s_pairs);
+    if (o < n) order[e0 + o] = (uint32_t)v0;
+    if (o + 1u < n) order[e0 + o + 1u] = (uint32_t)v1;
+}
+
 static int bits_for(uint32_t max_value)
 {
     int b = 0;
@@ -1226,10 +1386,17 @@
     return b;
 }
 
+static size_t order_tables_offset(int N)
+{
+    const size_t n = (size_t)(N > 0 ? N : 1);
+    return (sizeof(uint32_t) * (3 * n + (n + 255) / 256 + 64) + sort_scratch_bytes(n) + 16 + n / 32 + 128 + 15) & ~(size_t)15;
+}
+static_assert(kOrderRebuildWords == 2 * kOrderBuckets, "bucket counts + bucket cursors");
+uint32_t *order_rebuild_tables(int N, void *scratch) { return (uint32_t *)((char *)scratch + order_tables_offset(N)); }
+
 size_t order_scratch_bytes(int N)
 {
-    const size_t n = (size_t)(N > 0 ? N : 1);
-    return sizeof(uint32_t) * (3 * n + (n + 255) / 256 + 64) + sort_scratch_bytes(n) + 16 + n / 32 + 128;
+    return order_tables_offset(N) + sizeof(uint32_t) * (size_t)kOrderRebuildWords;
 }
 
 struct OrderScratch {
@@ -1317,6 +1484,27 @@
         }
         resort_windows = nB;
         resort_edges = edges;
+    } else if (a.bucket_rebuild) {
+        uint32_t *hist = order_rebuild_tables(N, a.scratch), *cursor = hist + kOrderBuckets;
+        {
+            ScopedTimer tm(T_SORT_HIST, st);
+            hipLaunchKernelGGL(order_bucket_hist_kernel, dim3((N + kOrderThreads * kOrderHistPer - 1) / (kOrderThreads * kOrderHistPer)),
+                               dim3(kOrderThreads), 0, st, N, (const uint32_t *)keys, hist);
+        }
+        SLS_LAUNCH_CHECK("order_bucket_hist_kernel");
+        {
+            ScopedTimer tm(T_SORT_SCATTER, st);
+            hipLaunchKernelGGL(order_bucket_scatter_kernel,
+                               dim3((N + kOrderThreads * kOrderScatterPer - 1) / (kOrderThreads * kOrderScatterPer)), dim3(kOrderThreads),
+                               0, st, N, (const uint32_t *)keys, (const uint32_t *)hist, cursor, s.comp);
+        }
+        SLS_LAUNCH_CHECK("order_bucket_scatter_kernel");
+        {
+            ScopedTimer tm(T_RESORT, st);
+            hipLaunchKernelGGL(order_run_sort_kernel, dim3((N + kOrderRunStride - 1) / kOrderRunStride), dim3(kOrderThreads), 0, st, N,
+                               (const uint32_t *)hist, (const uint64_t *)s.comp, order, a.fail_flag);
+        }
+        SLS_LAUNCH_CHECK("order_run_sort_kernel");
     } else {
         int which = 0;
         int rc = radix_sort_pairs_t<uint32_t>(keys, v0, s.keys_tmp, v1, s.n_dev, (uint32_t)N, kDepthKeyBits, s.sort_scratch,
diff --git a/splat_loam_amd/engine.py b/splat_loam_amd/engine.py
--- a/splat_loam_amd/engine.py
+++ b/splat_loam_amd/engine.py
@@ -91,7 +91,9 @@
         self._orders = {}
         self._set_order_ages()
         self.max_cached_orders = 64
-        self.stats = {"repeated_too_small": 0, "repeated_resort": 0, "repeated_exchange": 0, "repeated_det": 0}
+        self.stats = {"repeated_too_small": 0, "repeated_resort": 0, "repeated_exchange": 0, "repeated_det": 0,
+                      "repeated_rebuild": 0}
+        self.rebuild_through_radix = False
         self._enq = 0
         self.dp_mode = os.environ.get("SLS_DP_MODE", "rs_ag")
         self._dp = None
@@ -160,10 +162,14 @@
         ent = self._orders.get(id(camera))
         return ent if ent is not None and ent[2]() is camera else None
 
-    def _forget_order(self, camera, failed_repair=False):
+    def _forget_order(self, camera, failed_repair=False, failed_rebuild=False):
         ent = self._order_entry(camera)
+        if failed_repair and ent is not None and ent[4] == 0 and dist.is_initialized():
+            failed_repair, failed_rebuild = False, True
         if ent is not None:
             ent[1] = None
+            if failed_rebuild:
+                ent[5] = True
         if failed_repair:
             self._repair_rounds = min(self._repair_rounds + 1, 3)
             self._repair_until = self._enq + self.repair_span
@@ -185,7 +191,8 @@
             if len(self._orders) >= self.max_cached_orders:
                 self._orders.pop(next(iter(self._orders)))
             ent = [torch.empty((self.N,), dtype=torch.int32, device=self.dev), None, weakref.ref(camera),
-                   torch.zeros((int(lib.sls_block_order_bytes(H, W)) // 4,), dtype=torch.int32, device=self.dev)]
+                   torch.zeros((int(lib.sls_block_order_bytes(H, W)) // 4,), dtype=torch.int32, device=self.dev),
+                   None, False]
             self._orders[id(camera)] = ent
         age = self._enq - ent[1] if ent[1] is not None else None
         reuse = allow_reuse and self.reuse_depth_order and age is not None and age <= self.max_order_age_extra
@@ -195,6 +202,9 @@
         reuse = min(self._repair_rounds + (1 if age is not None and age > self.max_order_age else 0)
                     + (1 if age is not None and age > self.order_age_round3 else 0)
                     + (1 if age is not None and age > self.order_age_round4 else 0), 4) if reuse else 0
+        if reuse == 0 and (ent[5] or self.rebuild_through_radix):
+            reuse = -1
+        ent[4] = reuse
         if advance:
             self._enq += 1
             ent[1] = self._enq
@@ -267,6 +277,8 @@
             return "repeated_too_small"
         if st["resort_failed"]:
             return "repeated_resort"
+        if st.get("rebuild_failed"):
+            return "repeated_rebuild"
         return "repeated_det" if st.get("det_mispredicted") else "repeated_exchange"
 
     def _sharded(self, group):
@@ -296,6 +308,7 @@
         R, flags = int(h[0].item()) & 0xFFFFFFFF, int(h[1].item())
         f = h.view(torch.float32)
         return {"R": R, "overflow": bool(flags), "too_small": bool(flags & 1), "resort_failed": bool(flags & 2),
+                "rebuild_failed": bool(flags & 64),
                 "exchange_too_small": bool(flags & 4), "det_mispredicted": bool(flags & 8),
                 "handover_mismatch": bool(flags & 16), "outside_union": bool(flags & 32),
                 "exchange_count": int(h[7].item()) & 0xFFFFFFFF,
@@ -308,6 +321,7 @@
         f = h.view(np.float32)
         R, flags = int(h[0]) & 0xFFFFFFFF, int(h[1])
         return {"R": R, "overflow": bool(flags), "too_small": bool(flags & 1), "resort_failed": bool(flags & 2),
+                "rebuild_failed": bool(flags & 64),
                 "exchange_too_small": bool(flags & 4), "det_mispredicted": bool(flags & 8),
                 "handover_mismatch": bool(flags & 16), "outside_union": bool(flags & 32),
                 "exchange_count": int(h[7]) & 0xFFFFFFFF,
@@ -349,8 +363,8 @@
                 self.last = st
                 self.pose_grad = self._pose_buf[0] if pose_grad else None
                 return st
-            if st["too_small"] or st["resort_failed"]:
-                self._forget_order(camera, failed_repair=st["resort_failed"])
+            if st["too_small"] or st["resort_failed"] or st["rebuild_failed"]:
+                self._forget_order(camera, failed_repair=st["resort_failed"], failed_rebuild=st["rebuild_failed"])
             self.stats[self._void_reason(st)] += 1
             if st["too_small"]:
                 need = st["R"]
@@ -374,8 +388,8 @@
             if not st["overflow"]:
                 self.pose_grad = self._pose_buf[0]
                 return st
-            if st["too_small"] or st["resort_failed"]:
-                self._forget_order(camera, failed_repair=st["resort_failed"])
+            if st["too_small"] or st["resort_failed"] or st["rebuild_failed"]:
+                self._forget_order(camera, failed_repair=st["resort_failed"], failed_rebuild=st["rebuild_failed"])
             self.stats[self._void_reason(st)] += 1
             if st["too_small"]:
                 self.capacity = int(max(st["R"], self.capacity) * self.capacity_factor) + 1024
@@ -491,8 +505,8 @@
                 self.pose_grad = self._pose_buf[:len(cams)] if pose_grad else None
                 return st
             for cam, kst in zip(cams, st["keyframes"]):
-                if kst["too_small"] or kst["resort_failed"]:
-                    self._forget_order(cam, failed_repair=kst["resort_failed"])
+                if kst["too_small"] or kst["resort_failed"] or kst["rebuild_failed"]:
+                    self._forget_order(cam, failed_repair=kst["resort_failed"], failed_rebuild=kst["rebuild_failed"])
             self.stats[self._void_reason(st)] += 1
             if st["too_small"]:
                 need = st["R"]
@@ -558,10 +572,10 @@
         cur_st = self._note(self._parse_status(self._lag_dev[cur[0]].cpu())) if cur is not None else None
         cur_void = cur_st is not None and cur_st["overflow"]
         self.t -= 2 if cur is not None else 1
-        if st["too_small"] or st["resort_failed"]:
-            self._forget_order(pcam, failed_repair=st["resort_failed"])
-        if cur_void and (cur_st["too_small"] or cur_st["resort_failed"]):
-            self._forget_order(cur[1], failed_repair=cur_st["resort_failed"])
+        if st["too_small"] or st["resort_failed"] or st["rebuild_failed"]:
+            self._forget_order(pcam, failed_repair=st["resort_failed"], failed_rebuild=st["rebuild_failed"])
+        if cur_void and (cur_st["too_small"] or cur_st["resort_failed"] or cur_st["rebuild_failed"]):
+            self._forget_order(cur[1], failed_repair=cur_st["resort_failed"], failed_rebuild=cur_st["rebuild_failed"])
         self.stats[self._void_reason(st)] += 1
         if st["too_small"] or (cur_void and cur_st["too_small"]):
             need = max(st["R"], cur_st["R"] if cur_void else 0, self.capacity)
diff --git a/splat_loam_amd/rasterizer.py b/splat_loam_amd/rasterizer.py
--- a/splat_loam_amd/rasterizer.py
+++ b/splat_loam_amd/rasterizer.py
@@ -343,6 +343,7 @@
 _WS_CACHE: "OrderedDict[tuple, _WsEntry]" = OrderedDict()
 _WS_CACHE_MAX = 4
 _WS_ORDERS_MAX = 64
+rebuild_through_radix = False
 _SENTINEL = -1
 
 
@@ -441,7 +442,7 @@
     age = None if ent[1] is None else e.calls - ent[1]
     if e.rounds > 1 and e.calls >= e.rounds_until:
         e.rounds, e.rounds_until = e.rounds - 1, e.calls + 256
-    reuse = 0
+    reuse = -1 if rebuild_through_radix else 0
     if age is not None and age <= int(48 * scale):
         reuse = min(e.rounds + (1 if age > int(4 * scale) else 0) + (1 if age > int(12 * scale) else 0), 4)
     radii = torch.empty((N,), dtype=torch.int32, device=dev)
@@ -471,8 +472,8 @@
         if flags & 2:
             e.stats["repair_failed"] += 1
             e.rounds, e.rounds_until = min(e.rounds + 1, 3), e.calls + 256
-        reuse = 0
-    e.stats["repaired" if reuse else "from_scratch"] += 1
+        reuse = -1 if (flags & 64 or reuse < 0) else 0
+    e.stats["repaired" if reuse > 0 else "from_scratch"] += 1
     e.stats["R"] = R
     e.calls += 1
     ent[1] = e.calls
```
